# succinctlabs/sp1

Hardware: AMD Instinct MI355X
Metric: RISC-V cycles proved/sec (core shard prove): whole ShardProof of a full core shard of the reference's `fibonacci` guest, see config (higher is better)
Workload: dtype u32 (KoalaBear Montgomery words, exact integer arithmetic)

## Files before the change

### sp1_amd/csrc/gkr.hip

```cpp
#include <algorithm>
#include <array>
#include <chrono>
#include <cstring>
#include <optional>
#include <string>
#include <vector>

#include "device_ctx.hpp"
#include "host_par.hpp"

namespace sp1hip {
bool gkr_host_simd_available();
void gkr_host_round_sums(const uint32_t* tab, size_t stride, const uint32_t* eq, size_t eq_stride, size_t real_pairs, uint32_t out[6][4]);
void gkr_host_round_fold(const uint32_t* tab, uint32_t* out, size_t stride, size_t real_pairs, const uint32_t alpha[4]);
}
#include "round_sync.hpp"
#include "tensor_table.hpp"
#include "ext_host.hpp"
#include "gkr_kernels.hpp"
#include "gkr_rounds_host.hpp"

namespace sp1hip {

void challenger_observe(sp1hip_challenger_t* ch, uint32_t x);
kb::Ext challenger_sample_ext(sp1hip_challenger_t* ch);
void challenger_restore(sp1hip_challenger_t* dst, const sp1hip_challenger_t* src);

namespace gkr {

using namespace ext_host;

using gkr_rounds::Poly4;
Ext poly_eval(const Poly4& c, const Ext& x) { return ((c[3] * x + c[2]) * x + c[1]) * x + c[0]; }

Poly4 interpolate4(const Ext (&xs)[4], const Ext (&ys)[4]) {
    Poly4 res{kb::ext_zero(), kb::ext_zero(), kb::ext_zero(), kb::ext_zero()};
    Ext num[4][4], den[4];
    bool live[4];
    for (int i = 0; i < 4; i++) {
        live[i] = !kb::ext_eq(ys[i], kb::ext_zero());
        if (!live[i]) continue;
        den[i] = kb::ext_one();
        Ext cur[4] = {ys[i], kb::ext_zero(), kb::ext_zero(), kb::ext_zero()};
        int deg = 0;
        for (int j = 0; j < 4; j++) {
            if (j == i) continue;
            den[i] = den[i] * (xs[i] - xs[j]);
            Ext nxt[4] = {kb::ext_zero(), kb::ext_zero(), kb::ext_zero(), kb::ext_zero()};
            for (int k = 0; k <= deg; k++) { nxt[k + 1] = nxt[k + 1] + cur[k]; nxt[k] = nxt[k] - cur[k] * xs[j]; }
            deg++;
            for (int k = 0; k < 4; k++) cur[k] = nxt[k];
        }
        for (int k = 0; k < 4; k++) num[i][k] = cur[k];
    }
    Ext prefix[4], running = kb::ext_one();
    for (int i = 0; i < 4; i++) if (live[i]) { prefix[i] = running; running = running * den[i]; }
    Ext inv_all = kb::ext_inv(running);
    for (int i = 3; i >= 0; i--) {
        if (!live[i]) continue;
        const Ext inv = inv_all * prefix[i];
        inv_all = inv_all * den[i];
        for (int k = 0; k < 4; k++) res[k] = res[k] + num[i][k] * inv;
    }
    return res;
}

struct Bytes {
    std::vector<uint8_t> b;
    void u64(uint64_t v) { for (int i = 0; i < 8; i++) b.push_back((uint8_t)(v >> (8 * i))); }
    void felt(uint32_t m) { const uint32_t v = kb::from_monty(m); for (int i = 0; i < 4; i++) b.push_back((uint8_t)(v >> (8 * i))); }
    void ext(const Ext& e) { for (int k = 0; k < 4; k++) felt(e.c[k]); }
};

void observe_ext(sp1hip_challenger_t* ch, const Ext& e) { for (int k = 0; k < 4; k++) challenger_observe(ch, e.c[k]); }

struct ChipInfo {
    std::string name;
    uint32_t rows, k, main_w, prep_w, int0;
    const uint32_t* d_main;
    const uint32_t* d_prep;
};

constexpr uint32_t MAX_TILES = 512;
constexpr uint64_t GKR_LOOKAHEAD_DEFAULT = 4;
uint32_t tiles_for(uint64_t threads) { return (uint32_t)std::min<uint64_t>(std::max<uint64_t>((threads + 255) / 256, 1), MAX_TILES); }

struct ParsedInt { uint32_t is_send, kind; std::vector<uint32_t> mult; std::vector<std::vector<uint32_t>> values; };
struct RoundOut { Ext n0, n1, d0, d1; std::vector<Poly4> polys; Ext claimed_sum, eval; std::vector<Ext> point; };
struct PassShape { int fv, sv; bool first; uint32_t tiles, tile_size, total_slots; size_t flat_off; bool flat; };

struct GkrTimer {
    enum Part { ROWS, INT, LAYER_HEAD, WAIT, HOST, LAUNCH, SKIP };
    using Clock = std::chrono::steady_clock;
    bool on = false;
    Clock::time_point last, clk[2];
    double part_ms[7] = {};
    int waits = 0;
    static double ms(Clock::time_point a, Clock::time_point b) { return std::chrono::duration<double, std::milli>(b - a).count(); }
    void start() { static const bool env = env_flag("SP1HIP_GKR_DEBUG", false); on = env; last = Clock::now(); }
    void mark(const char* what) {
        if (!on) return;
        const auto now = Clock::now();
        fprintf(stderr, "[sp1hip gkr] %-28s %8.3f ms\n", what, ms(last, now));
        last = now;
    }
    void lap(Part p) {
        if (!on) return;
        const auto now = Clock::now();
        part_ms[p] += ms(clk[p >= WAIT], now);
        clk[p >= WAIT] = now;
        waits += p == WAIT;
    }
    void report_layers() {
        if (!on) return;
        fprintf(stderr, "[sp1hip gkr]   of which row-variable rounds %.3f ms, interaction-variable rounds (host) %.3f ms\n", part_ms[ROWS], part_ms[INT]);
        fprintf(stderr, "[sp1hip gkr]   %d hand-overs inside the layers: waiting for the sums %.3f ms, closed forms + transcript %.3f ms, launch calls %.3f ms\n",
                waits, part_ms[WAIT], part_ms[HOST], part_ms[LAUNCH]);
    }
};

struct Levels {
    int L = 0;
    uint32_t K = 0;
    std::vector<uint32_t> h;
    std::vector<size_t> entries;
    std::vector<std::vector<size_t>> off;
    std::vector<DeviceBuf> N, D;
    uint32_t rows_at(uint32_t i, int l) const { return (uint32_t)(((uint64_t)h[i] + (((uint64_t)1 << (L - l)) - 1)) >> (L - l)); }
    void* n_ptr(int l, uint32_t i) const { return (char*)N[l].p + off[l][i] * (l == L ? 4 : 16); }
    Ext* d_ptr(int l, uint32_t i) const { return D[l].ext() + off[l][i]; }
    int alloc(int L_, std::vector<uint32_t> rows_of_interaction, hipStream_t s) {
        L = L_; h = std::move(rows_of_interaction); K = (uint32_t)h.size();
        entries.assign(L + 2, 0);
        off.assign(L + 1, std::vector<size_t>(K + 1, 0));
        for (int l = 1; l <= L; l++) {
            for (uint32_t i = 0; i < K; i++) off[l][i + 1] = off[l][i] + rows_at(i, l);
            entries[l] = off[l][K];
        }
        N = std::vector<DeviceBuf>(L + 1); D = std::vector<DeviceBuf>(L + 1);
        for (int l = 1; l <= L; l++) {
            SP1HIP_TRY(N[l].alloc(std::max<size_t>(entries[l], 1) * (l == L ? 4 : 16), s));
            SP1HIP_TRY(D[l].alloc(std::max<size_t>(entries[l], 1) * 16, s));
        }
        return SP1HIP_SUCCESS;
    }
};

struct PassPlan {
    std::vector<PassShape> shapes;
    std::vector<PassDesc> all_descs;
    std::vector<uint16_t> flat_index;
};
struct PassChoice { int sv; bool flat; uint64_t total_slots; };
PassChoice choose_pass(const std::vector<uint32_t>& rows_in, int fv, int left, int depth, uint32_t flat_max_slots) {
    auto total_slots = [&](int sv) {
        uint64_t n = 0;
        for (uint32_t rin : rows_in) { const uint32_t ro = (rin + (1u << fv) - 1) >> fv; n += ((ro + (1u << sv) - 1) >> sv) << sv; }
        return n;
    };
    const bool index_fits = rows_in.size() <= 65536;
    if (depth > 2 && left > 2) {
        const int sv = std::min(depth, left);
        const uint64_t n = total_slots(sv);
        if (n <= flat_max_slots && index_fits) return PassChoice{sv, true, n};
    }
    const int sv = std::min(2, left);
    const uint64_t n = total_slots(sv);
    return PassChoice{sv, n <= flat_max_slots && index_fits, n};
}
size_t count_passes(const Levels& lv, uint32_t flat_max_slots, int depth) {
    size_t n = 0;
    std::vector<uint32_t> rows_in(lv.K);
    for (int v = 1; v <= lv.L - 1; v++) {
        for (uint32_t i = 0; i < lv.K; i++) rows_in[i] = (lv.rows_at(i, v + 1) + 1) / 2;
        for (int t = v, fv = 0;;) {
            const int sv = choose_pass(rows_in, fv, t - fv, depth, flat_max_slots).sv;
            for (uint32_t& r : rows_in) r = (r + (1u << fv) - 1) >> fv;
            t -= fv;
            n++;
            if (sv == 0) break;
            fv = sv;
        }
    }
    return n;
}

void plan_passes(const Levels& lv, uint32_t flat_max_slots, int depth, size_t n_passes, Ext* const (&scratch)[2], Ext* host_rows, PassPlan& plan) {
    const uint32_t K = lv.K;
    auto scratch_ptr = [&](int b, uint32_t i, int which, const std::vector<size_t>& so) -> Ext* { return scratch[b] + 4 * so[i] + (size_t)which * (so[i + 1] - so[i]); };
    constexpr uint32_t TARGET_TILES = 2048;
    plan.all_descs.reserve(n_passes * K);
    std::vector<uint32_t> rows_in(K);
    std::vector<size_t> so_prev, so_next;
    for (int v = 1; v <= lv.L - 1; v++) {
        for (uint32_t i = 0; i < K; i++) rows_in[i] = (lv.rows_at(i, v + 1) + 1) / 2;
        int cur = 0, t = v, fv = 0, pass = 0;
        for (;;) {
            const PassChoice choice = choose_pass(rows_in, fv, t - fv, depth, flat_max_slots);
            const int sv = choice.sv;
            const bool first = pass <= 1;
            if (fv > 0) { so_next.assign(K + 1, 0); for (uint32_t i = 0; i < K; i++) so_next[i + 1] = so_next[i] + ((rows_in[i] + (1u << fv) - 1) >> fv); }
            auto slots_of = [&](uint32_t rin) -> uint32_t { const uint32_t ro = (rin + (1u << fv) - 1) >> fv; return ((ro + (1u << sv) - 1) >> sv) << sv; };
            const uint64_t total_slots = choice.total_slots;
            const bool flat = choice.flat;
            const uint32_t tile_size = flat ? 1u : (uint32_t)std::max<uint64_t>(256, ((total_slots + TARGET_TILES - 1) / TARGET_TILES + 255) / 256 * 256);
            const size_t flat_off = plan.flat_index.size();
            plan.all_descs.resize(plan.all_descs.size() + K);
            PassDesc* out = plan.all_descs.data() + plan.all_descs.size() - K;
            uint32_t tile0 = 0;
            for (uint32_t i = 0; i < K; i++) {
                PassDesc& d = out[i];
                d = PassDesc{};
                d.rows_in = rows_in[i]; d.eq_int_index = i;
                if (first) { d.src[0] = lv.n_ptr(v + 1, i); d.src[1] = lv.d_ptr(v + 1, i); d.rows_x = lv.rows_at(i, v + 1); }
                else for (int w = 0; w < 4; w++) d.src[w] = scratch_ptr(cur ^ 1, i, w, so_prev);
                if (fv > 0) for (int w = 0; w < 4; w++)
                    d.dst[w] = (sv == 0 && host_rows) ? host_rows + 4 * so_next[i] + (size_t)w * (so_next[i + 1] - so_next[i]) : scratch_ptr(cur, i, w, so_next);
                d.tile0 = tile0;
                const uint32_t n_tiles = (slots_of(rows_in[i]) + tile_size - 1) / tile_size;
                if (flat) plan.flat_index.insert(plan.flat_index.end(), n_tiles, (uint16_t)i);
                tile0 += n_tiles;
// ... 97 lines not shown
        for (int w = 0; w < 4; w++) { tab[0][w].assign(W, (w & 1) ? kb::ext_one() : kb::ext_zero()); tab[1][w].resize(W / 2 + 1); }
    }
    void set_row(uint32_t i, const Ext* row) { for (int w = 0; w < 4; w++) tab[0][w][i] = row[w]; }
    RoundSums sums(int m, size_t real_pairs) const {
        const std::vector<Ext>& eqi = eq.tabs[m];
        const Ext *n0 = tab[side][0].data(), *d0 = tab[side][1].data(), *n1 = tab[side][2].data(), *d1 = tab[side][3].data();
        RoundSums parts[HostPar::Scope::MAX_THREADS];
        const int nparts = par.threads();
        for (int q = 0; q < nparts; q++) parts[q] = RoundSums{kb::ext_zero(), kb::ext_zero(), kb::ext_zero(), kb::ext_zero(), kb::ext_zero(), kb::ext_zero()};
        par.run(real_pairs, 24, [&](int part, size_t kb0, size_t ke) {
            RoundSums acc = parts[part];
            for (size_t k = kb0; k < ke; k++) {
                const size_t a = 2 * k, b = 2 * k + 1;
                acc.x0 = acc.x0 + eqi[a] * (d0[a] * n1[a] + d1[a] * n0[a]);
                acc.y0 = acc.y0 + eqi[a] * (d0[a] * d1[a]);
                const Ext sn0 = n0[a] + n0[b], sn1 = n1[a] + n1[b], sd0 = d0[a] + d0[b], sd1 = d1[a] + d1[b];
                const Ext es = eqi[a] + eqi[b];
                acc.xh = acc.xh + es * (sd0 * sn1 + sd1 * sn0);
                acc.yh = acc.yh + es * (sd0 * sd1);
                acc.e0 = acc.e0 + eqi[a];
                acc.es = acc.es + es;
            }
            parts[part] = acc;
        });
        RoundSums t = parts[0];
        for (int q = 1; q < nparts; q++) {
            t.x0 = t.x0 + parts[q].x0; t.y0 = t.y0 + parts[q].y0; t.xh = t.xh + parts[q].xh; t.yh = t.yh + parts[q].yh;
            t.e0 = t.e0 + parts[q].e0; t.es = t.es + parts[q].es;
        }
        return t;
    }
    void fold(size_t real_pairs, size_t half, const Ext& alpha) {
        const Ext *n0 = tab[side][0].data(), *d0 = tab[side][1].data(), *n1 = tab[side][2].data(), *d1 = tab[side][3].data();
        Ext *o0 = tab[side ^ 1][0].data(), *o1 = tab[side ^ 1][1].data(), *o2 = tab[side ^ 1][2].data(), *o3 = tab[side ^ 1][3].data();
        par.run(real_pairs, 48, [&](int, size_t kb0, size_t ke) {
            for (size_t k = kb0; k < ke; k++) {
                o0[k] = n0[2 * k] + alpha * (n0[2 * k + 1] - n0[2 * k]); o1[k] = d0[2 * k] + alpha * (d0[2 * k + 1] - d0[2 * k]);
                o2[k] = n1[2 * k] + alpha * (n1[2 * k + 1] - n1[2 * k]); o3[k] = d1[2 * k] + alpha * (d1[2 * k + 1] - d1[2 * k]);
            }
        });
        if (real_pairs < half) { o0[real_pairs] = kb::ext_zero(); o1[real_pairs] = kb::ext_one(); o2[real_pairs] = kb::ext_zero(); o3[real_pairs] = kb::ext_one(); }
        side ^= 1;
    }
    void first_row(Ext (&f)[4]) const { for (int w = 0; w < 4; w++) f[w] = tab[side][w][0]; }
};

template <class Tables>
void interaction_rounds(Tables& tb, size_t real, const std::vector<Ext>& int_point, const Ext& lambda, const Ext& PA, const Consts& k, LayerRounds& lr) {
    const int niv = (int)int_point.size();
    Ext eq_scale = k.one;
    for (int j = 0; j < niv; j++) {
        const size_t half = ((size_t)1 << (niv - j)) / 2, real_pairs = (real + 1) / 2;
        const RoundSums t = tb.sums(niv - j, real_pairs);
        const Ext pt = int_point[niv - 1 - j];
        const Ext s0 = lambda * t.x0 + t.y0 + ((k.one - pt) - t.e0);
        const Ext sh = lambda * t.xh + t.yh + (k.one - t.es) * k.four;
        const Ext PAe = PA * eq_scale;
        const Ext p0 = PAe * s0, ph = PAe * sh * k.inv8;
        const Ext xs[4] = {k.zero, k.one, k.inv2, (k.one - pt) * kb::ext_inv(k.one - (pt + pt))};
        const Ext ys[4] = {p0, lr.claim - p0, ph, k.zero};
        tb.fold(real_pairs, half, lr.finish_round(interpolate4(xs, ys), pt, eq_scale));
        real = real_pairs;
    }
    Ext f[4];
    tb.first_row(f);
    lr.ro.n0 = f[0]; lr.ro.d0 = f[1]; lr.ro.n1 = f[2]; lr.ro.d1 = f[3];
}

void interaction_rounds_host(bool simd, HostPar::Scope& par, const EqTabs& eq, uint32_t W, const std::vector<size_t>& so, const Ext* rows,
                             const std::vector<Ext>& int_point, const Ext& lambda, const Ext& PA, const Consts& k, LayerRounds& lr, GkrTimer& timer) {
    auto run = [&](auto tb) {
        const uint32_t K = (uint32_t)so.size() - 1;
        for (uint32_t i = 0; i < K; i++) if (so[i + 1] != so[i]) tb.set_row(i, rows + 4 * so[i]);
        timer.lap(GkrTimer::ROWS);
        interaction_rounds(tb, K, int_point, lambda, PA, k, lr);
        timer.lap(GkrTimer::INT);
    };
    if (simd) run(PlaneTables(eq, W)); else run(ScalarTables(eq, par, W));
}

#define SP1HIP_GKR_REQUIRE(cond, msg) \
    do { if (!(cond)) { sp1hip::set_error("sp1hip_logup_gkr_prove: %s", msg); return SP1HIP_ERROR_INVALID_ARGUMENT; } } while (0)

struct GkrProver {
    const sp1hip_gkr_chip_t* const chips;
    const int n_chips, L;
    sp1hip_challenger_t* const challenger;
    uint8_t* const h_proof;
    size_t* const proof_len;
    const sp1hip_stream_t stream;
    const hipStream_t s;

    GkrTimer timer;
    const Consts k;
    std::vector<ChipInfo> info;
    std::vector<ParsedInt> progs;
    size_t max_arity = 0, total_cols = 0, need = 0;
    uint32_t K = 0, W = 0;
    int niv = 0;
    struct Cloned { sp1hip_challenger_t* c = nullptr; ~Cloned() { sp1hip_challenger_free(c); } } clone;
    sp1hip_challenger_t* ch = nullptr;
    uint32_t witness = 0, flat_max_slots = 0;
    int lookahead = 2;
    Ext alpha;
    std::vector<Ext> betas;
    std::vector<uint32_t> int_chip;
    Levels lv;
    size_t n_passes_total = 0;
    hipStream_t side = nullptr;
    hipEvent_t* side_ev = nullptr;
    DeviceBuf d_all, d_flat;
    PinnedStage side_stage, stage;
    DeviceBuf d_progs, d_betas, d_descs;
    std::vector<uint32_t> flat;
    std::vector<IntDesc> descs;
    DeviceBuf d_trans, d_trans2;
    Mailbox mb;
    DeviceBuf d_eq_int, d_T, d_TL, d_partials, scratch[2];
    bool direct_final = false, simd = false;
    PassPlan plan;
    std::vector<Ext> out_n, out_d, eval_point;
    Ext num_eval, den_eval;
    size_t launch_idx = 0;
    RoundSyncHost rsync;
    std::optional<HostPar::Scope> par;
    std::vector<RoundOut> rounds;
    std::vector<Ext> trace_point, openings;

    int parse_programs() {
        info.resize(n_chips);
        for (int c = 0; c < n_chips; c++) {
            const sp1hip_gkr_chip_t& ci = chips[c];
            SP1HIP_GKR_REQUIRE(ci.name && ci.interactions, "null chip field");
            SP1HIP_GKR_REQUIRE(ci.real_rows <= ((uint64_t)1 << L), "chip taller than 2^max_log_row_count");
            SP1HIP_GKR_REQUIRE(ci.real_rows == 0 || ci.main_width == 0 || ci.d_main, "null main trace");
            SP1HIP_GKR_REQUIRE(ci.real_rows == 0 || ci.prep_width == 0 || ci.d_prep, "null preprocessed trace");
            if (c) SP1HIP_GKR_REQUIRE(strcmp(chips[c - 1].name, ci.name) < 0, "chips must be sorted by name (BTreeSet order)");
            info[c] = ChipInfo{ci.name, (uint32_t)ci.real_rows, 0, ci.main_width, ci.prep_width, (uint32_t)progs.size(), ci.d_main, ci.d_prep};
            const uint32_t* p = ci.interactions;
            const uint32_t* end = p + ci.n_words;
            SP1HIP_GKR_REQUIRE(ci.n_words >= 1, "empty interaction program");
            const uint32_t ni = *p++;
            info[c].k = ni;
            auto vcol = [&](std::vector<uint32_t>& out) -> bool {
                if (p + 2 > end) return false;
                const uint32_t nt = p[0];
                if (p[1] >= kb::P || p + 2 + 3 * (size_t)nt > end) return false;
                out.push_back(nt);
                out.push_back(kb::to_monty(p[1]));
                p += 2;
                for (uint32_t t = 0; t < nt; t++, p += 3) {
                    if (p[0] > 1 || p[2] >= kb::P) return false;
                    if (p[1] >= (p[0] ? ci.main_width : ci.prep_width)) return false;
                    out.push_back(p[0]); out.push_back(p[1]); out.push_back(kb::to_monty(p[2]));
                }
                return true;
            };
            for (uint32_t i = 0; i < ni; i++) {
                SP1HIP_GKR_REQUIRE(p + 3 <= end, "truncated interaction program");
                const uint32_t nv = p[2];
                SP1HIP_GKR_REQUIRE(p[0] <= 1 && p[1] < kb::P && nv < 4096, "bad interaction header");
                ParsedInt pi{p[0], p[1], {}, std::vector<std::vector<uint32_t>>(nv)};
                p += 3;
                SP1HIP_GKR_REQUIRE(vcol(pi.mult), "bad multiplicity column");
                for (uint32_t j = 0; j < nv; j++) SP1HIP_GKR_REQUIRE(vcol(pi.values[j]), "bad value column (index or weight out of range)");
                max_arity = std::max<size_t>(max_arity, nv + 1);
                progs.push_back(std::move(pi));
            }
            SP1HIP_GKR_REQUIRE(p == end, "trailing words in interaction program");
            total_cols += (size_t)ci.main_width + ci.prep_width;
        }
        K = (uint32_t)progs.size();
        SP1HIP_GKR_REQUIRE(K >= 1, "no interactions in the shard");
        niv = log2_ceil(K);
        W = 1u << niv;
        return SP1HIP_SUCCESS;
    }

    size_t proof_size() const {
        size_t n = 2 * (8 + (size_t)2 * W * 16 + 24) + 8;
        for (int v = 1; v <= L - 1; v++) n += 64 + 8 + (size_t)(niv + v) * (8 + 64) + 16 + 8 + (size_t)(niv + v) * 16 + 16;
        n += 8 + (size_t)L * 16 + 8;
        for (int c = 0; c < n_chips; c++) {
            n += 8 + info[c].name.size() + 8 + (size_t)info[c].main_w * 16 + 16 + 1;
            if (info[c].prep_w) n += 8 + (size_t)info[c].prep_w * 16 + 16;
        }
        return n + 4;
    }

    int transcript_head() {
        SP1HIP_TRY(sp1hip_challenger_clone(challenger, &clone.c));
        ch = clone.c;
        SP1HIP_TRY(sp1hip_challenger_grind(ch, 12, &witness, stream));
        alpha = challenger_sample_ext(ch);
        std::vector<Ext> beta_seed(log2_ceil(max_arity));
        for (auto& b : beta_seed) b = challenger_sample_ext(ch);
        (void)challenger_sample_ext(ch);
        betas = partial_lagrange_host(beta_seed);
        return SP1HIP_SUCCESS;
    }

    int alloc_levels_and_plan_buffers() {
        int_chip.resize(K);
        std::vector<uint32_t> rows(K);
        for (int c = 0; c < n_chips; c++) for (uint32_t i = 0; i < info[c].k; i++) { int_chip[info[c].int0 + i] = c; rows[info[c].int0 + i] = info[c].rows; }
        SP1HIP_TRY(lv.alloc(L, std::move(rows), s));
        timer.mark("parse + level buffers");
        flat_max_slots = (uint32_t)env_uint("SP1HIP_GKR_FLAT_SLOTS", 65536);
        lookahead = (int)std::min<uint64_t>(std::max<uint64_t>(env_uint("SP1HIP_GKR_LOOKAHEAD", GKR_LOOKAHEAD_DEFAULT), 2), 4);
        n_passes_total = count_passes(lv, flat_max_slots, lookahead);
        SP1HIP_TRY(aux_stream_for(s, 2, &side, &side_ev));
        SP1HIP_TRY(d_all.alloc(std::max<size_t>(n_passes_total * K, 1) * sizeof(PassDesc), side));
        SP1HIP_TRY(d_flat.alloc((n_passes_total * (size_t)flat_max_slots + 4) * sizeof(uint16_t), side));
        SP1HIP_TRY(side_stage.init(side));
        return stage.init(s);
    }

    int build_first_layer_and_tree() {
        std::vector<size_t> poff(K);
        for (uint32_t i = 0; i < K; i++) {
            poff[i] = flat.size();
            const ParsedInt& pi = progs[i];
            Ext head = alpha + kb::ext_mul_base(betas[0], kb::to_monty(pi.kind));
            uint32_t live = 0;
            for (size_t j = 0; j < pi.values.size(); j++) {
                if (pi.values[j][0] == 0) head = head + kb::ext_mul_base(betas[1 + j], pi.values[j][1]);
                else live++;
            }
            flat.insert(flat.end(), {pi.is_send, live, head.c[0], head.c[1], head.c[2], head.c[3]});
            flat.insert(flat.end(), pi.mult.begin(), pi.mult.end());
            for (size_t j = 0; j < pi.values.size(); j++) {
                if (pi.values[j][0] == 0) continue;
                flat.push_back((uint32_t)(1 + j));
                flat.insert(flat.end(), pi.values[j].begin(), pi.values[j].end());
            }
        }
        SP1HIP_TRY(upload(d_progs, flat.data(), flat.size() * 4, s, stage));
        SP1HIP_TRY(upload(d_betas, betas.data(), betas.size() * 16, s, stage));
        uint32_t max_rows = 0;
        descs.resize(K);
        for (uint32_t i = 0; i < K; i++) {
            const ChipInfo& c = info[int_chip[i]];
            descs[i] = IntDesc{d_progs.u32() + poff[i], c.d_main, c.d_prep, c.rows, (uint32_t*)lv.n_ptr(L, i), lv.d_ptr(L, i)};
            max_rows = std::max(max_rows, c.rows);
        }
        const bool fused_tree = L >= 3 && env_flag("SP1HIP_GKR_FUSED", true);
        if (fused_tree) {
            std::vector<FirstDesc> fdescs(K);
            for (uint32_t i = 0; i < K; i++)
                fdescs[i] = FirstDesc{descs[i].prog, descs[i].main, descs[i].prep, descs[i].rows, descs[i].n_out, descs[i].d_out,
                                      (Ext*)lv.n_ptr(L - 1, i), lv.d_ptr(L - 1, i), (Ext*)lv.n_ptr(L - 2, i), lv.d_ptr(L - 2, i)};
            SP1HIP_TRY(upload(d_descs, fdescs.data(), fdescs.size() * sizeof(FirstDesc), s, stage));
            if (max_rows) {
                ScopedTimer t("gkr_first_layer", s);
                hipLaunchKernelGGL(first_layers_kernel, dim3(tiles_for((max_rows + 3) / 4), K), dim3(256), 0, s, (const FirstDesc*)d_descs.p,
                                   (const Ext*)d_betas.p);
                SP1HIP_LAUNCH_CHECK();
            }
        } else {
            SP1HIP_TRY(upload(d_descs, descs.data(), descs.size() * sizeof(IntDesc), s, stage));
            if (max_rows) {
                ScopedTimer t("gkr_first_layer", s);
                hipLaunchKernelGGL(first_layer_kernel, dim3(tiles_for(max_rows), K), dim3(256), 0, s, (const IntDesc*)d_descs.p,
                                   (const Ext*)d_betas.p);
                SP1HIP_LAUNCH_CHECK();
            }
        }
        timer.mark("first layer enqueued");
        const int top = fused_tree ? L - 2 : L;
        std::vector<Trans2Desc> t2;
        std::vector<TransDesc> t1;
        std::vector<uint32_t> t2_mr, t1_mr;
        std::vector<int> t1_level;
        int l = top;
        if (fused_tree)
            for (; l >= 3; l -= 2) {
                uint32_t mr = 0;
                for (uint32_t i = 0; i < K; i++) {
                    const uint32_t rin = lv.rows_at(i, l);
                    t2.push_back(Trans2Desc{(const Ext*)lv.n_ptr(l, i), lv.d_ptr(l, i), (Ext*)lv.n_ptr(l - 1, i), lv.d_ptr(l - 1, i), (Ext*)lv.n_ptr(l - 2, i), lv.d_ptr(l - 2, i), rin});
                    mr = std::max(mr, (rin + 3) / 4);
                }
                t2_mr.push_back(mr);
            }
        for (; l >= 2; l--) {
            uint32_t mr = 0;
            for (uint32_t i = 0; i < K; i++) {
                const uint32_t rin = lv.rows_at(i, l);
                t1.push_back(TransDesc{lv.n_ptr(l, i), lv.d_ptr(l, i), (Ext*)lv.n_ptr(l - 1, i), lv.d_ptr(l - 1, i), rin});
                mr = std::max(mr, (rin + 1) / 2);
            }
            t1_mr.push_back(mr);
            t1_level.push_back(l);
        }
        if (!t2.empty()) SP1HIP_TRY(upload(d_trans2, t2.data(), t2.size() * sizeof(Trans2Desc), s, stage));
        if (!t1.empty()) SP1HIP_TRY(upload(d_trans, t1.data(), t1.size() * sizeof(TransDesc), s, stage));
        for (size_t j = 0; j < t2_mr.size(); j++) {
            if (!t2_mr[j]) continue;
            ScopedTimer t("gkr_transition", s);
            hipLaunchKernelGGL(transition2_kernel, dim3(tiles_for(t2_mr[j]), K), dim3(256), 0, s, (const Trans2Desc*)d_trans2.p + j * K);
            SP1HIP_LAUNCH_CHECK();
        }
        for (size_t j = 0; j < t1_mr.size(); j++) {
            if (!t1_mr[j]) continue;
            const TransDesc* d_t = (const TransDesc*)d_trans.p + j * K;
            ScopedTimer t("gkr_transition", s);
            if (t1_level[j] == L) hipLaunchKernelGGL(transition_kernel<true>, dim3(tiles_for(t1_mr[j]), K), dim3(256), 0, s, d_t);
            else hipLaunchKernelGGL(transition_kernel<false>, dim3(tiles_for(t1_mr[j]), K), dim3(256), 0, s, d_t);
            SP1HIP_LAUNCH_CHECK();
        }
        timer.mark("tree enqueued");
        return SP1HIP_SUCCESS;
    }

    int plan_and_upload_passes() {
        SP1HIP_TRY(mb.init(s));
        SP1HIP_TRY(d_eq_int.alloc((size_t)W * 16, s));
        SP1HIP_TRY(d_T.alloc(((size_t)2 << std::max(L - 1, 1)) * 16, s));
// ... 201 lines not shown
            for (uint32_t g = 0; g < info[c].prep_w; g += OPEN_COLS) od.push_back(OpenDesc{info[c].d_prep, info[c].rows, info[c].prep_w, g, out0 + g});
            out0 += info[c].prep_w;
            max_rows_open = std::max(max_rows_open, info[c].rows);
        }
        const uint32_t chunks = std::max<uint32_t>((max_rows_open + OPEN_ROWS - 1) / OPEN_ROWS, 1);
        SP1HIP_TRY(upload(d_od, od.data(), od.size() * sizeof(OpenDesc), s, stage));
        SP1HIP_TRY(d_part.alloc((size_t)chunks * total_cols * 16, s));
        SP1HIP_TRY(d_res.alloc(total_cols * 16, s));
        SP1HIP_HIP(hipMemsetAsync(d_part.p, 0, (size_t)chunks * total_cols * 16, s));
        ScopedTimer t("gkr_openings", s);
        hipLaunchKernelGGL(open_columns_kernel, dim3((uint32_t)od.size(), chunks), dim3(256), 0, s, (const OpenDesc*)d_od.p, d_eq.u32(),
                           1u << L, d_part.u32(), (uint32_t)total_cols);
        SP1HIP_LAUNCH_CHECK();
        hipLaunchKernelGGL(open_sum_kernel, dim3(((uint32_t)total_cols * 4 + 63) / 64), dim3(256), 0, s, d_part.u32(), chunks,
                           (uint32_t)total_cols * 4, d_res.u32());
        SP1HIP_LAUNCH_CHECK();
        return mb.fetch(d_res.p, total_cols * 4, openings.data());
    }

    void observe_openings() {
        challenger_observe(ch, kb::to_monty((uint32_t)n_chips));
        size_t o = 0;
        for (int c = 0; c < n_chips; c++) {
            const Ext* main = openings.data() + o;
            const Ext* prep = main + info[c].main_w;
            if (info[c].prep_w) {
                challenger_observe(ch, kb::to_monty(info[c].prep_w));
                for (uint32_t j = 0; j < info[c].prep_w; j++) observe_ext(ch, prep[j]);
            }
            challenger_observe(ch, kb::to_monty(info[c].main_w));
            for (uint32_t j = 0; j < info[c].main_w; j++) observe_ext(ch, main[j]);
            o += info[c].main_w + info[c].prep_w;
        }
        timer.mark("openings");
    }

    int write_proof() {
        Bytes w;
        for (const std::vector<Ext>* vv : {&out_n, &out_d}) {
            w.u64(vv->size());
            for (auto& e : *vv) w.ext(e);
            w.u64(2); w.u64(vv->size()); w.u64(1);
        }
        w.u64(rounds.size());
        for (auto& r : rounds) {
            w.ext(r.n0); w.ext(r.n1); w.ext(r.d0); w.ext(r.d1);
            w.u64(r.polys.size());
            for (auto& p : r.polys) { w.u64(4); for (auto& c : p) w.ext(c); }
            w.ext(r.claimed_sum);
            w.u64(r.point.size());
            for (auto& x : r.point) w.ext(x);
            w.ext(r.eval);
        }
        w.u64(trace_point.size());
        for (auto& x : trace_point) w.ext(x);
        w.u64(n_chips);
        size_t o = 0;
        for (int c = 0; c < n_chips; c++) {
            w.u64(info[c].name.size());
            for (char chr : info[c].name) w.b.push_back((uint8_t)chr);
            w.u64(info[c].main_w);
            for (uint32_t j = 0; j < info[c].main_w; j++) w.ext(openings[o + j]);
            w.u64(1); w.u64(info[c].main_w);
            w.b.push_back(info[c].prep_w ? 1 : 0);
            if (info[c].prep_w) {
                w.u64(info[c].prep_w);
                for (uint32_t j = 0; j < info[c].prep_w; j++) w.ext(openings[o + info[c].main_w + j]);
                w.u64(1); w.u64(info[c].prep_w);
            }
            o += info[c].main_w + info[c].prep_w;
        }
        w.felt(witness);
        if (w.b.size() != need) {
            set_error("internal error: GKR proof size %zu != expected %zu", w.b.size(), need);
            return SP1HIP_ERROR_RUNTIME;
        }
        memcpy(h_proof, w.b.data(), w.b.size());
        *proof_len = w.b.size();
        return SP1HIP_SUCCESS;
    }

    int prove() {
        timer.start();
        SP1HIP_TRY(parse_programs());
        need = proof_size();
        if (!h_proof || *proof_len < need) {
            *proof_len = need;
            set_error("sp1hip_logup_gkr_prove: proof buffer too small, need %zu bytes", need);
            return SP1HIP_ERROR_BUFFER_TOO_SMALL;
        }
        const DeviceCtx* ctx;
        SP1HIP_TRY(get_device_ctx(&ctx));
        SP1HIP_TRY(transcript_head());
        SP1HIP_TRY(alloc_levels_and_plan_buffers());
        SP1HIP_TRY(build_first_layer_and_tree());
        SP1HIP_TRY(plan_and_upload_passes());
        SP1HIP_TRY(fetch_circuit_output());
        SP1HIP_TRY(prove_layers());
        SP1HIP_TRY(open_traces());
        observe_openings();
        SP1HIP_TRY(write_proof());
        challenger_restore(challenger, ch);
        return SP1HIP_SUCCESS;
    }
};
#undef SP1HIP_GKR_REQUIRE
}
}

using namespace sp1hip;

extern "C" int sp1hip_logup_gkr_prove(const sp1hip_gkr_chip_t* chips, int n_chips, int max_log_row_count, sp1hip_challenger_t* challenger,
                                      uint8_t* h_proof, size_t* proof_len, sp1hip_stream_t stream) {
    SP1HIP_REQUIRE(chips && n_chips > 0 && challenger && proof_len, "bad argument");
    SP1HIP_REQUIRE(max_log_row_count >= 1 && max_log_row_count <= 30, "max_log_row_count out of range");
    gkr::GkrProver p{chips, n_chips, max_log_row_count, challenger, h_proof, proof_len, stream, S(stream)};
    return p.prove();
}
```

### sp1_amd/csrc/jagged.hip

```cpp
#include <algorithm>
#include <array>
#include <chrono>
#include <cstring>
#include <vector>

#include "device_ctx.hpp"
#include "jagged_host.hpp"
#include "round_sync.hpp"
#include "stacked_data.hpp"
#include "tensor_table.hpp"
#include "ext_host.hpp"
#include "jagged_kernels.hpp"

namespace sp1hip {

void challenger_observe(sp1hip_challenger_t* ch, uint32_t x);
kb::Ext challenger_sample_ext(sp1hip_challenger_t* ch);
void challenger_restore(sp1hip_challenger_t* dst, const sp1hip_challenger_t* src);

namespace {

using namespace ext_host;

struct Bytes {
// ... 99 lines not shown
};

struct StageMarks {
    bool open = false;
    void next(const char* name) { if (open) roctx_pop(); roctx_push(name); open = true; }
    ~StageMarks() { if (open) roctx_pop(); }
};

struct FirstRoundsPlan {
    int rf = 0;
    std::vector<JgTab> tabs0;
    uint32_t n_tiles0 = 0, n_tiles1 = 0, n_tiles2 = 0;
    bool tables_mult4 = false;
    bool skip_level1 = false;
    bool lookahead01 = false;
    std::vector<std::pair<uint64_t, uint64_t>> zero_tails;
    bool table_major() const { return !tabs0.empty(); }
};

FirstRoundsPlan plan_first_rounds(const std::vector<uint32_t>& prefix, uint32_t T, int log_m, int max_log_row_count,
                                  StackedCore* const* rounds, int n_rounds, bool factored, bool lookahead) {
    FirstRoundsPlan pl;
    uint32_t g = T;
    for (uint32_t pfx : prefix) g |= pfx;
    pl.rf = g ? __builtin_ctz(g) : 0;
    pl.rf = std::min(pl.rf, std::min(log_m - 2, max_log_row_count - 1));
    if (!factored) pl.rf = 0;
    if (pl.rf < 2) pl.rf = 0;
    if ((g & 1u) != 0 || !factored) return pl;
    uint64_t seg_start = 0;
    uint32_t col = 0;
    for (int r = 0; r < n_rounds; r++) {
        const StackedCore* d = rounds[r];
        uint64_t off = 0;
        const size_t n_real = d->row_counts.size() - 2;
        for (size_t t = 0; t < d->row_counts.size(); t++) {
            const uint32_t h = (uint32_t)d->row_counts[t], w = (uint32_t)d->column_counts[t];
            if (t < n_real && h && w) {
                for (uint32_t c_lo = 0; c_lo < w; c_lo += JG_COL_SLICE) {
                    const uint32_t wc = std::min(JG_COL_SLICE, w - c_lo);
                    const uint64_t o = off + (uint64_t)c_lo * h;
                    pl.tabs0.push_back(JgTab{(const uint32_t*)d->d_dense + o, h, col + c_lo, wc, pl.n_tiles0, (uint32_t)(seg_start + o),
                                             pl.n_tiles1, pl.n_tiles2});
                    pl.n_tiles0 += (h / 2 + JG_TAB_PAIRS - 1) / JG_TAB_PAIRS;
                    pl.n_tiles1 += ((h + 3) / 4 + JG_TAB_PAIRS - 1) / JG_TAB_PAIRS;
                    pl.n_tiles2 += ((h + 7) / 8 + JG_TAB_PAIRS - 1) / JG_TAB_PAIRS;
                }
            }
            if (t == n_real) pl.zero_tails.push_back({seg_start + off, seg_start + d->padded});
            off += (uint64_t)h * w;
            col += w;
        }
        seg_start += d->padded;
    }
    if (pl.table_major()) {
        pl.tables_mult4 = (g & 3u) == 0;
        pl.skip_level1 = (g & 7u) == 0 && pl.rf >= 2 && log_m >= 4;
        pl.lookahead01 = pl.skip_level1 && lookahead;
    }
    return pl;
}

void build_layer_matrices(const std::vector<Ext>& z_row, const std::vector<Ext>& z_index, int D, std::vector<Ext>* out) {
    auto lsb = [](const std::vector<Ext>& p, size_t i) { return p.size() <= i ? kb::ext_zero() : p[p.size() - 1 - i]; };
    out->assign((size_t)D * 4 * 16, kb::ext_zero());
    const Ext one = kb::ext_one();
    for (int layer = 0; layer < D; layer++) {
        const Ext zr = lsb(z_row, layer), zi = lsb(z_index, layer);
        const Ext er[2] = {one - zr, zr}, ei[2] = {one - zi, zi};
        for (int cb = 0; cb < 2; cb++)
            for (int nb = 0; nb < 2; nb++)
                for (int m = 0; m < 4; m++) {
                    const int carry = m & 1, cmp = m >> 1;
                    for (int rb = 0; rb < 2; rb++)
                        for (int ib = 0; ib < 2; ib++) {
                            const int sum = rb + carry + cb;
                            if (ib != (sum & 1)) continue;
                            const int new_cmp = ib == nb ? cmp : nb;
                            const int target = (sum >> 1) + 2 * new_cmp;
                            Ext& e = (*out)[(((size_t)layer * 4 + cb * 2 + nb) * 4 + m) * 4 + target];
                            e = e + er[rb] * ei[ib];
                        }
                }
    }
}

struct JeProver {
    const std::vector<uint32_t>& prefix;
    const int D;
    const std::vector<Ext>&z_row, &z_col, &z_trace;
    Scratch& sc;
    RoundTranscript& tr;

    const hipStream_t s = sc.s;
    const Ext half = kb::ext_inv(ext_c(2));
    uint32_t n = 0, nb = 0;
    std::vector<Ext> mats;
    DeviceBuf d_t, d_u, d_zc, d_mats, d_suffix, d_state, d_inter;
    JeCols C{};
    std::vector<Ext> B;
    DeviceBuf d_B, d_suffix2;

    int setup_columns() {
        const std::vector<Ext> col_eq = partial_lagrange_host(z_col);
        std::vector<uint32_t> ts, us;
        std::vector<Ext> zc;
        for (size_t c = 0; c + 1 < prefix.size(); c++) {
            if (!ts.empty() && ts.back() == prefix[c] && us.back() == prefix[c + 1]) zc.back() = zc.back() + col_eq[c];
            else { ts.push_back(prefix[c]); us.push_back(prefix[c + 1]); zc.push_back(col_eq[c]); }
        }
        n = (uint32_t)ts.size();
        SP1HIP_TRY(upload(d_t, ts.data(), n * 4, s, sc.stage));
        SP1HIP_TRY(upload(d_u, us.data(), n * 4, s, sc.stage));
        SP1HIP_TRY(upload(d_zc, zc.data(), (size_t)n * 16, s, sc.stage));
        build_layer_matrices(z_row, z_trace, D, &mats);
        SP1HIP_TRY(upload(d_mats, mats.data(), mats.size() * 16, s, sc.stage));
        SP1HIP_TRY(d_suffix.alloc((size_t)D * n * 64, s));
        SP1HIP_TRY(d_state.alloc((size_t)n * 128, s));
        SP1HIP_TRY(d_inter.alloc((size_t)n * 16, s));
        C = JeCols{d_t.u32(), d_u.u32(), d_zc.ext(), n};
        nb = Scratch::blocks_for(n);
        return SP1HIP_SUCCESS;
    }

    int finish_round() {
        SP1HIP_LAUNCH_CHECK();
        Ext y0, yh;
        SP1HIP_TRY(sc.finish(&y0, &yh));
        tr.finish_round(y0, yh + yh + yh + yh);
        return SP1HIP_SUCCESS;
    }

    int phase1() {
        hipLaunchKernelGGL(je_suffix_kernel<true>, dim3(nb), dim3(256), 0, s, C, (const Ext*)d_mats.p, D, d_suffix.ext(), sc.tail());
        SP1HIP_LAUNCH_CHECK();
        Ext expected_sum, unused;
        SP1HIP_TRY(sc.finish(&expected_sum, &unused));
        observe_ext(tr.ch, expected_sum);
        tr.begin(expected_sum);
        for (int r = 0; r < D; r++) {
            hipLaunchKernelGGL(je_phase1_round, dim3(nb), dim3(256), 0, s, C, (const Ext*)d_mats.p, (const Ext*)d_suffix.p, D, r, tr.alpha,
                               half, d_state.ext(), d_inter.ext(), sc.tail());
            SP1HIP_TRY(finish_round());
        }
        return SP1HIP_SUCCESS;
    }

    int phase2() {
        B.resize((size_t)D * 2 * 16);
        for (int layer = 0; layer < D; layer++)
            for (int cb = 0; cb < 2; cb++)
                for (int e = 0; e < 16; e++) {
                    const Ext a0 = mats[((size_t)layer * 4 + cb * 2 + 0) * 16 + e], a1 = mats[((size_t)layer * 4 + cb * 2 + 1) * 16 + e];
                    B[((size_t)layer * 2 + cb) * 16 + e] = a0 + tr.alphas[layer] * (a1 - a0);
                }
        SP1HIP_TRY(upload(d_B, B.data(), B.size() * 16, s, sc.stage));
        SP1HIP_TRY(d_suffix2.alloc((size_t)D * n * 64, s));
        hipLaunchKernelGGL(je_suffix_kernel<false>, dim3(nb), dim3(256), 0, s, C, (const Ext*)d_B.p, D, d_suffix2.ext(), sc.tail());
        SP1HIP_LAUNCH_CHECK();
        Ext W[4] = {kb::ext_one(), kb::ext_zero(), kb::ext_zero(), kb::ext_zero()};
        for (int rp = 0; rp < D; rp++) {
            Ext V[8];
            for (int b = 0; b < 2; b++)
                for (int k = 0; k < 4; k++) {
                    Ext acc = kb::ext_zero();
                    for (int m = 0; m < 4; m++) acc = acc + W[m] * B[((size_t)rp * 2 + b) * 16 + 4 * m + k];
// ... 500 lines not shown
```

### sp1_amd/csrc/prover.hip

```cpp
#include <algorithm>
#include <array>
#include <cstring>
#include <functional>
#include <memory>
#include <vector>

#include "basefold_host.hpp"

namespace sp1hip {


struct DuplexChallenger {
    uint32_t state[16] = {0};
    uint32_t in[8];
    int n_in = 0;
    uint32_t out[8];
    int n_out = 0;
    uint32_t injected[4];
    int n_injected = 0, next_injected = 0;

    void duplexing() {
        for (int i = 0; i < n_in; i++) state[i] = in[i];
        n_in = 0;
        p2_host_permute(state);
// ... 406 lines not shown
    *out = new sp1hip_challenger_s(*ch);
    return SP1HIP_SUCCESS;
}
void sp1hip_challenger_free(sp1hip_challenger_t* ch) { delete ch; }
int sp1hip_challenger_observe(sp1hip_challenger_t* ch, const uint32_t* felts, size_t n) {
    SP1HIP_REQUIRE(ch && (felts || n == 0), "null argument");
    for (size_t i = 0; i < n; i++) SP1HIP_REQUIRE(felts[i] < kb::P, "non-reduced field word");
    ch->ch.observe_slice(felts, n);
    return SP1HIP_SUCCESS;
}
int sp1hip_challenger_sample(sp1hip_challenger_t* ch, uint32_t* out) {
    SP1HIP_REQUIRE(ch && out, "null argument");
    *out = ch->ch.sample();
    return SP1HIP_SUCCESS;
}
int sp1hip_challenger_sample_ext(sp1hip_challenger_t* ch, sp1hip_ext_t* out) {
    SP1HIP_REQUIRE(ch && out, "null argument");
    kb::Ext e = ch->ch.sample_ext();
    memcpy(out->c, e.c, 16);
    return SP1HIP_SUCCESS;
}
int sp1hip_challenger_sample_bits(sp1hip_challenger_t* ch, int bits, uint32_t* out) {
    SP1HIP_REQUIRE(ch && out && bits >= 0 && bits < 32, "bad argument");
    *out = ch->ch.sample_bits(bits);
    return SP1HIP_SUCCESS;
}
int sp1hip_challenger_check_witness(sp1hip_challenger_t* ch, int bits, uint32_t witness, int* ok) {
    SP1HIP_REQUIRE(ch && ok && bits >= 0 && bits < 32 && witness < kb::P, "bad argument");
    *ok = ch->ch.check_witness(bits, witness) ? 1 : 0;
    return SP1HIP_SUCCESS;
}
int sp1hip_challenger_grind(sp1hip_challenger_t* ch, int bits, uint32_t* witness, sp1hip_stream_t stream) {
    SP1HIP_REQUIRE(ch && witness, "null argument");
    return grind(ch->ch, bits, witness, S(stream));
}
int sp1hip_challenger_inject_pow_witnesses(sp1hip_challenger_t* ch, const uint32_t* witnesses, int n) {
    SP1HIP_REQUIRE(ch && n >= 0 && n <= 4 && (witnesses || n == 0), "bad argument");
    for (int i = 0; i < n; i++) SP1HIP_REQUIRE(witnesses[i] < kb::P, "witness not a canonical field element");
    for (int i = 0; i < n; i++) ch->ch.injected[i] = witnesses[i];
    ch->ch.n_injected = n;
    ch->ch.next_injected = 0;
    return SP1HIP_SUCCESS;
}
int sp1hip_challenger_state(const sp1hip_challenger_t* ch, uint32_t* out34) {
    SP1HIP_REQUIRE(ch && out34, "null argument");
    memset(out34, 0, 34 * 4);
    memcpy(out34, ch->ch.state, 64);
    out34[16] = (uint32_t)ch->ch.n_in;
    memcpy(out34 + 17, ch->ch.in, 4 * ch->ch.n_in);
    out34[25] = (uint32_t)ch->ch.n_out;
    memcpy(out34 + 26, ch->ch.out, 4 * ch->ch.n_out);
    return SP1HIP_SUCCESS;
}

}

namespace sp1hip {
int basefold_data_alloc(BasefoldData* pd, const sp1hip_tensor_t* mles, int n_mles, int lg_n, int lg_blowup, hipStream_t s) {
    pd->lg_n = lg_n;
    pd->lg_blowup = lg_blowup;
    const size_t N = (size_t)1 << (lg_n + lg_blowup);
    for (int i = 0; i < n_mles; i++) {
        pd->mles.push_back(mles[i]);
        pd->cws.emplace_back(new DeviceBuf());
        SP1HIP_TRY(pd->cws.back()->alloc(N * mles[i].width * 4, s));
        pd->cw_tensors.push_back({pd->cws.back()->u32(), mles[i].width});
        pd->total_width += mles[i].width;
    }
    return pd->tree.alloc((2 * N - 1) * 32, s);
}

int basefold_data_fetch_commit(BasefoldData* pd, const uint32_t* d_root_and_commit, uint32_t h_commit[8], hipStream_t s) {
    uint32_t h[16];
    Mailbox mb;
    SP1HIP_TRY(mb.init(s));
    SP1HIP_TRY(mb.fetch(d_root_and_commit, 16, h));
    memcpy(pd->root, h, 32);
    memcpy(pd->commit, h + 8, 32);
    memcpy(h_commit, pd->commit, 32);
    return SP1HIP_SUCCESS;
}

int commit_mles_hooked(const sp1hip_tensor_t* mles, int n_mles, int lg_n, int lg_blowup, uint32_t h_commit[8],
                       sp1hip_basefold_data_t** out, sp1hip_stream_t stream, const std::function<int(int, hipStream_t)>* before_encode) {
    SP1HIP_REQUIRE(mles && n_mles > 0 && out && h_commit, "bad argument");
    SP1HIP_REQUIRE(lg_n >= 0 && lg_blowup >= 0 && lg_n + lg_blowup <= kb::TWO_ADICITY, "size out of range");
    hipStream_t s = S(stream);
    const DeviceCtx* ctx;
    SP1HIP_TRY(get_device_ctx(&ctx));
    std::unique_ptr<sp1hip_basefold_data_s> pd(new sp1hip_basefold_data_s());
    for (int i = 0; i < n_mles; i++) SP1HIP_REQUIRE(mles[i].d_data || mles[i].width == 0, "null mle");
    SP1HIP_TRY(basefold_data_alloc(pd.get(), mles, n_mles, lg_n, lg_blowup, s));
    const int lg_h = lg_n + lg_blowup;
    const size_t N = (size_t)1 << lg_h;
    DeviceBuf rc;
    SP1HIP_TRY(rc.alloc(64, s));
    const bool overlap = env_flag("SP1HIP_COMMIT_OVERLAP", N * (size_t)pd->total_width >= ((size_t)1 << 24));
    std::vector<LeafPart> parts;
    if (overlap) leaf_hash_plan(pd->cw_tensors.data(), n_mles, &parts);
    if (parts.size() >= 2) {
        hipStream_t aux;
        hipEvent_t* ev;
        SP1HIP_TRY(aux_stream_for(s, n_mles + 1, &aux, &ev));
        struct Join {
            hipStream_t aux;
            ~Join() { (void)hipStreamSynchronize(aux); }
        };
        TensorTable tab;
        uint32_t tw;
        SP1HIP_TRY(make_tensor_table(pd->cw_tensors.data(), n_mles, &tab, &tw));
        DeviceBuf cols, carry;
        SP1HIP_TRY(cols.alloc((size_t)tw * sizeof(uint32_t*), s));
        SP1HIP_TRY(carry.alloc(N * 8 * 4, s));
        SP1HIP_TRY(expand_columns_async(tab, tw, N, (const uint32_t**)cols.p, s));
        SP1HIP_HIP(hipEventRecord(ev[n_mles], s));
        SP1HIP_HIP(hipStreamWaitEvent(aux, ev[n_mles], 0));
        {
            Join join{aux};
            for (int i = 0; i < n_mles; i++) {
                if (before_encode) SP1HIP_TRY((*before_encode)(i, aux));
                SP1HIP_TRY(sp1hip_rs_encode_batch(pd->cws[i]->u32(), mles[i].d_data, lg_n, lg_blowup, mles[i].width, aux));
                SP1HIP_HIP(hipEventRecord(ev[i], aux));
            }
            for (int k = 0; k < (int)parts.size(); k++) {
                SP1HIP_HIP(hipStreamWaitEvent(s, ev[parts[k].last_tensor], 0));
                SP1HIP_TRY(leaf_hash_part((const uint32_t* const*)cols.p + parts[k].c0, parts[k].width, k, (int)parts.size(),
                                          (uint32_t)N, carry.u32(), pd->tree.u32(), ctx, s));
            }
            SP1HIP_TRY(merkle_finish_tree(pd->tree.u32(), lg_h, tw, rc.u32(), ctx, s));
            SP1HIP_TRY(basefold_data_fetch_commit(pd.get(), rc.u32(), h_commit, s));
        }
        *out = pd.release();
        return SP1HIP_SUCCESS;
    }
    for (int i = 0; i < n_mles; i++) {
        if (before_encode) SP1HIP_TRY((*before_encode)(i, s));
        SP1HIP_TRY(sp1hip_rs_encode_batch(pd->cws[i]->u32(), mles[i].d_data, lg_n, lg_blowup, mles[i].width, s));
    }
    SP1HIP_TRY(sp1hip_merkle_commit(pd->cw_tensors.data(), n_mles, lg_h, pd->tree.u32(), rc.u32(), s));
    SP1HIP_TRY(basefold_data_fetch_commit(pd.get(), rc.u32(), h_commit, s));
    *out = pd.release();
    return SP1HIP_SUCCESS;
}
}

extern "C" {

int sp1hip_commit_mles(const sp1hip_tensor_t* mles, int n_mles, int lg_n, int lg_blowup, uint32_t h_commit[8],
                       sp1hip_basefold_data_t** out, sp1hip_stream_t stream) {
    return commit_mles_hooked(mles, n_mles, lg_n, lg_blowup, h_commit, out, stream, nullptr);
}

void sp1hip_basefold_data_free(sp1hip_basefold_data_t* data) { delete data; }

int sp1hip_basefold_data_codeword(const sp1hip_basefold_data_t* data, int k, const uint32_t** d_cw, uint32_t* width,
                                  int* lg_height) {
    SP1HIP_REQUIRE(data && k >= 0 && k < (int)data->cws.size(), "bad argument");
    if (d_cw) *d_cw = data->cws[k]->u32();
    if (width) *width = data->mles[k].width;
    if (lg_height) *lg_height = data->lg_n + data->lg_blowup;
    return SP1HIP_SUCCESS;
}
int sp1hip_basefold_data_tree(const sp1hip_basefold_data_t* data, const uint32_t** d_tree, int* lg_height) {
    SP1HIP_REQUIRE(data, "null argument");
    if (d_tree) *d_tree = data->tree.u32();
    if (lg_height) *lg_height = data->lg_n + data->lg_blowup;
    return SP1HIP_SUCCESS;
}

size_t sp1hip_basefold_proof_size(int dim, const uint32_t* round_widths, int n_rounds, sp1hip_fri_config_t config) {
    return basefold_proof_size(32, dim, round_widths, n_rounds, config);
}

int sp1hip_basefold_prove(const sp1hip_ext_t* h_point, int dim, sp1hip_basefold_data_t* const* rounds, int n_rounds,
                          const sp1hip_ext_t* h_claims, size_t n_claims, sp1hip_fri_config_t config,
                          sp1hip_challenger_t* challenger, uint8_t* h_proof, size_t* proof_len, sp1hip_stream_t stream) {
    SP1HIP_REQUIRE(rounds && n_rounds > 0 && challenger, "null argument");
    std::vector<BasefoldData*> data(rounds, rounds + n_rounds);
    InnerBasefoldBackend be(challenger->ch);
    return basefold_prove_with(be, h_point, dim, data.data(), n_rounds, h_claims, n_claims, config, h_proof, proof_len, stream);
}

}
```

### sp1_amd/csrc/shard.hip

```cpp
#include <chrono>
#include <cstring>
#include <memory>
#include <string>
#include <mutex>
#include <unordered_map>
#include <vector>

#include "device_ctx.hpp"
#include "stacked_data.hpp"

namespace sp1hip {
void challenger_observe(sp1hip_challenger_t* ch, uint32_t x);
kb::Ext challenger_sample_ext(sp1hip_challenger_t* ch);
void challenger_restore(sp1hip_challenger_t* dst, const sp1hip_challenger_t* src);
size_t jagged_proof_size(int lsh, const std::vector<uint32_t>& round_widths, const std::vector<size_t>& tables_per_round,
                         uint64_t total_area, sp1hip_fri_config_t config);

namespace {

struct Reader {
    const uint8_t* p;
    size_t n, o = 0;
    uint64_t u64() { uint64_t v = 0; for (int i = 0; i < 8; i++) v |= (uint64_t)p[o + i] << (8 * i); o += 8; return v; }
    uint32_t canonical() { uint32_t v = 0; for (int i = 0; i < 4; i++) v |= (uint32_t)p[o + i] << (8 * i); o += 4; return v; }
    kb::Ext ext() { kb::Ext e; for (int k = 0; k < 4; k++) e.c[k] = kb::to_monty(canonical()); return e; }
    void skip(size_t k) { o += k; }
};

void put_u64(std::vector<uint8_t>& b, uint64_t v) { for (int i = 0; i < 8; i++) b.push_back((uint8_t)(v >> (8 * i))); }
void put_felt(std::vector<uint8_t>& b, uint32_t monty) { const uint32_t v = kb::from_monty(monty); for (int i = 0; i < 4; i++) b.push_back((uint8_t)(v >> (8 * i))); }

}
}

using namespace sp1hip;

extern "C" {

int sp1hip_prove_shard(const sp1hip_shard_chip_t* chips, int n_chips, const uint32_t* h_publics, int n_publics,
                       sp1hip_stacked_data_t* preprocessed, sp1hip_shard_params_t params, sp1hip_challenger_t* challenger,
                       uint8_t* h_proof, size_t* proof_len, sp1hip_stream_t stream) {
    SP1HIP_REQUIRE(chips && n_chips > 0 && preprocessed && challenger && proof_len, "bad argument");
    SP1HIP_REQUIRE(h_publics || n_publics == 0, "null public values");
    ActiveProver active;
    const auto sh_entry = std::chrono::steady_clock::now();
    uint64_t miss_n0 = 0, miss_b0 = 0;
    arena_miss_stats(&miss_n0, &miss_b0);
    const int L = params.max_log_row_count, lsh = params.log_stacking_height;
    SP1HIP_REQUIRE(preprocessed->jagged && preprocessed->max_log_row_count == L && preprocessed->log_stacking_height == lsh,
                   "the preprocessed round was committed with different parameters");
    hipStream_t s = S(stream);

    std::vector<sp1hip_gkr_chip_t> gk(n_chips);
    std::vector<sp1hip_zc_chip_t> zc(n_chips);
    std::vector<sp1hip_table_t> tables(n_chips);
    uint64_t main_area = 0;
    size_t total_w = 0, prep_cols = 0, opened_bytes = 8;
    for (int c = 0; c < n_chips; c++) {
        const sp1hip_shard_chip_t& ci = chips[c];
        SP1HIP_REQUIRE(ci.name && ci.program && ci.interactions, "null chip field");
        SP1HIP_REQUIRE(ci.main_width > 0, "a chip needs at least one main column");
        gk[c] = sp1hip_gkr_chip_t{ci.name, ci.interactions, ci.n_words, ci.main_width, ci.prep_width, ci.d_main, ci.d_prep, ci.real_rows};
        zc[c] = sp1hip_zc_chip_t{ci.program, ci.n_instr, ci.main_width, ci.prep_width, ci.num_constraints, ci.d_main, ci.d_prep, ci.real_rows};
        tables[c] = sp1hip_table_t{ci.d_main, ci.real_rows, ci.main_width};
        main_area += ci.real_rows * (uint64_t)ci.main_width;
        total_w += ci.main_width + ci.prep_width;
        prep_cols += ci.prep_width;
        opened_bytes += 8 + strlen(ci.name) + 8 + (size_t)ci.prep_width * 16 + 8 + (size_t)ci.main_width * 16 + 8 + (size_t)(L + 1) * 4;
    }
    SP1HIP_REQUIRE(prep_cols > 0, "a shard needs at least one preprocessed column (two commitment rounds)");
    SP1HIP_REQUIRE(main_area > 0, "empty shard");
    uint64_t shape_sig = 0xcbf29ce484222325ull;
    {
        auto mix = [&](uint64_t v) { shape_sig = (shape_sig ^ v) * 0x100000001b3ull; };
        mix((uint64_t)n_chips); mix((uint64_t)L); mix((uint64_t)lsh); mix((uint64_t)params.fri.log_blowup); mix((uint64_t)params.fri.num_queries);
        for (int c = 0; c < n_chips; c++) { mix(chips[c].real_rows); mix((uint64_t)chips[c].main_width << 32 | (uint32_t)chips[c].n_instr); }
    }

    size_t gkr_size = 0, zc_size = 0;
    uint64_t size_sig = shape_sig;
    for (int c = 0; c < n_chips; c++) {
        size_sig = (size_sig ^ ((uint64_t)chips[c].n_words << 32 | chips[c].num_constraints)) * 0x100000001b3ull;
        size_sig = (size_sig ^ ((uint64_t)strlen(chips[c].name) << 32 | chips[c].prep_width)) * 0x100000001b3ull;
    }
    size_sig = (size_sig ^ (uint64_t)n_publics) * 0x100000001b3ull;
    static std::mutex size_mutex;
    static std::unordered_map<uint64_t, std::pair<size_t, size_t>> size_cache;
    bool have_sizes = false;
    {
        std::lock_guard<std::mutex> lk(size_mutex);
        auto it = size_cache.find(size_sig);
        if (it != size_cache.end()) { gkr_size = it->second.first; zc_size = it->second.second; have_sizes = true; }
    }
    if (!have_sizes) {
        int st = sp1hip_logup_gkr_prove(gk.data(), n_chips, L, challenger, nullptr, &gkr_size, stream);
        if (st != SP1HIP_ERROR_BUFFER_TOO_SMALL) return st == SP1HIP_SUCCESS ? SP1HIP_ERROR_RUNTIME : st;
        std::vector<sp1hip_ext_t> dummy(std::max<size_t>({total_w, (size_t)L, 1}));
        st = sp1hip_zerocheck_prove(zc.data(), n_chips, L, dummy.data(), dummy.data(), dummy[0], dummy[0], h_publics, n_publics,
                                    challenger, nullptr, &zc_size, stream);
        if (st != SP1HIP_ERROR_BUFFER_TOO_SMALL) return st == SP1HIP_SUCCESS ? SP1HIP_ERROR_RUNTIME : st;
        std::lock_guard<std::mutex> lk(size_mutex);
        if (size_cache.size() > 4096) size_cache.clear();
        size_cache[size_sig] = {gkr_size, zc_size};
    }
    const uint64_t H = (uint64_t)1 << lsh;
    const uint64_t main_padded = std::max<uint64_t>((main_area + H - 1) / H, 1) * H;
    const std::vector<uint32_t> round_widths{(uint32_t)(preprocessed->padded >> lsh), (uint32_t)(main_padded >> lsh)};
    const std::vector<size_t> tables_per_round{preprocessed->row_counts.size(), (size_t)n_chips + 2};
    const size_t jag_size = jagged_proof_size(lsh, round_widths, tables_per_round, preprocessed->padded + main_padded, params.fri);
    const size_t zc_sumcheck_size = zc_size - (8 + (size_t)n_chips * 8 + total_w * 16);
    const size_t need = 8 + (size_t)n_publics * 4 + 32 + gkr_size + zc_sumcheck_size + opened_bytes + jag_size;
    if (!h_proof || *proof_len < need) {
        *proof_len = need;
        set_error("sp1hip_prove_shard: proof buffer too small, need %zu bytes", need);
        return SP1HIP_ERROR_BUFFER_TOO_SMALL;
    }

    const bool sh_timing = env_flag("SP1HIP_SHARD_TIMING", false);
    std::chrono::steady_clock::time_point sh_t[6];
    sh_t[0] = std::chrono::steady_clock::now();
    RoctxRange proof_range("sp1hip_prove_shard");
    struct StageMarks {
        hipStream_t s;
        bool open = false;
        int idx = -1;
        void close() { if (idx >= 0) timer_end(idx, s); idx = -1; if (open) roctx_pop(); open = false; set_stage_note(""); }
        void next(const char* name) {
            close();
            roctx_push(name);
            set_stage_note(name);
            open = true;
            if (timers_on()) { char buf[64]; snprintf(buf, sizeof buf, "stage_%s", name); idx = timer_begin(buf, s); }
        }
        ~StageMarks() { close(); }
    } marks{S(stream)};
    WaitPlan wait_plan(shape_sig);
    marks.next("commit");
    sp1hip_challenger_t* ch = nullptr;
    SP1HIP_TRY(sp1hip_challenger_clone(challenger, &ch));
    struct ChGuard { sp1hip_challenger_t* c; ~ChGuard() { sp1hip_challenger_free(c); } } guard{ch};

    for (int i = 0; i < n_publics; i++) {
        SP1HIP_REQUIRE(h_publics[i] < kb::P, "public value not reduced");
        challenger_observe(ch, h_publics[i]);
    }
    uint32_t main_commit[8];
    sp1hip_stacked_data_t* main_data = nullptr;
    SP1HIP_TRY(sp1hip_jagged_commit(tables.data(), n_chips, L, lsh, params.batch_size, params.fri.log_blowup, main_commit, &main_data, stream));
    std::unique_ptr<sp1hip_stacked_data_s> main_guard(main_data);
    for (int k = 0; k < 8; k++) challenger_observe(ch, main_commit[k]);
    challenger_observe(ch, kb::to_monty((uint32_t)n_chips));
    for (int c = 0; c < n_chips; c++) {
        challenger_observe(ch, kb::to_monty((uint32_t)chips[c].real_rows));
        const size_t nl = strlen(chips[c].name);
        challenger_observe(ch, kb::to_monty((uint32_t)nl));
        for (size_t b = 0; b < nl; b++) challenger_observe(ch, kb::to_monty((uint8_t)chips[c].name[b]));
    }

    sh_t[1] = std::chrono::steady_clock::now();
    marks.next("logup_gkr");
    std::vector<uint8_t> gkr_blob(gkr_size);
    size_t glen = gkr_size;
    SP1HIP_TRY(sp1hip_logup_gkr_prove(gk.data(), n_chips, L, ch, gkr_blob.data(), &glen, stream));
    std::vector<kb::Ext> zeta(L), openings;
    {
        Reader r{gkr_blob.data(), glen};
        for (int k = 0; k < 2; k++) { const uint64_t m = r.u64(); r.skip(m * 16 + 24); }
        const uint64_t nr = r.u64();
        for (uint64_t k = 0; k < nr; k++) {
            r.skip(64);
            const uint64_t np = r.u64();
            for (uint64_t q = 0; q < np; q++) { const uint64_t nc = r.u64(); r.skip(nc * 16); }
            r.skip(16);
            const uint64_t pl = r.u64();
            r.skip(pl * 16 + 16);
        }
        SP1HIP_REQUIRE(r.u64() == (uint64_t)L, "internal: GKR point dimension");
        for (auto& z : zeta) z = r.ext();
        SP1HIP_REQUIRE(r.u64() == (uint64_t)n_chips, "internal: GKR chip count");
        for (int c = 0; c < n_chips; c++) {
            r.skip(r.u64());
            const uint64_t mw = r.u64();
            for (uint64_t k = 0; k < mw; k++) openings.push_back(r.ext());
            r.skip(16);
            if (r.p[r.o++]) {
                const uint64_t pw = r.u64();
                for (uint64_t k = 0; k < pw; k++) openings.push_back(r.ext());
                r.skip(16);
            }
        }
    }
    sh_t[2] = std::chrono::steady_clock::now();
    marks.next("zerocheck");
    const kb::Ext batching = challenger_sample_ext(ch), gkr_batch = challenger_sample_ext(ch);
    sp1hip_ext_t c_batching, c_gkr;
    memcpy(&c_batching, &batching, 16);
    memcpy(&c_gkr, &gkr_batch, 16);
    std::vector<uint8_t> zc_blob(zc_size);
    size_t zlen = zc_size;
    SP1HIP_TRY(sp1hip_zerocheck_prove(zc.data(), n_chips, L, reinterpret_cast<const sp1hip_ext_t*>(zeta.data()),
                                      reinterpret_cast<const sp1hip_ext_t*>(openings.data()), c_batching, c_gkr, h_publics, n_publics, ch,
                                      zc_blob.data(), &zlen, stream));
    std::vector<kb::Ext> z_row(L), prep_claims, main_claims;
    std::vector<std::vector<kb::Ext>> chip_evals(n_chips);
    {
        Reader r{zc_blob.data(), zlen};
        const uint64_t np = r.u64();
        for (uint64_t q = 0; q < np; q++) { const uint64_t nc = r.u64(); r.skip(nc * 16); }
        r.skip(16);
        SP1HIP_REQUIRE(r.u64() == (uint64_t)L, "internal: zerocheck point dimension");
        for (auto& z : z_row) z = r.ext();
        r.skip(16);
        SP1HIP_REQUIRE(r.o == zc_sumcheck_size, "internal: zerocheck sumcheck size");
        SP1HIP_REQUIRE(r.u64() == (uint64_t)n_chips, "internal: zerocheck chip count");
        for (int c = 0; c < n_chips; c++) {
            const uint64_t w = r.u64();
            SP1HIP_REQUIRE(w == (uint64_t)chips[c].main_width + chips[c].prep_width, "internal: zerocheck opening width");
            for (uint64_t k = 0; k < w; k++) chip_evals[c].push_back(r.ext());
            prep_claims.insert(prep_claims.end(), chip_evals[c].begin(), chip_evals[c].begin() + chips[c].prep_width);
            main_claims.insert(main_claims.end(), chip_evals[c].begin() + chips[c].prep_width, chip_evals[c].end());
        }
    }
    sh_t[3] = std::chrono::steady_clock::now();
    marks.next("evaluation_proof");
    std::vector<kb::Ext> claims = prep_claims;
    claims.insert(claims.end(), main_claims.begin(), main_claims.end());
    const size_t per_round[2] = {prep_claims.size(), main_claims.size()};
    sp1hip_stacked_data_t* rounds[2] = {preprocessed, main_data};
    SP1HIP_REQUIRE(need >= jag_size, "internal error: shard proof sizes");
    uint8_t* const jag_at = h_proof + (need - jag_size);
    size_t jlen = jag_size;
    SP1HIP_TRY(sp1hip_jagged_prove(reinterpret_cast<const sp1hip_ext_t*>(z_row.data()), L, rounds, 2,
                                   reinterpret_cast<const sp1hip_ext_t*>(claims.data()), per_round, params.fri, ch, jag_at, &jlen,
                                   stream));
    SP1HIP_REQUIRE(jlen == jag_size, "internal error: jagged proof size");
    (void)s;

    sh_t[4] = std::chrono::steady_clock::now();
    marks.next("proof_bytes");
    std::vector<uint8_t> out;
    out.reserve(need - jag_size);
    put_u64(out, n_publics);
    for (int i = 0; i < n_publics; i++) put_felt(out, h_publics[i]);
    for (int k = 0; k < 8; k++) put_felt(out, main_commit[k]);
    out.insert(out.end(), gkr_blob.begin(), gkr_blob.begin() + glen);
    out.insert(out.end(), zc_blob.begin(), zc_blob.begin() + zc_sumcheck_size);
    put_u64(out, n_chips);
    for (int c = 0; c < n_chips; c++) {
        const size_t nl = strlen(chips[c].name);
        put_u64(out, nl);
        out.insert(out.end(), chips[c].name, chips[c].name + nl);
        put_u64(out, chips[c].prep_width);
        for (uint32_t k = 0; k < chips[c].prep_width; k++) for (int q = 0; q < 4; q++) put_felt(out, chip_evals[c][k].c[q]);
        put_u64(out, chips[c].main_width);
        for (uint32_t k = 0; k < chips[c].main_width; k++) for (int q = 0; q < 4; q++) put_felt(out, chip_evals[c][chips[c].prep_width + k].c[q]);
        put_u64(out, L + 1);
        for (int b = L; b >= 0; b--) put_felt(out, ((chips[c].real_rows >> b) & 1) ? kb::R1 : 0u);
    }
    if (out.size() + jlen != need) {
        set_error("internal error: shard proof size %zu != expected %zu", out.size() + jlen, need);
        return SP1HIP_ERROR_RUNTIME;
    }
    memcpy(h_proof, out.data(), out.size());
    *proof_len = need;
    challenger_restore(challenger, ch);
    if (sh_timing) {
        sh_t[5] = std::chrono::steady_clock::now();
        const auto ms = [&](int a, int b) { return std::chrono::duration<double, std::milli>(sh_t[b] - sh_t[a]).count(); };
        uint64_t miss_n1 = 0, miss_b1 = 0;
        arena_miss_stats(&miss_n1, &miss_b1);
        fprintf(stderr, "[sp1hip shard] prologue %.3f ms | commit %.3f | LogUp-GKR %.3f | zerocheck %.3f | evaluation proof %.3f | proof bytes %.3f | %llu arena misses (%.1f MB)\n",
                std::chrono::duration<double, std::milli>(sh_t[0] - sh_entry).count(), ms(0, 1), ms(1, 2), ms(2, 3), ms(3, 4), ms(4, 5),
                (unsigned long long)(miss_n1 - miss_n0), (double)(miss_b1 - miss_b0) / 1e6);
    }
    wait_plan.ok = true;
    return SP1HIP_SUCCESS;
}


struct sp1hip_pk_s {
    sp1hip_stacked_data_t* preprocessed = nullptr;
    sp1hip_vk_t vk{};
    sp1hip_shard_params_t params{};
    ~sp1hip_pk_s() { if (preprocessed) sp1hip_stacked_data_free(preprocessed); }
};

int sp1hip_setup(const sp1hip_table_t* preprocessed_tables, int n_tables, const uint32_t pc_start[3],
                 const uint32_t initial_global_cumulative_sum[14], uint32_t enable_untrusted_programs,
                 sp1hip_shard_params_t params, sp1hip_pk_t** out, sp1hip_stream_t stream) {
    SP1HIP_REQUIRE(preprocessed_tables && n_tables > 0 && pc_start && initial_global_cumulative_sum && out, "null argument");
    for (int i = 0; i < 3; i++) SP1HIP_REQUIRE(pc_start[i] < kb::P, "pc_start not reduced");
    for (int i = 0; i < 14; i++) SP1HIP_REQUIRE(initial_global_cumulative_sum[i] < kb::P, "cumulative sum not reduced");
    SP1HIP_REQUIRE(enable_untrusted_programs < kb::P, "flag not reduced");
    std::unique_ptr<sp1hip_pk_s> pk(new sp1hip_pk_s());
    SP1HIP_TRY(sp1hip_jagged_commit(preprocessed_tables, n_tables, params.max_log_row_count, params.log_stacking_height,
                                    params.batch_size, params.fri.log_blowup, pk->vk.preprocessed_commit, &pk->preprocessed, stream));
    memcpy(pk->vk.pc_start, pc_start, 12);
    memcpy(pk->vk.initial_global_cumulative_sum, initial_global_cumulative_sum, 56);
    pk->vk.enable_untrusted_programs = enable_untrusted_programs;
    pk->params = params;
    *out = pk.release();
    return SP1HIP_SUCCESS;
}

void sp1hip_pk_free(sp1hip_pk_t* pk) { delete pk; }

int sp1hip_pk_vk(const sp1hip_pk_t* pk, sp1hip_vk_t* out) {
    SP1HIP_REQUIRE(pk && out, "null argument");
    *out = pk->vk;
    return SP1HIP_SUCCESS;
}

int sp1hip_vk_observe_into(const sp1hip_vk_t* vk, sp1hip_challenger_t* challenger) {
    SP1HIP_REQUIRE(vk && challenger, "null argument");
    for (int k = 0; k < 8; k++) challenger_observe(challenger, vk->preprocessed_commit[k]);
    for (int k = 0; k < 3; k++) challenger_observe(challenger, vk->pc_start[k]);
    for (int k = 0; k < 14; k++) challenger_observe(challenger, vk->initial_global_cumulative_sum[k]);
    challenger_observe(challenger, vk->enable_untrusted_programs);
    for (int k = 0; k < 6; k++) challenger_observe(challenger, 0u);
    return SP1HIP_SUCCESS;
}

int sp1hip_prove_shard_with_pk(const sp1hip_pk_t* pk, const sp1hip_shard_chip_t* chips, int n_chips, const uint32_t* h_publics,
                               int n_publics, const uint32_t* pow_witnesses, int n_pow_witnesses, uint8_t* h_proof, size_t* proof_len,
                               sp1hip_stream_t stream) {
    SP1HIP_REQUIRE(pk && proof_len, "null argument");
    sp1hip_challenger_t* ch = nullptr;
    SP1HIP_TRY(sp1hip_challenger_new(&ch));
    struct ChGuard { sp1hip_challenger_t* c; ~ChGuard() { sp1hip_challenger_free(c); } } guard{ch};
    SP1HIP_TRY(sp1hip_vk_observe_into(&pk->vk, ch));
    if (n_pow_witnesses) SP1HIP_TRY(sp1hip_challenger_inject_pow_witnesses(ch, pow_witnesses, n_pow_witnesses));
    return sp1hip_prove_shard(chips, n_chips, h_publics, n_publics, pk->preprocessed, pk->params, ch, h_proof, proof_len, stream);
}

}
```

### sp1_amd/csrc/stacked.hip

```cpp
#include <cstring>
#include <memory>
#include <algorithm>
#include <functional>
#include <vector>

#include "device_ctx.hpp"
#include "round_sync.hpp"
#include "stacked_data.hpp"
#include "tensor_table.hpp"

using namespace sp1hip;

namespace sp1hip {
int commit_mles_hooked(const sp1hip_tensor_t* mles, int n_mles, int lg_n, int lg_blowup, uint32_t h_commit[8],
                       sp1hip_basefold_data_t** out, sp1hip_stream_t stream, const std::function<int(int, hipStream_t)>* before_encode);
}

namespace {
struct DenseSeg { const uint32_t* src; uint64_t dst_off, n; };
__global__ __launch_bounds__(256) void dense_fill_kernel(const DenseSeg* __restrict__ segs, uint32_t* __restrict__ dense) {
    const DenseSeg sg = segs[blockIdx.y];
    uint32_t* dst = dense + sg.dst_off;
    for (uint64_t base = (uint64_t)blockIdx.x * 1024u; base < sg.n; base += (uint64_t)gridDim.x * 1024u) {
#pragma unroll
        for (int k = 0; k < 4; k++) {
            const uint64_t i = base + (uint64_t)k * 256u + threadIdx.x;
            if (i < sg.n) dst[i] = sg.src[i];
        }
    }
}

void host_hash(const std::vector<uint32_t>& in, uint32_t out[8]) {
    uint32_t s[16] = {0};
    size_t fill = 0;
    for (uint32_t x : in) {
        s[fill++] = x;
        if (fill == 8) { p2_host_permute(s); fill = 0; }
    }
    if (fill) p2_host_permute(s);
    memcpy(out, s, 32);
}
void host_compress(const uint32_t l[8], const uint32_t r[8], uint32_t out[8]) {
    uint32_t s[16];
    memcpy(s, l, 32);
    memcpy(s + 8, r, 32);
    p2_host_permute(s);
    memcpy(out, s, 32);
}
}

namespace sp1hip {

int stacked_commit_dense(const sp1hip_table_t* tables, int n_tables, int log_stacking_height, int batch_size, int lg_blowup,
                         StackedCore* sd, uint64_t* num_added_vals, hipStream_t s, const std::function<int(const FillBatch&)>& commit) {
    SP1HIP_REQUIRE((tables || n_tables == 0) && n_tables >= 0 && sd, "bad argument");
    SP1HIP_REQUIRE(log_stacking_height >= 0 && log_stacking_height + lg_blowup <= kb::TWO_ADICITY, "stacking height out of range");
    SP1HIP_REQUIRE(batch_size >= 1, "batch_size must be positive");
    const DeviceCtx* ctx;
    SP1HIP_TRY(get_device_ctx(&ctx));
    const uint64_t H = (uint64_t)1 << log_stacking_height;
    uint64_t area = 0;
    for (int i = 0; i < n_tables; i++) {
        SP1HIP_REQUIRE(tables[i].d_data || tables[i].rows * tables[i].cols == 0, "null table data");
        area += tables[i].rows * (uint64_t)tables[i].cols;
    }
    uint64_t padded = ((area + H - 1) / H) * H;
    if (padded < H) padded = H;
    sd->stream = s;
    sd->area = area;
    sd->padded = padded;
    sd->log_stacking_height = log_stacking_height;
    SP1HIP_TRY(arena_alloc(&sd->d_dense, padded * 4, s));
    std::vector<uint64_t> table_off(n_tables + 1, 0);
    for (int i = 0; i < n_tables; i++) table_off[i + 1] = table_off[i] + tables[i].rows * (uint64_t)tables[i].cols;
    if (padded > area) SP1HIP_HIP(hipMemsetAsync((uint32_t*)sd->d_dense + area, 0, (padded - area) * 4, s));
    uint32_t* const dense = (uint32_t*)sd->d_dense;
    const uint64_t batch_words = (uint64_t)batch_size * H;
    const uint64_t n_batches_total = area == 0 ? 1 : (padded / H + (uint64_t)batch_size - 1) / (uint64_t)batch_size;
    std::vector<DenseSeg> segs;
    std::vector<std::pair<uint32_t, uint32_t>> batch_segs(n_batches_total, {0u, 0u});
    std::vector<uint64_t> batch_max(n_batches_total, 0);
    for (uint64_t b = 0; b < n_batches_total; b++) {
        const uint64_t lo = b * batch_words, hi = std::min<uint64_t>(lo + batch_words, area);
        batch_segs[b].first = (uint32_t)segs.size();
        for (int i = 0; i < n_tables && lo < hi; i++) {
            const uint64_t a = std::max(lo, table_off[i]), e = std::min(hi, table_off[i + 1]);
            if (a < e) { segs.push_back(DenseSeg{tables[i].d_data + (a - table_off[i]), a, e - a}); batch_max[b] = std::max(batch_max[b], e - a); }
        }
        batch_segs[b].second = (uint32_t)segs.size() - batch_segs[b].first;
    }
    AsyncScratch d_segs;
    PinnedStage seg_stage;
    SP1HIP_TRY(seg_stage.init(s));
    SP1HIP_TRY(d_segs.alloc(std::max<size_t>(segs.size(), 1) * sizeof(DenseSeg), s));
    SP1HIP_TRY(seg_stage.upload(d_segs.p, segs.data(), segs.size() * sizeof(DenseSeg)));
    const std::function<int(int, hipStream_t)> fill_batch = [&](int b, hipStream_t on) -> int {
        if ((uint64_t)b >= n_batches_total || batch_segs[b].second == 0) return SP1HIP_SUCCESS;
        const uint32_t gx = (uint32_t)std::min<uint64_t>((batch_max[b] + 1023) / 1024, 2048);
        hipLaunchKernelGGL(dense_fill_kernel, dim3(gx, batch_segs[b].second), dim3(256), 0, on,
                           (const DenseSeg*)d_segs.p + batch_segs[b].first, dense);
        SP1HIP_LAUNCH_CHECK();
        return SP1HIP_SUCCESS;
    };
    const uint64_t ncols = area == 0 ? 0 : padded / H;
    if (ncols == 0) sd->batches.push_back({(const uint32_t*)sd->d_dense, 0u});
    for (uint64_t c0 = 0; c0 < ncols; c0 += (uint64_t)batch_size) {
        const uint32_t w = (uint32_t)std::min<uint64_t>((uint64_t)batch_size, ncols - c0);
        sd->batches.push_back({(const uint32_t*)sd->d_dense + c0 * H, w});
    }
    SP1HIP_REQUIRE(sd->batches.size() <= 128, "more than 128 stacked batches in one commitment");
    SP1HIP_TRY(commit(fill_batch));
    if (num_added_vals) *num_added_vals = padded - area;
    return SP1HIP_SUCCESS;
}

int jagged_select_tables(const sp1hip_table_t* tables, int n_tables, int max_log_row_count, JaggedTables* out) {
    SP1HIP_REQUIRE((tables || n_tables == 0) && out, "bad argument");
    SP1HIP_REQUIRE(max_log_row_count >= 0 && max_log_row_count <= 30, "max_log_row_count out of range");
    const uint64_t M = (uint64_t)1 << max_log_row_count;
    for (int i = 0; i < n_tables; i++) {
        SP1HIP_REQUIRE(tables[i].rows <= M, "table taller than 2^max_log_row_count");
        out->rows.push_back(tables[i].rows);
        out->cols.push_back(tables[i].cols);
        if (tables[i].rows) out->dense.push_back(tables[i]);
    }
    return SP1HIP_SUCCESS;
}

std::vector<uint32_t> jagged_finish_counts(uint64_t added, int max_log_row_count, JaggedTables&& t, StackedCore* sd) {
    const uint64_t M = (uint64_t)1 << max_log_row_count;
    uint64_t added_cols = (added + M - 1) / M;
    if (added_cols < 1) added_cols = 1;
    t.rows.push_back(M);
    t.rows.push_back(added - (added_cols - 1) * M);
    t.cols.push_back(added_cols - 1);
    t.cols.push_back(1);
    std::vector<uint32_t> meta;
    meta.push_back((uint32_t)t.rows.size());
    for (uint64_t r : t.rows) meta.push_back((uint32_t)r);
    for (uint64_t c : t.cols) meta.push_back((uint32_t)c);
    sd->jagged = true;
    sd->max_log_row_count = max_log_row_count;
    sd->row_counts = std::move(t.rows);
    sd->column_counts = std::move(t.cols);
    sd->padding_column_count = added_cols;
    return meta;
}

}

extern "C" {

int sp1hip_stacked_commit(const sp1hip_table_t* tables, int n_tables, int log_stacking_height, int batch_size,
                          int lg_blowup, uint32_t h_commit[8], uint64_t* num_added_vals, sp1hip_stacked_data_t** out,
                          sp1hip_stream_t stream) {
    SP1HIP_REQUIRE(h_commit && out, "bad argument");
    std::unique_ptr<sp1hip_stacked_data_s> sd(new sp1hip_stacked_data_s());
    SP1HIP_TRY(stacked_commit_dense(tables, n_tables, log_stacking_height, batch_size, lg_blowup, sd.get(), num_added_vals, S(stream),
                                    [&](const FillBatch& fill_batch) {
        return commit_mles_hooked(sd->batches.data(), (int)sd->batches.size(), log_stacking_height, lg_blowup, sd->commit,
                                  &sd->basefold, stream, &fill_batch);
    }));
    memcpy(h_commit, sd->commit, 32);
    *out = sd.release();
    return SP1HIP_SUCCESS;
}

void sp1hip_stacked_data_free(sp1hip_stacked_data_t* data) { delete data; }

int sp1hip_stacked_data_info(const sp1hip_stacked_data_t* data, sp1hip_basefold_data_t** basefold, int* n_batches,
                             const uint32_t** d_dense, uint64_t* padded_area) {
    SP1HIP_REQUIRE(data, "null argument");
    if (basefold) *basefold = data->basefold;
    if (n_batches) *n_batches = (int)data->batches.size();
    if (d_dense) *d_dense = (const uint32_t*)data->d_dense;
    if (padded_area) *padded_area = data->padded;
    return SP1HIP_SUCCESS;
}

int sp1hip_stacked_batch(const sp1hip_stacked_data_t* data, int k, sp1hip_tensor_t* batch) {
    SP1HIP_REQUIRE(data && batch && k >= 0 && k < (int)data->batches.size(), "bad argument");
    *batch = data->batches[k];
    return SP1HIP_SUCCESS;
}

int sp1hip_jagged_commit(const sp1hip_table_t* tables, int n_tables, int max_log_row_count, int log_stacking_height,
                         int batch_size, int lg_blowup, uint32_t h_commit[8], sp1hip_stacked_data_t** out,
                         sp1hip_stream_t stream) {
    SP1HIP_REQUIRE(h_commit && out, "bad argument");
    JaggedTables t;
    SP1HIP_TRY(jagged_select_tables(tables, n_tables, max_log_row_count, &t));
    uint32_t inner[8];
    uint64_t added = 0;
    SP1HIP_TRY(sp1hip_stacked_commit(t.dense.data(), (int)t.dense.size(), log_stacking_height, batch_size, lg_blowup, inner,
                                     &added, out, stream));
    std::vector<uint32_t> meta = jagged_finish_counts(added, max_log_row_count, std::move(t), *out);
    for (uint32_t& x : meta) x = kb::to_monty(x);
    uint32_t h[8];
    host_hash(meta, h);
    host_compress(inner, h, h_commit);
    memcpy((*out)->jagged_commit, h_commit, 32);
    return SP1HIP_SUCCESS;
}

}
```

### sp1_amd/csrc/zc_compile.cpp

```cpp
#include <algorithm>
#include <cstring>
#include <functional>
#include <memory>
#include <mutex>
#include <unordered_map>
#include <vector>

#include "zc_compile.hpp"

namespace sp1hip {

constexpr uint32_t ZC_CHUNK_LIMIT = 96;
constexpr uint32_t ZC_CHUNK_HARD_MAX = 320;

static inline bool zc_is_imm(uint32_t op) { return op >= ZC_ADDC && op <= ZC_MULC; }

static void fold_immediates(const uint32_t* ssa, uint32_t n, std::vector<uint32_t>* out) {
    out->assign(ssa, ssa + (size_t)n * 3);
    for (uint32_t k = 0; k < n; k++) {
        const uint32_t op = ssa[3 * k], a = ssa[3 * k + 1], b = ssa[3 * k + 2];
        if (op != ZC_ADD && op != ZC_SUB && op != ZC_MUL) continue;
        const bool ca = ssa[3 * a] == ZC_CONST, cb = ssa[3 * b] == ZC_CONST;
        if (ca == cb) continue;
        uint32_t* o = out->data() + 3 * (size_t)k;
// ... 577 lines not shown
            }
            std::vector<uint32_t> users(main_width, 0);
            std::vector<std::vector<uint8_t>> in_prod(np->polys.size(), std::vector<uint8_t>(main_width, 0)), in_any = in_prod;
            for (size_t pi = 0; pi < np->polys.size(); pi++) {
                const ZcPoly& pl = np->polys[pi];
                auto mark = [&](const ZcLinForm& f, bool prod) { for (uint32_t c : f.cols) if (c < main_width) { in_any[pi][c] = 1; if (prod) in_prod[pi][c] = 1; } };
                for (const ZcPolyTerm& t : pl.terms) for (int f = 0; f < 3; f++) for (auto& lf : t.f[f]) mark(lf, true);
                for (auto& f : pl.rest) mark(f, false);
                for (uint32_t c = 0; c < main_width; c++) users[c] += in_any[pi][c];
            }
            for (size_t pi = 0; pi < np->polys.size(); pi++)
                for (uint32_t c = 0; c < main_width; c++)
                    if (in_any[pi][c] && !in_prod[pi][c] && !interp[c] && users[c] == 1) np->polys[pi].owned.push_back(c);
        }
        for (const ZcPoly& pl : np->polys) np->poly_segs.push_back(zc_poly_segments(pl));
        auto drop_hinted = [&](std::vector<uint32_t>& sch) {
            if (np->macros.empty()) return;
            for (size_t k = 0; k < sch.size() / 3; k++)
                if (sch[3 * k] == ZC_ASSERT_ZERO && hinted(sch[3 * k + 2])) { sch[3 * k] = ZC_CONST; sch[3 * k + 1] = 0; sch[3 * k + 2] = 0; }
        };
        std::vector<uint32_t> folded, sched;
        fold_immediates(program, n_instr, &folded);
        constexpr uint32_t ZC_LAZY_MIN_REGS = 64;
        uint32_t best_regs = 0xffffffffu;
        for (int mode = 0; mode < 4; mode++) {
            if (mode == 3 && best_regs < ZC_LAZY_MIN_REGS) continue;
            std::vector<uint32_t> cand;
            std::vector<Chunk> mono;
            schedule_program(folded.data(), n_instr, main_width, mode, &cand);
            std::vector<uint32_t> cand_f = cand;
            drop_hinted(cand_f);
            SP1HIP_TRY(build_chunks(cand_f.data(), (uint32_t)(cand_f.size() / 3), main_width, prep_width, 0xffffffffu, &mono, ZC_CHUNK_HARD_MAX, &np->macros, &np->polys));
            uint32_t regs = 0;
            for (auto& ck : mono) regs = std::max(regs, ck.n_regs);
            if (regs < best_regs) { best_regs = regs; sched.swap(cand); np->mono.swap(mono); }
        }
        const uint32_t n_sched = (uint32_t)(sched.size() / 3);
        if (zc_debug) {
            size_t mono_instr = 0;
            for (auto& ck : np->mono) mono_instr += ck.prog.size() / 4;
            fprintf(stderr, "[sp1hip zc] chip %d: %u ssa instrs, %u+%u cols -> undivided program %zu words, %u registers\n",
                    chip_index, n_instr, main_width, prep_width, mono_instr, best_regs);
        }
        SP1HIP_TRY(allocate_registers(sched.data(), n_sched, &np->prog, &np->n_regs));
        std::vector<uint32_t> sched_f = sched;
        drop_hinted(sched_f);
        SP1HIP_TRY(build_chunks(sched_f.data(), n_sched, main_width, prep_width, ZC_CHUNK_LIMIT, &np->chunks, ZC_CHUNK_HARD_MAX, &np->macros, &np->polys));
        SP1HIP_TRY(build_chunks(sched_f.data(), n_sched, main_width, prep_width, ZC_FINE_LIMIT, &np->fine, ZC_FINE_LIMIT, &np->macros, &np->polys));
        np->sched = sched;
        if (!np->macros.empty()) {
            std::vector<uint32_t> row(main_width), prow(std::max<uint32_t>(prep_width, 1u)), want(asserts_total(program, n_instr), 0u);
            uint64_t x = 0x9E3779B97F4A7C15ull ^ h;
            auto rnd = [&]() { x ^= x << 13; x ^= x >> 7; x ^= x << 17; return (uint32_t)(x % kb::P); };
            for (auto& v : row) v = rnd();
            for (auto& v : prow) v = rnd();
            uint32_t n_pub = 1;
            for (uint32_t k = 0; k < n_instr; k++) if (program[3 * k] == ZC_PUBLIC) n_pub = std::max(n_pub, program[3 * k + 1] + 1);
            std::vector<uint32_t> pub(n_pub, 0u);
            eval_words_row(np->prog.data(), np->prog.size() / 4, np->n_regs, row.data(), prow.data(), pub.data(),
                           [&](uint32_t idx, uint32_t v) { if (idx < want.size()) want[idx] = v; });
            for (const ZcMacro& m : np->macros) {
                bool ok = true;
                uint32_t n_seen = 0;
                macro_eval_row(m, np->polys, row.data(), [&](uint32_t j, uint32_t v) {
                    n_seen++;
                    const bool same = m.first_constraint + j < want.size() && want[m.first_constraint + j] == v;
                    if (!same && zc_debug)
                        fprintf(stderr, "[sp1hip zc] hint kind %u: constraint %u + %u: pieces give %08x, the program %08x\n", m.kind, m.first_constraint, j,
                                v, m.first_constraint + j < want.size() ? want[m.first_constraint + j] : 0u);
                    ok &= same;
                });
                SP1HIP_REQUIRE(ok && n_seen == m.n_constraints(), "a fused-kernel hint does not match the constraints it annotates");
            }
        }
        plan = np;
        std::lock_guard<std::mutex> lk(plan_mutex);
        if (plan_cache.size() > 4096) plan_cache.clear();
        plan_cache[h] = plan;
    }
    *out = plan;
    return SP1HIP_SUCCESS;
}

Ext zc_eval_zero_row(const ZcPlan& plan, const Ext* alpha_pows, const uint32_t* publics) {
    Ext acc = kb::ext_zero();
    eval_words_row(plan.prog.data(), plan.prog.size() / 4, plan.n_regs, nullptr, nullptr, publics,
                   [&](uint32_t idx, uint32_t v) { acc = acc + kb::ext_mul_base(alpha_pows[idx], v); });
    return acc;
}

}

using namespace sp1hip;

extern "C" int sp1hip_zerocheck_plan_eval(const uint32_t* program, uint32_t n_instr, uint32_t main_width, uint32_t prep_width,
                                          const uint32_t* main_row, const uint32_t* prep_row, const uint32_t* publics,
                                          uint32_t n_publics, int form, uint32_t* out_values, uint32_t n_constraints,
                                          uint32_t* out_stats) {
    SP1HIP_REQUIRE(program || n_instr == 0, "null program");
    SP1HIP_REQUIRE(out_values || n_constraints == 0, "null output");
    SP1HIP_REQUIRE(form >= 0 && form <= 3, "form: 0 whole program, 1 chunks, 2 undivided, 3 fine");
    uint32_t asserts = 0;
    for (uint32_t k = 0; k < n_instr; k++) {
        const uint32_t op = program[3 * k], a = program[3 * k + 1];
        SP1HIP_REQUIRE(op <= ZC_ASSERT_ZERO || op == ZC_HINT, "bad opcode in constraint program");
        if (op == ZC_ASSERT_ZERO) asserts++;
        if (op == ZC_LOAD_MAIN) SP1HIP_REQUIRE(a < main_width && main_row, "main column out of range");
        if (op == ZC_LOAD_PREP) SP1HIP_REQUIRE(a < prep_width && prep_row, "preprocessed column out of range");
        if (op == ZC_PUBLIC) SP1HIP_REQUIRE(a < n_publics && publics, "public value index out of range");
    }
    SP1HIP_REQUIRE(asserts == n_constraints, "n_constraints does not match the program");
    std::shared_ptr<const ZcPlan> plan;
    SP1HIP_TRY(zc_get_plan(program, n_instr, main_width, prep_width, -1, &plan));
    std::vector<uint32_t> seen(n_constraints, 0);
    auto on_assert = [&](uint32_t idx, uint32_t v) { if (idx < n_constraints) { out_values[idx] = v; seen[idx]++; } };
    uint32_t words = 0, pieces = 0, regs = 0;
    if (form == 0) {
        eval_words_row(plan->prog.data(), plan->prog.size() / 4, plan->n_regs, main_row, prep_row, publics, on_assert);
        words = (uint32_t)(plan->prog.size() / 4); pieces = 1; regs = plan->n_regs;
    } else {
        const std::vector<Chunk>& cks = form == 1 ? plan->chunks : form == 2 ? plan->mono : plan->fine;
        for (const Chunk& ck : cks) {
            eval_words_row(ck.prog.data(), ck.prog.size() / 4, ck.n_regs, main_row, prep_row, publics, on_assert);
            words += (uint32_t)(ck.prog.size() / 4); pieces++; regs = std::max(regs, ck.n_regs);
        }
    }
    if (form != 0) {
        for (const ZcMacro& m : plan->macros) {
            macro_eval_row(m, plan->polys, main_row, [&](uint32_t j, uint32_t v) { on_assert(m.first_constraint + j, v); });
            pieces += m.n_pieces();
        }
    }
    for (uint32_t k = 0; k < n_constraints; k++) SP1HIP_REQUIRE(seen[k] == 1, "a constraint was not evaluated exactly once");
    if (out_stats) { out_stats[0] = words; out_stats[1] = pieces; out_stats[2] = regs; }
    return SP1HIP_SUCCESS;
}

extern "C" int sp1hip_zerocheck_poly_check(const uint32_t* program, uint32_t n_instr, uint32_t main_width, uint32_t prep_width,
                                           const uint32_t* main_row, sp1hip_ext_t alpha_c, sp1hip_ext_t* out_collapsed,
                                           sp1hip_ext_t* out_direct, uint32_t* n_identities) {
    SP1HIP_REQUIRE(program && main_row && out_collapsed && out_direct && n_identities, "null argument");
    for (uint32_t k = 0; k < n_instr; k++) SP1HIP_REQUIRE(program[3 * k] <= ZC_ASSERT_ZERO || program[3 * k] == ZC_HINT, "bad opcode in constraint program");
    std::shared_ptr<const ZcPlan> plan;
    SP1HIP_TRY(zc_get_plan(program, n_instr, main_width, prep_width, -1, &plan));
    const Ext alpha{{alpha_c.c[0], alpha_c.c[1], alpha_c.c[2], alpha_c.c[3]}};
    SP1HIP_REQUIRE(!kb::ext_eq(alpha, kb::ext_zero()), "the batching challenge is zero");
    const uint32_t n_c = asserts_total(program, n_instr);
    std::vector<Ext> pows(n_c);
    { Ext cur = kb::ext_one(); for (uint32_t k = n_c; k-- > 0;) { pows[k] = cur; cur = cur * alpha; } }
    const Ext rho = kb::ext_inv(alpha);
    Ext collapsed = kb::ext_zero(), direct = kb::ext_zero();
    std::vector<kb::Ext> scratch[2];
    uint32_t count = 0;
    for (const ZcMacro& m : plan->macros) {
        if (m.kind != ZC_HINT_POLY) continue;
        count++;
        const ZcPoly& pl = plan->polys[m.aux0];
        std::vector<uint32_t> tb;
        zc_poly_table(pl, plan->poly_segs[m.aux0], pows.data() + m.first_constraint, rho, &tb, scratch);
        size_t off = ZC_POLY_HDR;
        auto form = [&](uint32_t n, bool with_const) -> Ext {
            Ext f = kb::ext_zero();
            if (with_const) { f = Ext{{tb[off + 4], tb[off + 5], tb[off + 6], tb[off + 7]}}; off += ZC_POLY_ENTRY; }
            for (uint32_t k = 0; k < n; k++, off += ZC_POLY_ENTRY) f = f + kb::ext_mul_base(Ext{{tb[off + 4], tb[off + 5], tb[off + 6], tb[off + 7]}}, main_row[tb[off]]);
            return f;
        };
        Ext v = kb::ext_zero();
        for (uint32_t t = 0; t < tb[0]; t++) {
            Ext p = form(tb[4 + 3 * t], true) * form(tb[5 + 3 * t], true);
            if (tb[6 + 3 * t] != ZC_POLY_NONE) p = p * form(tb[6 + 3 * t], true);
            v = v + p;
// ... 11 lines not shown
```

### sp1_amd/csrc/zc_compile.hpp

```cpp
#pragma once
#include <memory>
#include <vector>

#include "common.hpp"
#include "zc_device.hpp"
#include "zc_poseidon2.hpp"
#include "zc_keccak.hpp"
#include "zc_mul.hpp"
#include "zc_poly.hpp"

namespace sp1hip {

using Ext = kb::Ext;
static inline Ext operator+(const Ext& a, const Ext& b) { return kb::ext_add(a, b); }
static inline Ext operator-(const Ext& a, const Ext& b) { return kb::ext_sub(a, b); }
static inline Ext operator*(const Ext& a, const Ext& b) { return kb::ext_mul(a, b); }

struct ZcMacro {
    uint32_t kind, base_col, first_constraint, aux0 = 0, aux1 = 0;
    uint32_t n_c = 0;
    uint32_t n_constraints() const { return kind == ZC_HINT_POLY ? n_c : kind == ZC_HINT_POSEIDON2 ? ZC_P2_CONSTRAINTS : kind == ZC_HINT_KECCAK ? ZC_KK_CONSTRAINTS : kind == ZC_HINT_MUL ? ZC_MUL_CONSTRAINTS : kind == ZC_HINT_SEPTIC_CURVE ? 7u : 14u; }
    uint32_t n_pieces() const { return kind == ZC_HINT_POLY ? 1u : kind == ZC_HINT_POSEIDON2 ? ZC_P2_PIECES : kind == ZC_HINT_KECCAK ? ZC_KK_PIECES : kind == ZC_HINT_MUL ? ZC_MUL_PIECES : kind == ZC_HINT_SEPTIC_CURVE ? 2u : 4u; }
    uint32_t n_host_pieces() const { return kind == ZC_HINT_SEPTIC_CURVE ? 1u : kind == ZC_HINT_SEPTIC_SUM ? 2u : n_pieces(); }
    void owned(uint32_t* lo, uint32_t* n) const {
        if (kind == ZC_HINT_POLY) { *lo = 0; *n = 0; }
        else if (kind == ZC_HINT_POSEIDON2) { *lo = base_col; *n = ZC_P2_COLUMNS; }
        else if (kind == ZC_HINT_KECCAK) { *lo = base_col; *n = ZC_KK_COLUMNS; }
        else if (kind == ZC_HINT_MUL) { *lo = base_col + MUL_CARRY; *n = ZC_MUL_OWNED; }
        else if (kind == ZC_HINT_SEPTIC_CURVE) { *lo = base_col; *n = 14; }
        else { *lo = aux0; *n = 28; }
    }
};

struct Chunk {
    std::vector<uint32_t> prog;
    uint32_t n_regs = 1, alpha_off = 0;
};

struct ZcPlan {
    uint32_t n_instr = 0, main_w = 0, prep_w = 0;
    bool macros_enabled = true;
    bool mul_enabled = true;
    std::vector<uint32_t> source;
    std::vector<uint32_t> prog;
    uint32_t n_regs = 1;
    std::vector<Chunk> chunks, mono, fine;
    std::vector<uint32_t> sched;
    std::vector<ZcMacro> macros;
    std::vector<ZcPoly> polys;
    std::vector<std::vector<ZcPolySeg>> poly_segs;
};

constexpr uint32_t ZC_FINE_LIMIT = 32, ZC_FINE_MAX_TERMS = 64;

int zc_get_plan(const uint32_t* program, uint32_t n_instr, uint32_t main_width, uint32_t prep_width, int chip_index,
                std::shared_ptr<const ZcPlan>* out, uint64_t rows = ~0ull);

Ext zc_eval_zero_row(const ZcPlan& plan, const Ext* alpha_pows, const uint32_t* publics);

}
```

### sp1_amd/csrc/zerocheck.hip

```cpp
#include <algorithm>
#include <array>
#include <chrono>
#include <cstring>
#include <memory>
#include <vector>

#include "zc_compile.hpp"
#include "zc_kernels.hpp"

namespace sp1hip {

constexpr uint32_t ZC_MONO_MIN_TERMS = 1024;
constexpr uint32_t ZC_FORK_MAX_BLOCKS = 1u << 30;
constexpr uint32_t ZC_MAX_PAIRS = 131072;
constexpr uint32_t ZC_SMALL_ROUND_WGS = 16384;
constexpr int ZC_FORK_STREAMS = 3, ZC_N_FORK = 2;

static Ext ext_c(uint32_t canonical) { return kb::ext_from_base(kb::to_monty(canonical)); }
using UniPoly = std::vector<Ext>;

struct VGeq {
    uint32_t threshold;
    Ext geq_c, eq_c;
    VGeq fix(const Ext& alpha) const {
        VGeq r;
        r.threshold = threshold >> 1;
        r.geq_c = geq_c;
        r.eq_c = (threshold & 1) == 0 ? (kb::ext_one() - alpha) * eq_c : alpha * (eq_c + geq_c) - geq_c;
        return r;
    }
    Ext at(size_t idx) const {
        if (idx < threshold) return kb::ext_zero();
        if (idx == threshold) return eq_c + geq_c;
        return geq_c;
    }
};

struct DevBuf {
    void* p = nullptr;
    hipStream_t s = nullptr;
    size_t n = 0;
    int alloc(size_t bytes, hipStream_t stream) {
        s = stream;
        n = bytes;
        return arena_alloc(&p, bytes, stream);
    }
    void release() { arena_free(p, n, s); p = nullptr; }
    ~DevBuf() { release(); }
    DevBuf() = default;
    DevBuf(const DevBuf&) = delete;
    DevBuf& operator=(const DevBuf&) = delete;
    uint32_t* u32() const { return (uint32_t*)p; }
};

template <bool FIRST> static inline size_t zc_rf_lane_bytes(uint32_t n_regs) { return (size_t)n_regs * (FIRST ? 4 : 16); }
constexpr size_t ZC_LDS_CU = 160 * 1024;
constexpr size_t ZC_LDS_BUDGET = ZC_LDS_CU;

template <bool FIRST> static inline uint32_t zc_wg_for(uint32_t n_regs, size_t other_lds) {
    uint32_t best = 0, best_lanes = 0;
    for (uint32_t wg = 256; wg >= 64; wg >>= 1) {
        const size_t per_wg = other_lds + zc_rf_lane_bytes<FIRST>(n_regs) * wg;
        if (per_wg > ZC_LDS_CU) continue;
        const uint32_t lanes = (uint32_t)std::min<size_t>(ZC_LDS_CU / per_wg, 2048 / wg) * wg;
        if (lanes > best_lanes) { best_lanes = lanes; best = wg; }
    }
    return best;
}

struct Group { bool staged; uint32_t wg, resident, max_regs, max_instr, block_lo, n_blocks; std::vector<int> chips; };
template <bool FIRST, class Kernel>
static int launch_interpreter(Kernel kern_staged, Kernel kern_plain, uint32_t wgs_per_block, const Group& g, const ZcDesc* d_descs, int n_descs,
                              const uint32_t* eq, uint32_t eq_len, const uint32_t* publics, uint32_t* partial, hipStream_t s) {
    const size_t lds = 32 * 4 + (g.staged ? (size_t)g.max_instr * 16 : 0);
    const uint32_t wg = zc_wg_for<FIRST>(g.max_regs, lds);
    SP1HIP_REQUIRE(wg != 0, "internal: a register file that does not fit LDS reached the launch (plan_round cuts such programs finer)");
    const size_t total = lds + zc_rf_lane_bytes<FIRST>(g.max_regs) * wg;
    const Kernel kern = g.staged ? kern_staged : kern_plain;
    if (total > 48 * 1024) SP1HIP_TRY(ensure_dynamic_lds((const void*)kern, (int)ZC_LDS_BUDGET));
    hipLaunchKernelGGL(kern, dim3(g.n_blocks * wgs_per_block), dim3(wg), total, s, d_descs, n_descs, eq, eq_len, publics, partial, (uint32_t)(lds / 4), g.block_lo);
    SP1HIP_LAUNCH_CHECK();
    return SP1HIP_SUCCESS;
}
template <bool FIRST, class... Args> static int launch_round(const Group& g, Args... args) {
    return launch_interpreter<FIRST>(zc_round_kernel<FIRST, 0, true>, zc_round_kernel<FIRST, 0, false>, 3u, g, args...);
}
template <class... Args> static int launch_biv_round(const Group& g, Args... args) {
    return launch_interpreter<false>(zc_biv_round_kernel<0, true>, zc_biv_round_kernel<0, false>, (uint32_t)ZC_BIV_GROUPS, g, args...);
}

struct ByteOut {
    std::vector<uint8_t> b;
    void u64(uint64_t v) { for (int i = 0; i < 8; i++) b.push_back((uint8_t)(v >> (8 * i))); }
    void ext(const Ext& e) {
        for (int k = 0; k < 4; k++) { uint32_t c = kb::from_monty(e.c[k]); for (int i = 0; i < 4; i++) b.push_back((uint8_t)(c >> (8 * i))); }
    }
};

void challenger_observe(sp1hip_challenger_t* ch, uint32_t x);
kb::Ext challenger_sample_ext(sp1hip_challenger_t* ch);
void challenger_restore(sp1hip_challenger_t* dst, const sp1hip_challenger_t* src);
// ... 189 lines not shown
                h = h - pe * small(gq);
            }
            H[i][xi(x)][xi(y)] = h;
        }
    }
}

struct RoundPlan {
    std::vector<ZcDesc> descs;
    std::vector<ZcChipRange> ranges;
    std::vector<int> desc_chip;
    std::vector<Group> groups;
    uint32_t total_blocks = 0, macro_lo[ZC_MACRO_KINDS + 1] = {}, macro_n[ZC_MACRO_KINDS + 1] = {};
    bool poly_wave = false;
    std::vector<ZcFixDesc> fds;
    std::vector<uint32_t*> fresh;
    std::vector<std::pair<int, bool>> owner;
    uint32_t fix_blocks = 0;
    size_t off_ranges = 0, off_fds = 0, pack_bytes = 0;
    std::vector<uint8_t> pack;
    std::vector<uint64_t> rows_next;
    std::vector<const uint32_t*> main_next, prep_next;
    int n_launches() const { return (int)groups.size() + (macro_n[1] ? 1 : 0) + (macro_n[2] ? 1 : 0) + (macro_n[3] ? 1 : 0) + (macro_n[5] ? 1 : 0) + (macro_n[7] ? 1 : 0); }
};
struct PlanViews { const ZcDesc* descs; const ZcChipRange* ranges; const ZcFixDesc* fds; };

struct RoundFork {
    hipStream_t s = nullptr;
    bool forked = false;
    hipStream_t* fork_s = nullptr;
    hipEvent_t* fork_ev = nullptr;
    bool used[ZC_FORK_STREAMS] = {};
    int begin(hipStream_t caller, bool fork) {
        s = caller;
        forked = fork;
        if (forked) {
            SP1HIP_TRY(fork_streams_for(s, ZC_FORK_STREAMS, &fork_s, &fork_ev));
            SP1HIP_HIP(hipEventRecord(fork_ev[0], s));
        }
        return SP1HIP_SUCCESS;
    }
    int stream_of(int slot, hipStream_t* out) {
        *out = s;
        if (!forked || slot == 0) return SP1HIP_SUCCESS;
        if (slot > ZC_N_FORK) slot = 1 + (slot - 1) % ZC_N_FORK;
        if (!used[slot - 1]) { used[slot - 1] = true; SP1HIP_HIP(hipStreamWaitEvent(fork_s[slot - 1], fork_ev[0], 0)); }
        *out = fork_s[slot - 1];
        return SP1HIP_SUCCESS;
    }
    int join() {
        if (forked)
            for (int k = 0; k < ZC_FORK_STREAMS; k++)
                if (used[k]) {
                    SP1HIP_HIP(hipEventRecord(fork_ev[1 + k], fork_s[k]));
                    SP1HIP_HIP(hipStreamWaitEvent(s, fork_ev[1 + k], 0));
                }
        return SP1HIP_SUCCESS;
    }
};

struct ZcTimer {
    enum Part { PLAN, WAIT, UNI };
    using Clock = std::chrono::steady_clock;
    bool on = false;
    Clock::time_point t0, t1, t2, iter;
    double part_ms[3] = {0, 0, 0};
    static double ms(Clock::time_point a, Clock::time_point b) { return std::chrono::duration<double, std::milli>(b - a).count(); }
    void start() { on = env_flag("SP1HIP_ZC_TIMING", false); t0 = t1 = t2 = iter = Clock::now(); }
    void setup_done() { t1 = iter = Clock::now(); }
    void lap(Part p) {
        if (!on) return;
        const auto now = Clock::now();
        part_ms[p] += ms(iter, now);
        iter = now;
    }
    void rounds_done() { t2 = Clock::now(); }
    void report(int n_rounds) const {
        if (!on) return;
        fprintf(stderr, "[sp1hip zerocheck] set-up %.3f ms | %d rounds %.3f ms (planning + launches %.3f, waiting for the sums %.3f, univariates + transcript %.3f) | openings + proof %.3f ms\n",
                ms(t0, t1), n_rounds, ms(t1, t2), part_ms[PLAN], part_ms[WAIT], part_ms[UNI], ms(t2, Clock::now()));
    }
};

struct ZcProver {
    const sp1hip_zc_chip_t* chips;
    const int n_chips, L;
    const sp1hip_ext_t *h_zeta, *h_openings;
    const Ext alpha, gkr;
    const uint32_t* h_publics;
    const int n_publics;
    sp1hip_challenger_t* challenger;
    uint8_t* h_proof;
    size_t* proof_len;
    hipStream_t s;

    ActiveProver active;
    size_t need = 0;
    const DeviceCtx* ctx = nullptr;
    ZcTimer timer;
    std::vector<uint32_t> publics;
    DevBuf d_publics;
    Mailbox mb;
    RoundSyncHost rsync;
    PinnedStage stage;
    std::vector<uint32_t> blob;
    std::vector<std::unique_ptr<ChipState>> st;
    DevBuf d_blob;
    std::vector<Ext> zeta;
    DevBuf d_eq_all;
    RoundTranscript tr;
    std::vector<std::array<uint32_t, 16>> sums;
    std::vector<uint32_t> h_sums;
    DevBuf d_partial, d_sums;
    size_t partial_cap = 0;
    DevBuf d_fold[2];
    DevBuf d_descs2[2];
    size_t descs_cap2[2] = {0, 0};
    bool fork_enabled = true, bivariate = true;
    std::vector<std::unique_ptr<RoundPlan>> plans;

    ZcProver(const sp1hip_zc_chip_t* chips_, int n_chips_, int max_log_row_count, const sp1hip_ext_t* h_zeta_, const sp1hip_ext_t* h_openings_,
             sp1hip_ext_t alpha_c, sp1hip_ext_t gkr_c, const uint32_t* h_publics_, int n_publics_, sp1hip_challenger_t* challenger_,
             uint8_t* h_proof_, size_t* proof_len_, sp1hip_stream_t stream)
        : chips(chips_), n_chips(n_chips_), L(max_log_row_count), h_zeta(h_zeta_), h_openings(h_openings_),
          alpha{{alpha_c.c[0], alpha_c.c[1], alpha_c.c[2], alpha_c.c[3]}}, gkr{{gkr_c.c[0], gkr_c.c[1], gkr_c.c[2], gkr_c.c[3]}},
          h_publics(h_publics_), n_publics(n_publics_), challenger(challenger_), h_proof(h_proof_), proof_len(proof_len_), s(S(stream)) {}

    int check_arguments() {
        SP1HIP_REQUIRE(chips && n_chips > 0 && h_zeta && h_openings && challenger && proof_len, "null argument");
        SP1HIP_REQUIRE(L >= 1 && L <= 30, "max_log_row_count out of range");
        SP1HIP_REQUIRE(h_publics || n_publics == 0, "null publics");
        size_t total_w = 0;
        for (int i = 0; i < n_chips; i++) {
            SP1HIP_REQUIRE(chips[i].program || chips[i].n_instr == 0, "null constraint program");
            SP1HIP_REQUIRE(chips[i].real_rows <= ((uint64_t)1 << L), "chip taller than 2^max_log_row_count");
            SP1HIP_REQUIRE(chips[i].real_rows == 0 || (chips[i].d_main || chips[i].main_width == 0), "null main trace");
            SP1HIP_REQUIRE(chips[i].real_rows == 0 || (chips[i].d_prep || chips[i].prep_width == 0), "null preprocessed trace");
            total_w += chips[i].main_width + chips[i].prep_width;
        }
        need = 8 + (size_t)L * (8 + 80) + 16 + 8 + (size_t)L * 16 + 16 + 8 + (size_t)n_chips * 8 + total_w * 16;
        if (!h_proof || *proof_len < need) {
            *proof_len = need;
            set_error("sp1hip_zerocheck_prove: proof buffer too small, need %zu bytes", need);
            return SP1HIP_ERROR_BUFFER_TOO_SMALL;
        }
        return SP1HIP_SUCCESS;
    }

    int setup_chips() {
        SP1HIP_TRY(get_device_ctx(&ctx));
        timer.start();
        publics.assign(h_publics, h_publics + n_publics);
        SP1HIP_TRY(d_publics.alloc((size_t)n_publics * 4, s));

        int max_constraints = 0;
        for (int i = 0; i < n_chips; i++) max_constraints = std::max<int>(max_constraints, chips[i].num_constraints);
        std::vector<Ext> pows(max_constraints);
        { Ext cur = kb::ext_one(); for (auto& x : pows) { x = cur; cur = cur * alpha; } }

        SP1HIP_TRY(mb.init(s));
        SP1HIP_TRY(rsync.init(s));
        SP1HIP_TRY(stage.init(s));
        if (n_publics) SP1HIP_TRY(stage.upload(d_publics.p, publics.data(), (size_t)n_publics * 4));
        Ext rho = kb::ext_zero();
        bool have_rho = false;
        std::vector<kb::Ext> poly_scratch[2];
        tr.chip.resize(n_chips);
        size_t oo = 0;
        for (int i = 0; i < n_chips; i++) {
            std::unique_ptr<ChipState> c(new ChipState());
            c->in = &chips[i];
            uint32_t asserts = 0;
            for (uint32_t k = 0; k < chips[i].n_instr; k++) {
                const uint32_t op = chips[i].program[3 * k], a = chips[i].program[3 * k + 1];
                SP1HIP_REQUIRE(op <= ZC_ASSERT_ZERO || op == ZC_HINT, "bad opcode in constraint program");
                if (op == ZC_ASSERT_ZERO) asserts++;
                if (op == ZC_LOAD_MAIN) SP1HIP_REQUIRE(a < chips[i].main_width, "main column out of range");
                if (op == ZC_LOAD_PREP) SP1HIP_REQUIRE(a < chips[i].prep_width, "preprocessed column out of range");
                if (op == ZC_PUBLIC) SP1HIP_REQUIRE((int)a < n_publics, "public value index out of range");
            }
            SP1HIP_REQUIRE(asserts == chips[i].num_constraints, "num_constraints does not match the program");
            {
                std::shared_ptr<const ZcPlan> plan;
                SP1HIP_TRY(zc_get_plan(chips[i].program, chips[i].n_instr, chips[i].main_width, chips[i].prep_width, i, &plan, chips[i].real_rows));
                c->chunks = plan->chunks; c->mono = plan->mono; c->fine = plan->fine;
                c->macros = plan->macros;
                c->plan = plan;
            }
            c->alpha_pows.assign(pows.begin(), pows.begin() + chips[i].num_constraints);
            std::reverse(c->alpha_pows.begin(), c->alpha_pows.end());
            { Ext cur = gkr; for (uint32_t k = 0; k < chips[i].main_width + chips[i].prep_width; k++) { c->gkr_pows.push_back(cur); cur = cur * gkr; } }
            ChipClaim& cc = tr.chip[i];
            cc.pad_adj = zc_eval_zero_row(*c->plan, c->alpha_pows.data(), publics.data());
            Ext claim = kb::ext_zero();
            for (uint32_t k = 0; k < chips[i].main_width + chips[i].prep_width; k++, oo++) {
                const Ext o{{h_openings[oo].c[0], h_openings[oo].c[1], h_openings[oo].c[2], h_openings[oo].c[3]}};
                claim = claim + o * c->gkr_pows[k];
            }
            tr.claims.push_back(claim);
            cc.rows = chips[i].real_rows;
            cc.eq_adj = kb::ext_one();
            cc.vgeq = VGeq{(uint32_t)chips[i].real_rows, kb::ext_one(), kb::ext_zero()};
            c->d_main = chips[i].d_main;
            c->d_prep = chips[i].d_prep;
            auto pad4 = [&]() { while (blob.size() & 3) blob.push_back(0); };
            pad4();
            c->off_prog = blob.size();
            for (auto form : {std::make_pair(&c->chunks, &c->chunk_off), std::make_pair(&c->mono, &c->mono_off), std::make_pair(&c->fine, &c->fine_off)})
                for (auto& ck : *form.first) {
                    form.second->push_back((uint32_t)((blob.size() - c->off_prog) / 4));
                    blob.insert(blob.end(), ck.prog.begin(), ck.prog.end());
                }
            pad4();
            c->off_alpha = blob.size();
            for (const Ext& e : c->alpha_pows) blob.insert(blob.end(), e.c, e.c + 4);
            c->off_gkr = blob.size();
            for (const Ext& e : c->gkr_pows) blob.insert(blob.end(), e.c, e.c + 4);
            c->poly_off.assign(c->macros.size(), 0);
            for (size_t mi = 0; mi < c->macros.size(); mi++) {
                const ZcMacro& m = c->macros[mi];
                if (m.kind != ZC_HINT_POLY) continue;
                if (!have_rho) {
                    SP1HIP_REQUIRE(!kb::ext_eq(alpha, kb::ext_zero()), "the batching challenge is zero");
                    rho = kb::ext_inv(alpha); have_rho = true;
                }
                while (blob.size() & 7) blob.push_back(0);
                c->poly_off[mi] = blob.size();
                zc_poly_table(c->plan->polys[m.aux0], c->plan->poly_segs[m.aux0], c->alpha_pows.data() + m.first_constraint, rho, &blob, poly_scratch);
            }
            st.push_back(std::move(c));
        }
        SP1HIP_TRY(d_blob.alloc(std::max<size_t>(blob.size(), 4) * 4, s));
        SP1HIP_TRY(stage.upload(d_blob.p, blob.data(), blob.size() * 4));
        for (auto& c : st) {
            c->p_prog = d_blob.u32() + c->off_prog;
            c->p_alpha = d_blob.u32() + c->off_alpha;
            c->p_gkr = d_blob.u32() + c->off_gkr;
            c->p_blob = d_blob.u32();
        }
        return SP1HIP_SUCCESS;
    }

    int setup_rounds() {
        zeta.resize(L);
        memcpy(zeta.data(), h_zeta, (size_t)L * 16);
        tr.begin(challenger);
        SP1HIP_TRY(d_eq_all.alloc(((size_t)1 << L) * 16, s));
        SP1HIP_TRY(eq_prefix_tables_soa_async(zeta.data(), L - 1, d_eq_all.u32(), s));
        sums.resize(n_chips);
        h_sums.resize((size_t)n_chips * 64);
        SP1HIP_TRY(d_sums.alloc((size_t)n_chips * 256, s));
        {
            size_t words[2] = {4, 4};
            for (int half = 0; half < 2; half++)
                for (int i = 0; i < n_chips; i++) {
                    uint64_t rows = chips[i].real_rows;
                    for (int k = 0; k < half && rows; k++) rows = (rows + 1) / 2;
                    if (rows == 0) continue;
                    const uint64_t out_rows = (rows + 1) / 2;
                    for (uint32_t width : {chips[i].main_width, chips[i].prep_width})
                        if (width) words[half] += (((size_t)out_rows * width * 4 + 3) & ~(size_t)3);
                }
            SP1HIP_TRY(d_fold[0].alloc(words[0] * 4, s));
            SP1HIP_TRY(d_fold[1].alloc(words[1] * 4, s));
        }
        timer.setup_done();
        fork_enabled = env_flag("SP1HIP_ZC_FORK", true);
        bivariate = env_flag("SP1HIP_ZC_BIVARIATE", true) && L >= 2;
        return plan_next(0);
    }

    int plan_round(int r, const std::vector<uint64_t>& vrows, const std::vector<const uint32_t*>& vmain,
                   const std::vector<const uint32_t*>& vprep, RoundPlan& rp, bool biv) {
        const uint64_t unit = biv ? 4 : 2;
        std::vector<ZcDesc>& descs = rp.descs;
        std::vector<ZcChipRange>& ranges = rp.ranges;
        std::vector<int>& desc_chip = rp.desc_chip;
        std::vector<Group>& groups = rp.groups;
        std::vector<char> use_mono(n_chips, 0);
        for (int i = 0; i < n_chips; i++) {
            ChipState& c = *st[i];
            if (vrows[i] == 0) continue;
            const uint32_t terms = (uint32_t)((vrows[i] + unit - 1) / unit);
            uint32_t mono_regs = 1;
            for (auto& ck : c.mono) mono_regs = std::max(mono_regs, ck.n_regs);
            const uint32_t mono_wg = (r == 0 && !biv) ? zc_wg_for<true>(mono_regs, 128) : zc_wg_for<false>(mono_regs, 128);
            size_t chunk_words = 0, mono_words = 0;
            for (auto& ck : c.chunks) chunk_words += ck.prog.size();
            for (auto& ck : c.mono) mono_words += ck.prog.size();
            use_mono[i] = c.chunks.size() > 1 && terms >= ZC_MONO_MIN_TERMS && mono_wg != 0 && 2 * chunk_words > 3 * mono_words;
            if (!use_mono[i] && terms <= ZC_FINE_MAX_TERMS && c.fine.size() > c.chunks.size()) use_mono[i] = 2;
            const std::vector<Chunk>& cks = use_mono[i] == 1 ? c.mono : use_mono[i] == 2 ? c.fine : c.chunks;
            uint32_t regs = 1, instr = 1;
            for (auto& ck : cks) { regs = std::max(regs, ck.n_regs); instr = std::max<uint32_t>(instr, (uint32_t)(ck.prog.size() / 4)); }
            const uint32_t stage_max = (uint32_t)env_uint("SP1HIP_ZC_STAGE_MAX", 0);
            bool staged = instr <= stage_max;
            uint32_t wg = (r == 0 && !biv) ? zc_wg_for<true>(regs, staged ? 128 + (size_t)instr * 16 : 128) : zc_wg_for<false>(regs, staged ? 128 + (size_t)instr * 16 : 128);
            if (wg == 0 && use_mono[i] != 2) {
                use_mono[i] = 2;
                regs = 1; instr = 1;
                for (auto& ck : c.fine) { regs = std::max(regs, ck.n_regs); instr = std::max<uint32_t>(instr, (uint32_t)(ck.prog.size() / 4)); }
                staged = instr <= stage_max;
                wg = (r == 0 && !biv) ? zc_wg_for<true>(regs, staged ? 128 + (size_t)instr * 16 : 128) : zc_wg_for<false>(regs, staged ? 128 + (size_t)instr * 16 : 128);
            }
            SP1HIP_REQUIRE(wg != 0, "constraint program too large: one constraint keeps more than 160 extension values live (the LDS register file of one wave)");
            uint32_t resident = 0;
            if (terms > ZC_FINE_MAX_TERMS) {
                const size_t per_wg = (staged ? 128 + (size_t)instr * 16 : 128) + ((r == 0 && !biv) ? zc_rf_lane_bytes<true>(regs) : zc_rf_lane_bytes<false>(regs)) * wg;
                resident = (uint32_t)std::min<size_t>(ZC_LDS_CU / per_wg, 2048 / wg);
            }
            size_t g = 0;
            for (; g < groups.size(); g++) if (groups[g].staged == staged && groups[g].wg == wg && groups[g].resident == resident) break;
            if (g == groups.size()) groups.push_back(Group{staged, wg, resident, 1, 1, 0, 0, {}});
            groups[g].max_regs = std::max(groups[g].max_regs, regs);
            groups[g].max_instr = std::max(groups[g].max_instr, instr);
            groups[g].chips.push_back(i);
        }
        uint32_t& total_blocks = rp.total_blocks;
        total_blocks = 0;
        for (auto& g : groups) {
            g.block_lo = total_blocks;
            for (int i : g.chips) {
                ChipState& c = *st[i];
                const uint32_t terms = (uint32_t)((vrows[i] + unit - 1) / unit);
                const uint32_t bp = g.wg ? g.wg : 256u;
                uint32_t blocks = (terms + bp - 1) / bp;
                if (blocks > ZC_MAX_PAIRS / bp) blocks = std::max(1u, ZC_MAX_PAIRS / bp);
                const std::vector<Chunk>& cks = use_mono[i] == 1 ? c.mono : use_mono[i] == 2 ? c.fine : c.chunks;
                const std::vector<uint32_t>& offs = use_mono[i] == 1 ? c.mono_off : use_mono[i] == 2 ? c.fine_off : c.chunk_off;
                ZcChipRange rg{total_blocks, 0, biv ? (uint32_t)(vrows[i] / 4) : terms - 1, 0};
                for (size_t q = 0; q < cks.size(); q++) {
                    ZcDesc d{};
                    d.prog = c.p_prog + (size_t)offs[q] * 4;
                    d.n_instr = (uint32_t)(cks[q].prog.size() / 4);
                    d.main = vmain[i]; d.prep = vprep[i]; d.main_w = c.in->main_width; d.prep_w = c.in->prep_width;
                    d.rows = (uint32_t)vrows[i]; d.alpha_pows = c.p_alpha; d.gkr_pows = c.p_gkr;
                    d.block_start = total_blocks; d.n_blocks = blocks;
                    d.alpha_off = cks[q].alpha_off; d.flags = (q == 0 && !biv) ? 1u : 0u;
                    d.block_pairs = bp;
                    total_blocks += blocks;
                    descs.push_back(d);
                }
                rg.n_blocks = total_blocks - rg.block_start;
                ranges.push_back(rg);
                desc_chip.push_back(i);
            }
            g.n_blocks = total_blocks - g.block_lo;
        }
// ... 342 lines not shown
        if (!rp.descs.empty()) SP1HIP_TRY(round_sums(r, rp));
        SP1HIP_TRY(plan_next(r + 1));
        {
            std::vector<char> have(n_chips, 0);
            for (size_t k = 0; k < rp.desc_chip.size(); k++) {
                const int ci = rp.desc_chip[k];
                const uint32_t* src = h_sums.data() + k * 16;
                if (!have[ci]) { memcpy(sums[ci].data(), src, 64); have[ci] = 1; }
                else for (int w = 0; w < 12; w++) sums[ci][w] = kb::add(sums[ci][w], src[w]);
            }
        }
        std::vector<std::array<Ext, 3>> hv(n_chips);
        tr.node_values(sums, hv);
        const Ext a_r = tr.round_messages(zeta[L - r - 1], hv);
        timer.lap(ZcTimer::UNI);
        if (!rp.fds.empty()) {
            const ZcFixDesc* d_fix = device_plan(rp, r & 1).fds;
            ScopedTimer tm("zerocheck_fix", s);
            if (r == 0) hipLaunchKernelGGL(zc_fix_kernel<true>, dim3(rp.fix_blocks), dim3(256), 0, s, d_fix, (int)rp.fds.size(), a_r);
            else hipLaunchKernelGGL(zc_fix_kernel<false>, dim3(rp.fix_blocks), dim3(256), 0, s, d_fix, (int)rp.fds.size(), a_r);
            SP1HIP_LAUNCH_CHECK();
            apply_fix(rp);
        }
        tr.update_claims();
        tr.fold_rows(2);
        return SP1HIP_SUCCESS;
    }

    int write_proof() {
        ByteOut w;
        w.u64((uint64_t)L);
        for (auto& m : tr.msgs) { w.u64(m.size()); for (auto& cf : m) w.ext(cf); }
        Ext claimed = kb::ext_zero(), final_eval = kb::ext_zero();
        for (auto& cl : tr.claims) claimed = claimed * tr.lambda + cl;
        for (int i = 0; i < n_chips; i++) final_eval = final_eval * tr.lambda + tr.round_claims[i];
        w.ext(claimed);
        w.u64(tr.point.size());
        for (auto& x : tr.point) w.ext(x);
        w.ext(final_eval);
        w.u64((uint64_t)n_chips);
        std::vector<std::vector<Ext>> chip_evals(n_chips);
        {
            std::vector<ZcGatherDesc> gd;
            size_t total_words = 0;
            for (int i = 0; i < n_chips; i++) {
                ChipState& c = *st[i];
                const uint32_t wp = c.in->prep_width, wm = c.in->main_width;
                if (tr.chip[i].rows && wp) gd.push_back({c.d_prep, wp * 4, (uint32_t)total_words});
                total_words += (size_t)wp * 4;
                if (tr.chip[i].rows && wm) gd.push_back({c.d_main, wm * 4, (uint32_t)total_words});
                total_words += (size_t)wm * 4;
            }
            std::vector<uint32_t> flat(total_words, 0);
            if (!gd.empty()) {
                DevBuf d_gd, d_flat;
                SP1HIP_TRY(d_gd.alloc(gd.size() * sizeof(ZcGatherDesc), s));
                SP1HIP_TRY(d_flat.alloc(total_words * 4, s));
                SP1HIP_HIP(hipMemsetAsync(d_flat.p, 0, total_words * 4, s));
                SP1HIP_TRY(stage.upload(d_gd.p, gd.data(), gd.size() * sizeof(ZcGatherDesc)));
                hipLaunchKernelGGL(zc_gather_kernel, dim3((unsigned)gd.size()), dim3(256), 0, s, (const ZcGatherDesc*)d_gd.p, d_flat.u32());
                SP1HIP_LAUNCH_CHECK();
                SP1HIP_TRY(mb.fetch(d_flat.p, total_words, flat.data()));
            }
            size_t off = 0;
            for (int i = 0; i < n_chips; i++) {
                const uint32_t wtot = st[i]->in->prep_width + st[i]->in->main_width;
                for (uint32_t k = 0; k < wtot; k++, off += 4)
                    chip_evals[i].push_back(Ext{{flat[off], flat[off + 1], flat[off + 2], flat[off + 3]}});
                w.u64(chip_evals[i].size());
                for (auto& e : chip_evals[i]) w.ext(e);
            }
        }
        challenger_observe(challenger, kb::to_monty((uint32_t)n_chips));
        for (int i = 0; i < n_chips; i++) {
            const uint32_t wp = st[i]->in->prep_width, wm = st[i]->in->main_width;
            challenger_observe(challenger, kb::to_monty(wp));
            for (uint32_t k = 0; k < wp; k++) for (int q = 0; q < 4; q++) challenger_observe(challenger, chip_evals[i][k].c[q]);
            challenger_observe(challenger, kb::to_monty(wm));
            for (uint32_t k = 0; k < wm; k++) for (int q = 0; q < 4; q++) challenger_observe(challenger, chip_evals[i][wp + k].c[q]);
        }
        if (w.b.size() != need) { set_error("internal error: zerocheck proof size %zu != %zu", w.b.size(), need); return SP1HIP_ERROR_RUNTIME; }
        memcpy(h_proof, w.b.data(), need);
        *proof_len = need;
        return SP1HIP_SUCCESS;
    }
};

static int zerocheck_prove_impl(ZcProver& p) {
    SP1HIP_TRY(p.check_arguments());
    SP1HIP_TRY(p.setup_chips());
    SP1HIP_TRY(p.setup_rounds());
    if (p.bivariate) SP1HIP_TRY(p.run_bivariate_rounds());
    for (int r = p.bivariate ? 2 : 0; r < p.L; r++) SP1HIP_TRY(p.run_round(r));
    p.tr.update_claims();
    p.timer.rounds_done();
    SP1HIP_TRY(p.write_proof());
    p.timer.report(p.L);
    return SP1HIP_SUCCESS;
}

template <bool FIRST>
__global__ __launch_bounds__(256) void fix_last_variable_kernel(const uint32_t* __restrict__ in, uint32_t rows, uint32_t width,
                                                                kb::Ext alpha, const uint32_t* __restrict__ padding,
                                                                uint32_t* __restrict__ out) {
    using K = KT<FIRST>;
    const uint32_t out_rows = (rows + 1) / 2;
    const size_t t = (size_t)blockIdx.x * 256u + threadIdx.x;
    if (t >= (size_t)out_rows * width) return;
    const uint32_t c = (uint32_t)(t / out_rows), i = (uint32_t)(t % out_rows);
    typename K::T x = K::load(in, c, rows, 2 * i), y;
    if (2 * i + 1 < rows) y = K::load(in, c, rows, 2 * i + 1);
    else if (!padding) y = K::zero();
    else y = K::load(padding, c, 1, 0);
    const kb::Ext r = kb::ext_add(K::scale(alpha, K::sub(y, x)), K::to_ext(x));
#pragma unroll
    for (int q = 0; q < 4; q++) out[((size_t)c * 4 + q) * out_rows + i] = r.c[q];
}
}

using namespace sp1hip;

extern "C" int sp1hip_zerocheck_biv_interp_host(uint32_t r00, uint32_t r01, uint32_t r10, uint32_t r11, uint32_t node, uint32_t* out) {
    SP1HIP_REQUIRE(out && node < (uint32_t)ZC_BIV_NODES, "node out of range");
    SP1HIP_REQUIRE(r00 < kb::P && r01 < kb::P && r10 < kb::P && r11 < kb::P, "word not reduced");
    *out = zc_biv_interp(r00, r01, r10, r11, zc_biv_node(node));
    return SP1HIP_SUCCESS;
}

extern "C" int sp1hip_fix_last_variable(const uint32_t* d_in, uint64_t rows, uint32_t width, int in_is_ext, sp1hip_ext_t alpha,
                                        const uint32_t* d_padding, uint32_t* d_out, sp1hip_stream_t stream) {
    SP1HIP_REQUIRE(rows < ((uint64_t)1 << 32), "too many rows");
    if (rows == 0 || width == 0) return SP1HIP_SUCCESS;
    SP1HIP_REQUIRE(d_in && d_out && d_in != d_out, "bad buffers");
    const kb::Ext a{{alpha.c[0], alpha.c[1], alpha.c[2], alpha.c[3]}};
    const uint64_t total = ((rows + 1) / 2) * width;
    SP1HIP_REQUIRE((total + 255) / 256 < ((uint64_t)1 << 31), "table too large for one launch");
    const dim3 grid((unsigned)((total + 255) / 256));
    if (in_is_ext) hipLaunchKernelGGL(fix_last_variable_kernel<false>, grid, dim3(256), 0, S(stream), d_in, (uint32_t)rows, width, a, d_padding, d_out);
    else hipLaunchKernelGGL(fix_last_variable_kernel<true>, grid, dim3(256), 0, S(stream), d_in, (uint32_t)rows, width, a, d_padding, d_out);
    SP1HIP_LAUNCH_CHECK();
    return SP1HIP_SUCCESS;
}

extern "C" int sp1hip_zerocheck_prove(const sp1hip_zc_chip_t* chips, int n_chips, int max_log_row_count,
                                      const sp1hip_ext_t* h_zeta, const sp1hip_ext_t* h_openings, sp1hip_ext_t alpha,
                                      sp1hip_ext_t gkr_batch, const uint32_t* h_publics, int n_publics,
                                      sp1hip_challenger_t* challenger, uint8_t* h_proof, size_t* proof_len,
                                      sp1hip_stream_t stream) {
    sp1hip_challenger_t* backup = nullptr;
    if (challenger) SP1HIP_TRY(sp1hip_challenger_clone(challenger, &backup));
    int st;
    {
        ZcProver p(chips, n_chips, max_log_row_count, h_zeta, h_openings, alpha, gkr_batch, h_publics, n_publics, challenger, h_proof, proof_len, stream);
        st = zerocheck_prove_impl(p);
    }
    if (st != SP1HIP_SUCCESS && challenger) challenger_restore(challenger, backup);
    sp1hip_challenger_free(backup);
    return st;
}
```

Measured before the change: 102.8 million.

## Prepare GKR and zerocheck host plans while the trace commitment runs

Splits the GKR and zerocheck provers into a challenge-independent prepared stage (parsing interaction programs, level layouts, constraint plans, flat program tables, fold buffer sizes) and a proving stage. A hook in the MLE commit lets that preparation run on the host while the device builds the Merkle tree, taking the host setup off the critical path. The jagged evaluation also gains a 4x4 transfer-matrix fold for the layers above D. The change adds a fair amount of plumbing and hand-over structs between stages.

Measured after the change: 102.9 million, median of 4. About the same (+0.1%).

```diff
diff --git a/sp1_amd/csrc/gkr.hip b/sp1_amd/csrc/gkr.hip
--- a/sp1_amd/csrc/gkr.hip
+++ b/sp1_amd/csrc/gkr.hip
@@ -19,6 +19,7 @@
 #include "ext_host.hpp"
 #include "gkr_kernels.hpp"
 #include "gkr_rounds_host.hpp"
+#include "stage_prepared.hpp"
 
 namespace sp1hip {
 
@@ -129,7 +130,7 @@
     uint32_t rows_at(uint32_t i, int l) const { return (uint32_t)(((uint64_t)h[i] + (((uint64_t)1 << (L - l)) - 1)) >> (L - l)); }
     void* n_ptr(int l, uint32_t i) const { return (char*)N[l].p + off[l][i] * (l == L ? 4 : 16); }
     Ext* d_ptr(int l, uint32_t i) const { return D[l].ext() + off[l][i]; }
-    int alloc(int L_, std::vector<uint32_t> rows_of_interaction, hipStream_t s) {
+    void layout(int L_, std::vector<uint32_t> rows_of_interaction) {
         L = L_; h = std::move(rows_of_interaction); K = (uint32_t)h.size();
         entries.assign(L + 2, 0);
         off.assign(L + 1, std::vector<size_t>(K + 1, 0));
@@ -137,6 +138,8 @@
             for (uint32_t i = 0; i < K; i++) off[l][i + 1] = off[l][i] + rows_at(i, l);
             entries[l] = off[l][K];
         }
+    }
+    int alloc(hipStream_t s) {
         N = std::vector<DeviceBuf>(L + 1); D = std::vector<DeviceBuf>(L + 1);
         for (int l = 1; l <= L; l++) {
             SP1HIP_TRY(N[l].alloc(std::max<size_t>(entries[l], 1) * (l == L ? 4 : 16), s));
@@ -400,50 +403,22 @@
 #define SP1HIP_GKR_REQUIRE(cond, msg) \
     do { if (!(cond)) { sp1hip::set_error("sp1hip_logup_gkr_prove: %s", msg); return SP1HIP_ERROR_INVALID_ARGUMENT; } } while (0)
 
-struct GkrProver {
-    const sp1hip_gkr_chip_t* const chips;
-    const int n_chips, L;
-    sp1hip_challenger_t* const challenger;
-    uint8_t* const h_proof;
-    size_t* const proof_len;
-    const sp1hip_stream_t stream;
-    const hipStream_t s;
-
-    GkrTimer timer;
-    const Consts k;
+struct GkrPrepared {
+    const sp1hip_gkr_chip_t* chips = nullptr;
+    int n_chips = 0, L = 0;
     std::vector<ChipInfo> info;
     std::vector<ParsedInt> progs;
     size_t max_arity = 0, total_cols = 0, need = 0;
     uint32_t K = 0, W = 0;
     int niv = 0;
-    struct Cloned { sp1hip_challenger_t* c = nullptr; ~Cloned() { sp1hip_challenger_free(c); } } clone;
-    sp1hip_challenger_t* ch = nullptr;
-    uint32_t witness = 0, flat_max_slots = 0;
-    int lookahead = 2;
-    Ext alpha;
-    std::vector<Ext> betas;
     std::vector<uint32_t> int_chip;
     Levels lv;
+    uint32_t flat_max_slots = 0;
+    int lookahead = 2;
     size_t n_passes_total = 0;
-    hipStream_t side = nullptr;
-    hipEvent_t* side_ev = nullptr;
-    DeviceBuf d_all, d_flat;
-    PinnedStage side_stage, stage;
-    DeviceBuf d_progs, d_betas, d_descs;
     std::vector<uint32_t> flat;
-    std::vector<IntDesc> descs;
-    DeviceBuf d_trans, d_trans2;
-    Mailbox mb;
-    DeviceBuf d_eq_int, d_T, d_TL, d_partials, scratch[2];
-    bool direct_final = false, simd = false;
-    PassPlan plan;
-    std::vector<Ext> out_n, out_d, eval_point;
-    Ext num_eval, den_eval;
-    size_t launch_idx = 0;
-    RoundSyncHost rsync;
-    std::optional<HostPar::Scope> par;
-    std::vector<RoundOut> rounds;
-    std::vector<Ext> trace_point, openings;
+    std::vector<size_t> poff;
+    double build_ms = 0;
 
     int parse_programs() {
         info.resize(n_chips);
@@ -495,16 +470,90 @@
         return SP1HIP_SUCCESS;
     }
 
-    size_t proof_size() const {
-        size_t n = 2 * (8 + (size_t)2 * W * 16 + 24) + 8;
-        for (int v = 1; v <= L - 1; v++) n += 64 + 8 + (size_t)(niv + v) * (8 + 64) + 16 + 8 + (size_t)(niv + v) * 16 + 16;
-        n += 8 + (size_t)L * 16 + 8;
-        for (int c = 0; c < n_chips; c++) {
-            n += 8 + info[c].name.size() + 8 + (size_t)info[c].main_w * 16 + 16 + 1;
-            if (info[c].prep_w) n += 8 + (size_t)info[c].prep_w * 16 + 16;
-        }
-        return n + 4;
-    }
+    size_t proof_size() const { return gkr_proof_size(chips, n_chips, L, K); }
+
+    void layout_and_programs() {
+        int_chip.resize(K);
+        std::vector<uint32_t> rows(K);
+        for (int c = 0; c < n_chips; c++) for (uint32_t i = 0; i < info[c].k; i++) { int_chip[info[c].int0 + i] = c; rows[info[c].int0 + i] = info[c].rows; }
+        lv.layout(L, std::move(rows));
+        flat_max_slots = (uint32_t)env_uint("SP1HIP_GKR_FLAT_SLOTS", 65536);
+        lookahead = (int)std::min<uint64_t>(std::max<uint64_t>(env_uint("SP1HIP_GKR_LOOKAHEAD", GKR_LOOKAHEAD_DEFAULT), 2), 4);
+        n_passes_total = count_passes(lv, flat_max_slots, lookahead);
+        poff.resize(K);
+        for (uint32_t i = 0; i < K; i++) {
+            poff[i] = flat.size();
+            const ParsedInt& pi = progs[i];
+            uint32_t live = 0;
+            for (size_t j = 0; j < pi.values.size(); j++) live += pi.values[j][0] != 0;
+            flat.insert(flat.end(), {pi.is_send, live, 0u, 0u, 0u, 0u});
+            flat.insert(flat.end(), pi.mult.begin(), pi.mult.end());
+            for (size_t j = 0; j < pi.values.size(); j++) {
+                if (pi.values[j][0] == 0) continue;
+                flat.push_back((uint32_t)(1 + j));
+                flat.insert(flat.end(), pi.values[j].begin(), pi.values[j].end());
+            }
+        }
+    }
+
+    int build(const sp1hip_gkr_chip_t* chips_, int n_chips_, int L_) {
+        const auto t0 = std::chrono::steady_clock::now();
+        chips = chips_; n_chips = n_chips_; L = L_;
+        SP1HIP_TRY(parse_programs());
+        need = proof_size();
+        layout_and_programs();
+        build_ms = std::chrono::duration<double, std::milli>(std::chrono::steady_clock::now() - t0).count();
+        return SP1HIP_SUCCESS;
+    }
+};
+
+struct GkrProver {
+    GkrPrepared& pp;
+    sp1hip_challenger_t* const challenger;
+    uint8_t* const h_proof;
+    size_t* const proof_len;
+    const sp1hip_stream_t stream;
+    const hipStream_t s;
+
+    const sp1hip_gkr_chip_t* const chips = pp.chips;
+    const int n_chips = pp.n_chips, L = pp.L;
+    const std::vector<ChipInfo>& info = pp.info;
+    const std::vector<ParsedInt>& progs = pp.progs;
+    const size_t max_arity = pp.max_arity, total_cols = pp.total_cols, need = pp.need;
+    const uint32_t K = pp.K, W = pp.W;
+    const int niv = pp.niv;
+    const std::vector<uint32_t>& int_chip = pp.int_chip;
+    Levels& lv = pp.lv;
+    const uint32_t flat_max_slots = pp.flat_max_slots;
+    const int lookahead = pp.lookahead;
+    const size_t n_passes_total = pp.n_passes_total;
+    std::vector<uint32_t>& flat = pp.flat;
+
+    GkrTimer timer;
+    const Consts k;
+    struct Cloned { sp1hip_challenger_t* c = nullptr; ~Cloned() { sp1hip_challenger_free(c); } } clone;
+    sp1hip_challenger_t* ch = nullptr;
+    uint32_t witness = 0;
+    Ext alpha;
+    std::vector<Ext> betas;
+    hipStream_t side = nullptr;
+    hipEvent_t* side_ev = nullptr;
+    DeviceBuf d_all, d_flat;
+    PinnedStage side_stage, stage;
+    DeviceBuf d_progs, d_betas, d_descs;
+    std::vector<IntDesc> descs;
+    DeviceBuf d_trans, d_trans2;
+    Mailbox mb;
+    DeviceBuf d_eq_int, d_T, d_TL, d_partials, scratch[2];
+    bool direct_final = false, simd = false;
+    PassPlan plan;
+    std::vector<Ext> out_n, out_d, eval_point;
+    Ext num_eval, den_eval;
+    size_t launch_idx = 0;
+    RoundSyncHost rsync;
+    std::optional<HostPar::Scope> par;
+    std::vector<RoundOut> rounds;
+    std::vector<Ext> trace_point, openings;
 
     int transcript_head() {
         SP1HIP_TRY(sp1hip_challenger_clone(challenger, &clone.c));
@@ -519,14 +568,8 @@
     }
 
     int alloc_levels_and_plan_buffers() {
-        int_chip.resize(K);
-        std::vector<uint32_t> rows(K);
-        for (int c = 0; c < n_chips; c++) for (uint32_t i = 0; i < info[c].k; i++) { int_chip[info[c].int0 + i] = c; rows[info[c].int0 + i] = info[c].rows; }
-        SP1HIP_TRY(lv.alloc(L, std::move(rows), s));
-        timer.mark("parse + level buffers");
-        flat_max_slots = (uint32_t)env_uint("SP1HIP_GKR_FLAT_SLOTS", 65536);
-        lookahead = (int)std::min<uint64_t>(std::max<uint64_t>(env_uint("SP1HIP_GKR_LOOKAHEAD", GKR_LOOKAHEAD_DEFAULT), 2), 4);
-        n_passes_total = count_passes(lv, flat_max_slots, lookahead);
+        SP1HIP_TRY(lv.alloc(s));
+        timer.mark("grind + level buffers");
         SP1HIP_TRY(aux_stream_for(s, 2, &side, &side_ev));
         SP1HIP_TRY(d_all.alloc(std::max<size_t>(n_passes_total * K, 1) * sizeof(PassDesc), side));
         SP1HIP_TRY(d_flat.alloc((n_passes_total * (size_t)flat_max_slots + 4) * sizeof(uint16_t), side));
@@ -535,23 +578,13 @@
     }
 
     int build_first_layer_and_tree() {
-        std::vector<size_t> poff(K);
+        const std::vector<size_t>& poff = pp.poff;
         for (uint32_t i = 0; i < K; i++) {
-            poff[i] = flat.size();
             const ParsedInt& pi = progs[i];
             Ext head = alpha + kb::ext_mul_base(betas[0], kb::to_monty(pi.kind));
-            uint32_t live = 0;
-            for (size_t j = 0; j < pi.values.size(); j++) {
+            for (size_t j = 0; j < pi.values.size(); j++)
                 if (pi.values[j][0] == 0) head = head + kb::ext_mul_base(betas[1 + j], pi.values[j][1]);
-                else live++;
-            }
-            flat.insert(flat.end(), {pi.is_send, live, head.c[0], head.c[1], head.c[2], head.c[3]});
-            flat.insert(flat.end(), pi.mult.begin(), pi.mult.end());
-            for (size_t j = 0; j < pi.values.size(); j++) {
-                if (pi.values[j][0] == 0) continue;
-                flat.push_back((uint32_t)(1 + j));
-                flat.insert(flat.end(), pi.values[j].begin(), pi.values[j].end());
-            }
+            memcpy(&flat[poff[i] + 2], head.c, 16);
         }
         SP1HIP_TRY(upload(d_progs, flat.data(), flat.size() * 4, s, stage));
         SP1HIP_TRY(upload(d_betas, betas.data(), betas.size() * 16, s, stage));
@@ -919,8 +952,7 @@
 
     int prove() {
         timer.start();
-        SP1HIP_TRY(parse_programs());
-        need = proof_size();
+        if (timer.on) fprintf(stderr, "[sp1hip gkr] %-28s %8.3f ms (before this call's clock: host only)\n", "prepared", pp.build_ms);
         if (!h_proof || *proof_len < need) {
             *proof_len = need;
             set_error("sp1hip_logup_gkr_prove: proof buffer too small, need %zu bytes", need);
@@ -941,7 +973,47 @@
         return SP1HIP_SUCCESS;
     }
 };
+}
+
+size_t gkr_proof_size(const sp1hip_gkr_chip_t* chips, int n_chips, int L, uint32_t K) {
+    const uint32_t W = 1u << gkr::log2_ceil(K);
+    const int niv = gkr::log2_ceil(K);
+    size_t n = 2 * (8 + (size_t)2 * W * 16 + 24) + 8;
+    for (int v = 1; v <= L - 1; v++) n += 64 + 8 + (size_t)(niv + v) * (8 + 64) + 16 + 8 + (size_t)(niv + v) * 16 + 16;
+    n += 8 + (size_t)L * 16 + 8;
+    for (int c = 0; c < n_chips; c++) {
+        n += 8 + strlen(chips[c].name) + 8 + (size_t)chips[c].main_width * 16 + 16 + 1;
+        if (chips[c].prep_width) n += 8 + (size_t)chips[c].prep_width * 16 + 16;
+    }
+    return n + 4;
+}
+int gkr_shape_size(const sp1hip_gkr_chip_t* chips, int n_chips, int L, size_t* out) {
+    uint64_t K = 0;
+    for (int c = 0; c < n_chips; c++) {
+        SP1HIP_GKR_REQUIRE(chips[c].name && chips[c].interactions, "null chip field");
+        SP1HIP_GKR_REQUIRE(chips[c].n_words >= 1, "empty interaction program");
+        K += chips[c].interactions[0];
+    }
+    SP1HIP_GKR_REQUIRE(K >= 1, "no interactions in the shard");
+    SP1HIP_GKR_REQUIRE(K < ((uint64_t)1 << 24), "too many interactions in the shard");
+    *out = gkr_proof_size(chips, n_chips, L, (uint32_t)K);
+    return SP1HIP_SUCCESS;
+}
 #undef SP1HIP_GKR_REQUIRE
+void GkrPreparedFree::operator()(gkr::GkrPrepared* p) const { delete p; }
+int gkr_prepare(const sp1hip_gkr_chip_t* chips, int n_chips, int L, GkrPreparedPtr* out) {
+    GkrPreparedPtr pp(new gkr::GkrPrepared());
+    SP1HIP_TRY(pp->build(chips, n_chips, L));
+    *out = std::move(pp);
+    return SP1HIP_SUCCESS;
+}
+size_t gkr_prepared_size(const gkr::GkrPrepared& pp) { return pp.need; }
+int gkr_prove_prepared(gkr::GkrPrepared& pp, sp1hip_challenger_t* challenger, uint8_t* h_proof, size_t* proof_len, sp1hip_stream_t stream,
+                       GkrHandOver* hand) {
+    gkr::GkrProver p{pp, challenger, h_proof, proof_len, stream, S(stream)};
+    SP1HIP_TRY(p.prove());
+    if (hand) { hand->zeta = std::move(p.trace_point); hand->openings = std::move(p.openings); }
+    return SP1HIP_SUCCESS;
 }
 }
 
@@ -951,6 +1023,8 @@
                                       uint8_t* h_proof, size_t* proof_len, sp1hip_stream_t stream) {
     SP1HIP_REQUIRE(chips && n_chips > 0 && challenger && proof_len, "bad argument");
     SP1HIP_REQUIRE(max_log_row_count >= 1 && max_log_row_count <= 30, "max_log_row_count out of range");
-    gkr::GkrProver p{chips, n_chips, max_log_row_count, challenger, h_proof, proof_len, stream, S(stream)};
+    gkr::GkrPrepared pp;
+    SP1HIP_TRY(pp.build(chips, n_chips, max_log_row_count));
+    gkr::GkrProver p{pp, challenger, h_proof, proof_len, stream, S(stream)};
     return p.prove();
 }
diff --git a/sp1_amd/csrc/jagged.hip b/sp1_amd/csrc/jagged.hip
--- a/sp1_amd/csrc/jagged.hip
+++ b/sp1_amd/csrc/jagged.hip
@@ -205,6 +205,41 @@
                             e = e + er[rb] * ei[ib];
                         }
                 }
+    }
+    const int layers = (int)std::max(z_row.size(), z_index.size()) + 1;
+    if (layers <= D || D < 1) return;
+    auto mul = [](const Ext* a, const Ext* b, Ext* c) {
+        for (int m = 0; m < 4; m++)
+            for (int j = 0; j < 4; j++) {
+                Ext acc = kb::ext_zero();
+                for (int k = 0; k < 4; k++) acc = acc + a[4 * m + k] * b[4 * k + j];
+                c[4 * m + j] = acc;
+            }
+    };
+    Ext H[16], tmp[16];
+    for (int e = 0; e < 16; e++) H[e] = e % 5 == 0 ? one : kb::ext_zero();
+    for (int layer = D; layer < layers; layer++) {
+        const Ext zr = lsb(z_row, layer), zi = lsb(z_index, layer);
+        const Ext er[2] = {one - zr, zr}, ei[2] = {one - zi, zi};
+        Ext M[16];
+        for (auto& e : M) e = kb::ext_zero();
+        for (int m = 0; m < 4; m++) {
+            const int carry = m & 1, cmp = m >> 1;
+            for (int rb = 0; rb < 2; rb++)
+                for (int ib = 0; ib < 2; ib++) {
+                    const int sum = rb + carry;
+                    if (ib != (sum & 1)) continue;
+                    const int new_cmp = ib == 0 ? cmp : 0;
+                    M[4 * m + (sum >> 1) + 2 * new_cmp] = M[4 * m + (sum >> 1) + 2 * new_cmp] + er[rb] * ei[ib];
+                }
+        }
+        mul(H, M, tmp);
+        memcpy(H, tmp, sizeof H);
+    }
+    for (int q = 0; q < 4; q++) {
+        Ext* A = out->data() + ((size_t)(D - 1) * 4 + q) * 16;
+        mul(A, H, tmp);
+        memcpy(A, tmp, sizeof tmp);
     }
 }
 
diff --git a/sp1_amd/csrc/prover.hip b/sp1_amd/csrc/prover.hip
--- a/sp1_amd/csrc/prover.hip
+++ b/sp1_amd/csrc/prover.hip
@@ -512,7 +512,8 @@
 }
 
 int commit_mles_hooked(const sp1hip_tensor_t* mles, int n_mles, int lg_n, int lg_blowup, uint32_t h_commit[8],
-                       sp1hip_basefold_data_t** out, sp1hip_stream_t stream, const std::function<int(int, hipStream_t)>* before_encode) {
+                       sp1hip_basefold_data_t** out, sp1hip_stream_t stream, const std::function<int(int, hipStream_t)>* before_encode,
+                       const std::function<void()>* while_committing) {
     SP1HIP_REQUIRE(mles && n_mles > 0 && out && h_commit, "bad argument");
     SP1HIP_REQUIRE(lg_n >= 0 && lg_blowup >= 0 && lg_n + lg_blowup <= kb::TWO_ADICITY, "size out of range");
     hipStream_t s = S(stream);
@@ -558,6 +559,7 @@
                                           (uint32_t)N, carry.u32(), pd->tree.u32(), ctx, s));
             }
             SP1HIP_TRY(merkle_finish_tree(pd->tree.u32(), lg_h, tw, rc.u32(), ctx, s));
+            if (while_committing) (*while_committing)();
             SP1HIP_TRY(basefold_data_fetch_commit(pd.get(), rc.u32(), h_commit, s));
         }
         *out = pd.release();
@@ -568,6 +570,7 @@
         SP1HIP_TRY(sp1hip_rs_encode_batch(pd->cws[i]->u32(), mles[i].d_data, lg_n, lg_blowup, mles[i].width, s));
     }
     SP1HIP_TRY(sp1hip_merkle_commit(pd->cw_tensors.data(), n_mles, lg_h, pd->tree.u32(), rc.u32(), s));
+    if (while_committing) (*while_committing)();
     SP1HIP_TRY(basefold_data_fetch_commit(pd.get(), rc.u32(), h_commit, s));
     *out = pd.release();
     return SP1HIP_SUCCESS;
@@ -578,7 +581,7 @@
 
 int sp1hip_commit_mles(const sp1hip_tensor_t* mles, int n_mles, int lg_n, int lg_blowup, uint32_t h_commit[8],
                        sp1hip_basefold_data_t** out, sp1hip_stream_t stream) {
-    return commit_mles_hooked(mles, n_mles, lg_n, lg_blowup, h_commit, out, stream, nullptr);
+    return commit_mles_hooked(mles, n_mles, lg_n, lg_blowup, h_commit, out, stream, nullptr, nullptr);
 }
 
 void sp1hip_basefold_data_free(sp1hip_basefold_data_t* data) { delete data; }
diff --git a/sp1_amd/csrc/shard.hip b/sp1_amd/csrc/shard.hip
--- a/sp1_amd/csrc/shard.hip
+++ b/sp1_amd/csrc/shard.hip
@@ -1,13 +1,13 @@
 #include <chrono>
 #include <cstring>
+#include <functional>
 #include <memory>
 #include <string>
-#include <mutex>
-#include <unordered_map>
 #include <vector>
 
 #include "device_ctx.hpp"
 #include "stacked_data.hpp"
+#include "stage_prepared.hpp"
 
 namespace sp1hip {
 void challenger_observe(sp1hip_challenger_t* ch, uint32_t x);
@@ -15,17 +15,11 @@
 void challenger_restore(sp1hip_challenger_t* dst, const sp1hip_challenger_t* src);
 size_t jagged_proof_size(int lsh, const std::vector<uint32_t>& round_widths, const std::vector<size_t>& tables_per_round,
                          uint64_t total_area, sp1hip_fri_config_t config);
+int jagged_commit_hooked(const sp1hip_table_t* tables, int n_tables, int max_log_row_count, int log_stacking_height, int batch_size,
+                         int lg_blowup, uint32_t h_commit[8], sp1hip_stacked_data_t** out, sp1hip_stream_t stream,
+                         const std::function<void()>* while_committing);
 
 namespace {
-
-struct Reader {
-    const uint8_t* p;
-    size_t n, o = 0;
-    uint64_t u64() { uint64_t v = 0; for (int i = 0; i < 8; i++) v |= (uint64_t)p[o + i] << (8 * i); o += 8; return v; }
-    uint32_t canonical() { uint32_t v = 0; for (int i = 0; i < 4; i++) v |= (uint32_t)p[o + i] << (8 * i); o += 4; return v; }
-    kb::Ext ext() { kb::Ext e; for (int k = 0; k < 4; k++) e.c[k] = kb::to_monty(canonical()); return e; }
-    void skip(size_t k) { o += k; }
-};
 
 void put_u64(std::vector<uint8_t>& b, uint64_t v) { for (int i = 0; i < 8; i++) b.push_back((uint8_t)(v >> (8 * i))); }
 void put_felt(std::vector<uint8_t>& b, uint32_t monty) { const uint32_t v = kb::from_monty(monty); for (int i = 0; i < 4; i++) b.push_back((uint8_t)(v >> (8 * i))); }
@@ -78,31 +72,8 @@
     }
 
     size_t gkr_size = 0, zc_size = 0;
-    uint64_t size_sig = shape_sig;
-    for (int c = 0; c < n_chips; c++) {
-        size_sig = (size_sig ^ ((uint64_t)chips[c].n_words << 32 | chips[c].num_constraints)) * 0x100000001b3ull;
-        size_sig = (size_sig ^ ((uint64_t)strlen(chips[c].name) << 32 | chips[c].prep_width)) * 0x100000001b3ull;
-    }
-    size_sig = (size_sig ^ (uint64_t)n_publics) * 0x100000001b3ull;
-    static std::mutex size_mutex;
-    static std::unordered_map<uint64_t, std::pair<size_t, size_t>> size_cache;
-    bool have_sizes = false;
-    {
-        std::lock_guard<std::mutex> lk(size_mutex);
-        auto it = size_cache.find(size_sig);
-        if (it != size_cache.end()) { gkr_size = it->second.first; zc_size = it->second.second; have_sizes = true; }
-    }
-    if (!have_sizes) {
-        int st = sp1hip_logup_gkr_prove(gk.data(), n_chips, L, challenger, nullptr, &gkr_size, stream);
-        if (st != SP1HIP_ERROR_BUFFER_TOO_SMALL) return st == SP1HIP_SUCCESS ? SP1HIP_ERROR_RUNTIME : st;
-        std::vector<sp1hip_ext_t> dummy(std::max<size_t>({total_w, (size_t)L, 1}));
-        st = sp1hip_zerocheck_prove(zc.data(), n_chips, L, dummy.data(), dummy.data(), dummy[0], dummy[0], h_publics, n_publics,
-                                    challenger, nullptr, &zc_size, stream);
-        if (st != SP1HIP_ERROR_BUFFER_TOO_SMALL) return st == SP1HIP_SUCCESS ? SP1HIP_ERROR_RUNTIME : st;
-        std::lock_guard<std::mutex> lk(size_mutex);
-        if (size_cache.size() > 4096) size_cache.clear();
-        size_cache[size_sig] = {gkr_size, zc_size};
-    }
+    SP1HIP_TRY(gkr_shape_size(gk.data(), n_chips, L, &gkr_size));
+    SP1HIP_TRY(zc_shape_size(zc.data(), n_chips, L, &zc_size));
     const uint64_t H = (uint64_t)1 << lsh;
     const uint64_t main_padded = std::max<uint64_t>((main_area + H - 1) / H, 1) * H;
     const std::vector<uint32_t> round_widths{(uint32_t)(preprocessed->padded >> lsh), (uint32_t)(main_padded >> lsh)};
@@ -119,6 +90,7 @@
     const bool sh_timing = env_flag("SP1HIP_SHARD_TIMING", false);
     std::chrono::steady_clock::time_point sh_t[6];
     sh_t[0] = std::chrono::steady_clock::now();
+    double prepare_ms = 0;
     RoctxRange proof_range("sp1hip_prove_shard");
     struct StageMarks {
         hipStream_t s;
@@ -144,10 +116,26 @@
         SP1HIP_REQUIRE(h_publics[i] < kb::P, "public value not reduced");
         challenger_observe(ch, h_publics[i]);
     }
+    GkrPreparedPtr gkr_pp;
+    ZcPreparedPtr zc_pp;
+    int prepare_st = SP1HIP_SUCCESS;
+    std::string prepare_err;
+    const std::function<void()> prepare_stages = [&]() {
+        const auto t0 = std::chrono::steady_clock::now();
+        prepare_st = gkr_prepare(gk.data(), n_chips, L, &gkr_pp);
+        if (prepare_st == SP1HIP_SUCCESS) prepare_st = zc_prepare(zc.data(), n_chips, L, h_publics, n_publics, &zc_pp);
+        if (prepare_st != SP1HIP_SUCCESS) prepare_err = sp1hip_last_error();
+        prepare_ms = std::chrono::duration<double, std::milli>(std::chrono::steady_clock::now() - t0).count();
+    };
     uint32_t main_commit[8];
     sp1hip_stacked_data_t* main_data = nullptr;
-    SP1HIP_TRY(sp1hip_jagged_commit(tables.data(), n_chips, L, lsh, params.batch_size, params.fri.log_blowup, main_commit, &main_data, stream));
+    const int commit_st = jagged_commit_hooked(tables.data(), n_chips, L, lsh, params.batch_size, params.fri.log_blowup, main_commit, &main_data,
+                                               stream, &prepare_stages);
     std::unique_ptr<sp1hip_stacked_data_s> main_guard(main_data);
+    if (commit_st != SP1HIP_SUCCESS) return commit_st;
+    if (prepare_st != SP1HIP_SUCCESS) { set_error("%s", prepare_err.c_str()); return prepare_st; }
+    SP1HIP_REQUIRE(gkr_pp && zc_pp, "internal: the stages were not prepared");
+    SP1HIP_REQUIRE(gkr_prepared_size(*gkr_pp) == gkr_size && zc_prepared_size(*zc_pp) == zc_size, "internal: prepared proof sizes");
     for (int k = 0; k < 8; k++) challenger_observe(ch, main_commit[k]);
     challenger_observe(ch, kb::to_monty((uint32_t)n_chips));
     for (int c = 0; c < n_chips; c++) {
@@ -161,35 +149,11 @@
     marks.next("logup_gkr");
     std::vector<uint8_t> gkr_blob(gkr_size);
     size_t glen = gkr_size;
-    SP1HIP_TRY(sp1hip_logup_gkr_prove(gk.data(), n_chips, L, ch, gkr_blob.data(), &glen, stream));
-    std::vector<kb::Ext> zeta(L), openings;
-    {
-        Reader r{gkr_blob.data(), glen};
-        for (int k = 0; k < 2; k++) { const uint64_t m = r.u64(); r.skip(m * 16 + 24); }
-        const uint64_t nr = r.u64();
-        for (uint64_t k = 0; k < nr; k++) {
-            r.skip(64);
-            const uint64_t np = r.u64();
-            for (uint64_t q = 0; q < np; q++) { const uint64_t nc = r.u64(); r.skip(nc * 16); }
-            r.skip(16);
-            const uint64_t pl = r.u64();
-            r.skip(pl * 16 + 16);
-        }
-        SP1HIP_REQUIRE(r.u64() == (uint64_t)L, "internal: GKR point dimension");
-        for (auto& z : zeta) z = r.ext();
-        SP1HIP_REQUIRE(r.u64() == (uint64_t)n_chips, "internal: GKR chip count");
-        for (int c = 0; c < n_chips; c++) {
-            r.skip(r.u64());
-            const uint64_t mw = r.u64();
-            for (uint64_t k = 0; k < mw; k++) openings.push_back(r.ext());
-            r.skip(16);
-            if (r.p[r.o++]) {
-                const uint64_t pw = r.u64();
-                for (uint64_t k = 0; k < pw; k++) openings.push_back(r.ext());
-                r.skip(16);
-            }
-        }
-    }
+    GkrHandOver gkr_out;
+    SP1HIP_TRY(gkr_prove_prepared(*gkr_pp, ch, gkr_blob.data(), &glen, stream, &gkr_out));
+    gkr_pp.reset();
+    SP1HIP_REQUIRE(gkr_out.zeta.size() == (size_t)L && gkr_out.openings.size() >= total_w, "internal: GKR hand-over");
+    const std::vector<kb::Ext>&zeta = gkr_out.zeta, &openings = gkr_out.openings;
     sh_t[2] = std::chrono::steady_clock::now();
     marks.next("zerocheck");
     const kb::Ext batching = challenger_sample_ext(ch), gkr_batch = challenger_sample_ext(ch);
@@ -198,28 +162,18 @@
     memcpy(&c_gkr, &gkr_batch, 16);
     std::vector<uint8_t> zc_blob(zc_size);
     size_t zlen = zc_size;
-    SP1HIP_TRY(sp1hip_zerocheck_prove(zc.data(), n_chips, L, reinterpret_cast<const sp1hip_ext_t*>(zeta.data()),
-                                      reinterpret_cast<const sp1hip_ext_t*>(openings.data()), c_batching, c_gkr, h_publics, n_publics, ch,
-                                      zc_blob.data(), &zlen, stream));
-    std::vector<kb::Ext> z_row(L), prep_claims, main_claims;
-    std::vector<std::vector<kb::Ext>> chip_evals(n_chips);
-    {
-        Reader r{zc_blob.data(), zlen};
-        const uint64_t np = r.u64();
-        for (uint64_t q = 0; q < np; q++) { const uint64_t nc = r.u64(); r.skip(nc * 16); }
-        r.skip(16);
-        SP1HIP_REQUIRE(r.u64() == (uint64_t)L, "internal: zerocheck point dimension");
-        for (auto& z : z_row) z = r.ext();
-        r.skip(16);
-        SP1HIP_REQUIRE(r.o == zc_sumcheck_size, "internal: zerocheck sumcheck size");
-        SP1HIP_REQUIRE(r.u64() == (uint64_t)n_chips, "internal: zerocheck chip count");
-        for (int c = 0; c < n_chips; c++) {
-            const uint64_t w = r.u64();
-            SP1HIP_REQUIRE(w == (uint64_t)chips[c].main_width + chips[c].prep_width, "internal: zerocheck opening width");
-            for (uint64_t k = 0; k < w; k++) chip_evals[c].push_back(r.ext());
-            prep_claims.insert(prep_claims.end(), chip_evals[c].begin(), chip_evals[c].begin() + chips[c].prep_width);
-            main_claims.insert(main_claims.end(), chip_evals[c].begin() + chips[c].prep_width, chip_evals[c].end());
-        }
+    ZcHandOver zc_out;
+    SP1HIP_TRY(zc_prove_prepared(*zc_pp, reinterpret_cast<const sp1hip_ext_t*>(zeta.data()), reinterpret_cast<const sp1hip_ext_t*>(openings.data()),
+                                 c_batching, c_gkr, ch, zc_blob.data(), &zlen, stream, &zc_out));
+    zc_pp.reset();
+    SP1HIP_REQUIRE(zlen == zc_size && zc_out.point.size() == (size_t)L && zc_out.chip_evals.size() == (size_t)n_chips, "internal: zerocheck hand-over");
+    const std::vector<kb::Ext>& z_row = zc_out.point;
+    const std::vector<std::vector<kb::Ext>>& chip_evals = zc_out.chip_evals;
+    std::vector<kb::Ext> prep_claims, main_claims;
+    for (int c = 0; c < n_chips; c++) {
+        SP1HIP_REQUIRE(chip_evals[c].size() == (size_t)chips[c].main_width + chips[c].prep_width, "internal: zerocheck opening width");
+        prep_claims.insert(prep_claims.end(), chip_evals[c].begin(), chip_evals[c].begin() + chips[c].prep_width);
+        main_claims.insert(main_claims.end(), chip_evals[c].begin() + chips[c].prep_width, chip_evals[c].end());
     }
     sh_t[3] = std::chrono::steady_clock::now();
     marks.next("evaluation_proof");
@@ -269,6 +223,7 @@
         const auto ms = [&](int a, int b) { return std::chrono::duration<double, std::milli>(sh_t[b] - sh_t[a]).count(); };
         uint64_t miss_n1 = 0, miss_b1 = 0;
         arena_miss_stats(&miss_n1, &miss_b1);
+        fprintf(stderr, "[sp1hip shard] stages prepared under the commit: %.3f ms of host time\n", prepare_ms);
         fprintf(stderr, "[sp1hip shard] prologue %.3f ms | commit %.3f | LogUp-GKR %.3f | zerocheck %.3f | evaluation proof %.3f | proof bytes %.3f | %llu arena misses (%.1f MB)\n",
                 std::chrono::duration<double, std::milli>(sh_t[0] - sh_entry).count(), ms(0, 1), ms(1, 2), ms(2, 3), ms(3, 4), ms(4, 5),
                 (unsigned long long)(miss_n1 - miss_n0), (double)(miss_b1 - miss_b0) / 1e6);
diff --git a/sp1_amd/csrc/stacked.hip b/sp1_amd/csrc/stacked.hip
--- a/sp1_amd/csrc/stacked.hip
+++ b/sp1_amd/csrc/stacked.hip
@@ -13,7 +13,8 @@
 
 namespace sp1hip {
 int commit_mles_hooked(const sp1hip_tensor_t* mles, int n_mles, int lg_n, int lg_blowup, uint32_t h_commit[8],
-                       sp1hip_basefold_data_t** out, sp1hip_stream_t stream, const std::function<int(int, hipStream_t)>* before_encode);
+                       sp1hip_basefold_data_t** out, sp1hip_stream_t stream, const std::function<int(int, hipStream_t)>* before_encode,
+                       const std::function<void()>* while_committing);
 }
 
 namespace {
@@ -147,23 +148,49 @@
     return meta;
 }
 
-}
-
-extern "C" {
-
-int sp1hip_stacked_commit(const sp1hip_table_t* tables, int n_tables, int log_stacking_height, int batch_size,
-                          int lg_blowup, uint32_t h_commit[8], uint64_t* num_added_vals, sp1hip_stacked_data_t** out,
-                          sp1hip_stream_t stream) {
+static int stacked_commit_hooked(const sp1hip_table_t* tables, int n_tables, int log_stacking_height, int batch_size, int lg_blowup,
+                                 uint32_t h_commit[8], uint64_t* num_added_vals, sp1hip_stacked_data_t** out, sp1hip_stream_t stream,
+                                 const std::function<void()>* while_committing) {
     SP1HIP_REQUIRE(h_commit && out, "bad argument");
     std::unique_ptr<sp1hip_stacked_data_s> sd(new sp1hip_stacked_data_s());
     SP1HIP_TRY(stacked_commit_dense(tables, n_tables, log_stacking_height, batch_size, lg_blowup, sd.get(), num_added_vals, S(stream),
                                     [&](const FillBatch& fill_batch) {
         return commit_mles_hooked(sd->batches.data(), (int)sd->batches.size(), log_stacking_height, lg_blowup, sd->commit,
-                                  &sd->basefold, stream, &fill_batch);
+                                  &sd->basefold, stream, &fill_batch, while_committing);
     }));
     memcpy(h_commit, sd->commit, 32);
     *out = sd.release();
     return SP1HIP_SUCCESS;
+}
+
+int jagged_commit_hooked(const sp1hip_table_t* tables, int n_tables, int max_log_row_count, int log_stacking_height, int batch_size,
+                         int lg_blowup, uint32_t h_commit[8], sp1hip_stacked_data_t** out, sp1hip_stream_t stream,
+                         const std::function<void()>* while_committing) {
+    SP1HIP_REQUIRE(h_commit && out, "bad argument");
+    JaggedTables t;
+    SP1HIP_TRY(jagged_select_tables(tables, n_tables, max_log_row_count, &t));
+    uint32_t inner[8];
+    uint64_t added = 0;
+    SP1HIP_TRY(stacked_commit_hooked(t.dense.data(), (int)t.dense.size(), log_stacking_height, batch_size, lg_blowup, inner, &added, out,
+                                     stream, while_committing));
+    std::vector<uint32_t> meta = jagged_finish_counts(added, max_log_row_count, std::move(t), *out);
+    for (uint32_t& x : meta) x = kb::to_monty(x);
+    uint32_t h[8];
+    host_hash(meta, h);
+    host_compress(inner, h, h_commit);
+    memcpy((*out)->jagged_commit, h_commit, 32);
+    return SP1HIP_SUCCESS;
+}
+
+}
+
+extern "C" {
+
+int sp1hip_stacked_commit(const sp1hip_table_t* tables, int n_tables, int log_stacking_height, int batch_size,
+                          int lg_blowup, uint32_t h_commit[8], uint64_t* num_added_vals, sp1hip_stacked_data_t** out,
+                          sp1hip_stream_t stream) {
+    SP1HIP_REQUIRE(h_commit && out, "bad argument");
+    return stacked_commit_hooked(tables, n_tables, log_stacking_height, batch_size, lg_blowup, h_commit, num_added_vals, out, stream, nullptr);
 }
 
 void sp1hip_stacked_data_free(sp1hip_stacked_data_t* data) { delete data; }
@@ -188,19 +215,7 @@
                          int batch_size, int lg_blowup, uint32_t h_commit[8], sp1hip_stacked_data_t** out,
                          sp1hip_stream_t stream) {
     SP1HIP_REQUIRE(h_commit && out, "bad argument");
-    JaggedTables t;
-    SP1HIP_TRY(jagged_select_tables(tables, n_tables, max_log_row_count, &t));
-    uint32_t inner[8];
-    uint64_t added = 0;
-    SP1HIP_TRY(sp1hip_stacked_commit(t.dense.data(), (int)t.dense.size(), log_stacking_height, batch_size, lg_blowup, inner,
-                                     &added, out, stream));
-    std::vector<uint32_t> meta = jagged_finish_counts(added, max_log_row_count, std::move(t), *out);
-    for (uint32_t& x : meta) x = kb::to_monty(x);
-    uint32_t h[8];
-    host_hash(meta, h);
-    host_compress(inner, h, h_commit);
-    memcpy((*out)->jagged_commit, h_commit, 32);
-    return SP1HIP_SUCCESS;
-}
-
-}
+    return jagged_commit_hooked(tables, n_tables, max_log_row_count, log_stacking_height, batch_size, lg_blowup, h_commit, out, stream, nullptr);
+}
+
+}
diff --git a/sp1_amd/csrc/stage_prepared.hpp b/sp1_amd/csrc/stage_prepared.hpp
--- /dev/null
+++ b/sp1_amd/csrc/stage_prepared.hpp
@@ -0,0 +1,30 @@
+#pragma once
+#include <memory>
+#include <vector>
+
+#include "common.hpp"
+
+namespace sp1hip {
+
+namespace gkr { struct GkrPrepared; }
+struct GkrPreparedFree { void operator()(gkr::GkrPrepared* p) const; };
+using GkrPreparedPtr = std::unique_ptr<gkr::GkrPrepared, GkrPreparedFree>;
+struct GkrHandOver { std::vector<kb::Ext> zeta, openings; };
+size_t gkr_proof_size(const sp1hip_gkr_chip_t* chips, int n_chips, int max_log_row_count, uint32_t n_interactions);
+int gkr_shape_size(const sp1hip_gkr_chip_t* chips, int n_chips, int max_log_row_count, size_t* out);
+int gkr_prepare(const sp1hip_gkr_chip_t* chips, int n_chips, int max_log_row_count, GkrPreparedPtr* out);
+size_t gkr_prepared_size(const gkr::GkrPrepared& pp);
+int gkr_prove_prepared(gkr::GkrPrepared& pp, sp1hip_challenger_t* challenger, uint8_t* h_proof, size_t* proof_len, sp1hip_stream_t stream,
+                       GkrHandOver* hand);
+
+struct ZcPrepared;
+struct ZcPreparedFree { void operator()(ZcPrepared* p) const; };
+using ZcPreparedPtr = std::unique_ptr<ZcPrepared, ZcPreparedFree>;
+struct ZcHandOver { std::vector<kb::Ext> point; std::vector<std::vector<kb::Ext>> chip_evals; };
+int zc_shape_size(const sp1hip_zc_chip_t* chips, int n_chips, int max_log_row_count, size_t* out);
+int zc_prepare(const sp1hip_zc_chip_t* chips, int n_chips, int max_log_row_count, const uint32_t* h_publics, int n_publics, ZcPreparedPtr* out);
+size_t zc_prepared_size(const ZcPrepared& pp);
+int zc_prove_prepared(ZcPrepared& pp, const sp1hip_ext_t* h_zeta, const sp1hip_ext_t* h_openings, sp1hip_ext_t alpha, sp1hip_ext_t gkr_batch,
+                      sp1hip_challenger_t* challenger, uint8_t* h_proof, size_t* proof_len, sp1hip_stream_t stream, ZcHandOver* hand);
+
+}
diff --git a/sp1_amd/csrc/zc_compile.cpp b/sp1_amd/csrc/zc_compile.cpp
--- a/sp1_amd/csrc/zc_compile.cpp
+++ b/sp1_amd/csrc/zc_compile.cpp
@@ -683,11 +683,9 @@
     return SP1HIP_SUCCESS;
 }
 
-Ext zc_eval_zero_row(const ZcPlan& plan, const Ext* alpha_pows, const uint32_t* publics) {
-    Ext acc = kb::ext_zero();
+void zc_zero_row_values(const ZcPlan& plan, const uint32_t* publics, std::vector<std::pair<uint32_t, uint32_t>>* out) {
     eval_words_row(plan.prog.data(), plan.prog.size() / 4, plan.n_regs, nullptr, nullptr, publics,
-                   [&](uint32_t idx, uint32_t v) { acc = acc + kb::ext_mul_base(alpha_pows[idx], v); });
-    return acc;
+                   [&](uint32_t idx, uint32_t v) { if (v) out->push_back({idx, v}); });
 }
 
 }
diff --git a/sp1_amd/csrc/zc_compile.hpp b/sp1_amd/csrc/zc_compile.hpp
--- a/sp1_amd/csrc/zc_compile.hpp
+++ b/sp1_amd/csrc/zc_compile.hpp
@@ -56,6 +56,6 @@
 int zc_get_plan(const uint32_t* program, uint32_t n_instr, uint32_t main_width, uint32_t prep_width, int chip_index,
                 std::shared_ptr<const ZcPlan>* out, uint64_t rows = ~0ull);
 
-Ext zc_eval_zero_row(const ZcPlan& plan, const Ext* alpha_pows, const uint32_t* publics);
+void zc_zero_row_values(const ZcPlan& plan, const uint32_t* publics, std::vector<std::pair<uint32_t, uint32_t>>* out);
 
 }
diff --git a/sp1_amd/csrc/zerocheck.hip b/sp1_amd/csrc/zerocheck.hip
--- a/sp1_amd/csrc/zerocheck.hip
+++ b/sp1_amd/csrc/zerocheck.hip
@@ -7,6 +7,7 @@
 
 #include "zc_compile.hpp"
 #include "zc_kernels.hpp"
+#include "stage_prepared.hpp"
 
 namespace sp1hip {
 
@@ -17,6 +18,9 @@
 constexpr int ZC_FORK_STREAMS = 3, ZC_N_FORK = 2;
 
 static Ext ext_c(uint32_t canonical) { return kb::ext_from_base(kb::to_monty(canonical)); }
+static size_t zc_proof_size(int L, int n_chips, size_t total_w) {
+    return 8 + (size_t)L * (8 + 80) + 16 + 8 + (size_t)L * 16 + 16 + 8 + (size_t)n_chips * 8 + total_w * 16;
+}
 using UniPoly = std::vector<Ext>;
 
 struct VGeq {
@@ -372,7 +376,88 @@
     }
 };
 
+struct ZcPrepared {
+    const sp1hip_zc_chip_t* chips = nullptr;
+    int n_chips = 0, L = 0, n_publics = 0;
+    size_t need = 0;
+    std::vector<uint32_t> publics;
+    std::vector<std::unique_ptr<ChipState>> st;
+    std::vector<std::vector<std::pair<uint32_t, uint32_t>>> zero_vals;
+    std::vector<uint32_t> blob;
+    int max_constraints = 0;
+    size_t fold_words[2] = {4, 4};
+    double build_ms = 0;
+
+    int check_arguments(const sp1hip_zc_chip_t* chips_, int n_chips_, int max_log_row_count, const uint32_t* h_publics, int n_publics_) {
+        chips = chips_; n_chips = n_chips_; L = max_log_row_count; n_publics = n_publics_;
+        SP1HIP_REQUIRE(chips && n_chips > 0, "null argument");
+        SP1HIP_REQUIRE(L >= 1 && L <= 30, "max_log_row_count out of range");
+        SP1HIP_REQUIRE(h_publics || n_publics == 0, "null publics");
+        size_t total_w = 0;
+        for (int i = 0; i < n_chips; i++) {
+            SP1HIP_REQUIRE(chips[i].program || chips[i].n_instr == 0, "null constraint program");
+            SP1HIP_REQUIRE(chips[i].real_rows <= ((uint64_t)1 << L), "chip taller than 2^max_log_row_count");
+            SP1HIP_REQUIRE(chips[i].real_rows == 0 || (chips[i].d_main || chips[i].main_width == 0), "null main trace");
+            SP1HIP_REQUIRE(chips[i].real_rows == 0 || (chips[i].d_prep || chips[i].prep_width == 0), "null preprocessed trace");
+            total_w += chips[i].main_width + chips[i].prep_width;
+        }
+        need = zc_proof_size(L, n_chips, total_w);
+        if (n_publics) publics.assign(h_publics, h_publics + n_publics);
+        return SP1HIP_SUCCESS;
+    }
+
+    int setup_chips() {
+        const auto t0 = std::chrono::steady_clock::now();
+        for (int i = 0; i < n_chips; i++) {
+            std::unique_ptr<ChipState> c(new ChipState());
+            c->in = &chips[i];
+            uint32_t asserts = 0;
+            for (uint32_t k = 0; k < chips[i].n_instr; k++) {
+                const uint32_t op = chips[i].program[3 * k], a = chips[i].program[3 * k + 1];
+                SP1HIP_REQUIRE(op <= ZC_ASSERT_ZERO || op == ZC_HINT, "bad opcode in constraint program");
+                if (op == ZC_ASSERT_ZERO) asserts++;
+                if (op == ZC_LOAD_MAIN) SP1HIP_REQUIRE(a < chips[i].main_width, "main column out of range");
+                if (op == ZC_LOAD_PREP) SP1HIP_REQUIRE(a < chips[i].prep_width, "preprocessed column out of range");
+                if (op == ZC_PUBLIC) SP1HIP_REQUIRE((int)a < n_publics, "public value index out of range");
+            }
+            SP1HIP_REQUIRE(asserts == chips[i].num_constraints, "num_constraints does not match the program");
+            max_constraints = std::max<int>(max_constraints, chips[i].num_constraints);
+            {
+                std::shared_ptr<const ZcPlan> plan;
+                SP1HIP_TRY(zc_get_plan(chips[i].program, chips[i].n_instr, chips[i].main_width, chips[i].prep_width, i, &plan, chips[i].real_rows));
+                c->chunks = plan->chunks; c->mono = plan->mono; c->fine = plan->fine;
+                c->macros = plan->macros;
+                c->plan = plan;
+            }
+            zero_vals.emplace_back();
+            zc_zero_row_values(*c->plan, publics.data(), &zero_vals.back());
+            c->d_main = chips[i].d_main;
+            c->d_prep = chips[i].d_prep;
+            while (blob.size() & 3) blob.push_back(0);
+            c->off_prog = blob.size();
+            for (auto form : {std::make_pair(&c->chunks, &c->chunk_off), std::make_pair(&c->mono, &c->mono_off), std::make_pair(&c->fine, &c->fine_off)})
+                for (auto& ck : *form.first) {
+                    form.second->push_back((uint32_t)((blob.size() - c->off_prog) / 4));
+                    blob.insert(blob.end(), ck.prog.begin(), ck.prog.end());
+                }
+            st.push_back(std::move(c));
+        }
+        for (int half = 0; half < 2; half++)
+            for (int i = 0; i < n_chips; i++) {
+                uint64_t rows = chips[i].real_rows;
+                for (int k = 0; k < half && rows; k++) rows = (rows + 1) / 2;
+                if (rows == 0) continue;
+                const uint64_t out_rows = (rows + 1) / 2;
+                for (uint32_t width : {chips[i].main_width, chips[i].prep_width})
+                    if (width) fold_words[half] += (((size_t)out_rows * width * 4 + 3) & ~(size_t)3);
+            }
+        build_ms = std::chrono::duration<double, std::milli>(std::chrono::steady_clock::now() - t0).count();
+        return SP1HIP_SUCCESS;
+    }
+};
+
 struct ZcProver {
+    ZcPrepared& pp;
     const sp1hip_zc_chip_t* chips;
     const int n_chips, L;
     const sp1hip_ext_t *h_zeta, *h_openings;
@@ -385,16 +470,16 @@
     hipStream_t s;
 
     ActiveProver active;
-    size_t need = 0;
+    const size_t need;
     const DeviceCtx* ctx = nullptr;
     ZcTimer timer;
-    std::vector<uint32_t> publics;
+    const std::vector<uint32_t>& publics;
     DevBuf d_publics;
     Mailbox mb;
     RoundSyncHost rsync;
     PinnedStage stage;
-    std::vector<uint32_t> blob;
-    std::vector<std::unique_ptr<ChipState>> st;
+    std::vector<uint32_t>& blob;
+    std::vector<std::unique_ptr<ChipState>>& st;
     DevBuf d_blob;
     std::vector<Ext> zeta;
     DevBuf d_eq_all;
@@ -408,27 +493,17 @@
     size_t descs_cap2[2] = {0, 0};
     bool fork_enabled = true, bivariate = true;
     std::vector<std::unique_ptr<RoundPlan>> plans;
-
-    ZcProver(const sp1hip_zc_chip_t* chips_, int n_chips_, int max_log_row_count, const sp1hip_ext_t* h_zeta_, const sp1hip_ext_t* h_openings_,
-             sp1hip_ext_t alpha_c, sp1hip_ext_t gkr_c, const uint32_t* h_publics_, int n_publics_, sp1hip_challenger_t* challenger_,
-             uint8_t* h_proof_, size_t* proof_len_, sp1hip_stream_t stream)
-        : chips(chips_), n_chips(n_chips_), L(max_log_row_count), h_zeta(h_zeta_), h_openings(h_openings_),
+    ZcHandOver* hand = nullptr;
+
+    ZcProver(ZcPrepared& pp_, const sp1hip_ext_t* h_zeta_, const sp1hip_ext_t* h_openings_, sp1hip_ext_t alpha_c, sp1hip_ext_t gkr_c,
+             sp1hip_challenger_t* challenger_, uint8_t* h_proof_, size_t* proof_len_, sp1hip_stream_t stream)
+        : pp(pp_), chips(pp_.chips), n_chips(pp_.n_chips), L(pp_.L), h_zeta(h_zeta_), h_openings(h_openings_),
           alpha{{alpha_c.c[0], alpha_c.c[1], alpha_c.c[2], alpha_c.c[3]}}, gkr{{gkr_c.c[0], gkr_c.c[1], gkr_c.c[2], gkr_c.c[3]}},
-          h_publics(h_publics_), n_publics(n_publics_), challenger(challenger_), h_proof(h_proof_), proof_len(proof_len_), s(S(stream)) {}
+          h_publics(pp_.publics.data()), n_publics(pp_.n_publics), challenger(challenger_), h_proof(h_proof_), proof_len(proof_len_), s(S(stream)),
+          need(pp_.need), publics(pp_.publics), blob(pp_.blob), st(pp_.st) {}
 
     int check_arguments() {
-        SP1HIP_REQUIRE(chips && n_chips > 0 && h_zeta && h_openings && challenger && proof_len, "null argument");
-        SP1HIP_REQUIRE(L >= 1 && L <= 30, "max_log_row_count out of range");
-        SP1HIP_REQUIRE(h_publics || n_publics == 0, "null publics");
-        size_t total_w = 0;
-        for (int i = 0; i < n_chips; i++) {
-            SP1HIP_REQUIRE(chips[i].program || chips[i].n_instr == 0, "null constraint program");
-            SP1HIP_REQUIRE(chips[i].real_rows <= ((uint64_t)1 << L), "chip taller than 2^max_log_row_count");
-            SP1HIP_REQUIRE(chips[i].real_rows == 0 || (chips[i].d_main || chips[i].main_width == 0), "null main trace");
-            SP1HIP_REQUIRE(chips[i].real_rows == 0 || (chips[i].d_prep || chips[i].prep_width == 0), "null preprocessed trace");
-            total_w += chips[i].main_width + chips[i].prep_width;
-        }
-        need = 8 + (size_t)L * (8 + 80) + 16 + 8 + (size_t)L * 16 + 16 + 8 + (size_t)n_chips * 8 + total_w * 16;
+        SP1HIP_REQUIRE(h_zeta && h_openings && challenger && proof_len, "null argument");
         if (!h_proof || *proof_len < need) {
             *proof_len = need;
             set_error("sp1hip_zerocheck_prove: proof buffer too small, need %zu bytes", need);
@@ -440,12 +515,10 @@
     int setup_chips() {
         SP1HIP_TRY(get_device_ctx(&ctx));
         timer.start();
-        publics.assign(h_publics, h_publics + n_publics);
+        if (timer.on) fprintf(stderr, "[sp1hip zerocheck] prepared %.3f ms (before this call's clock: host only)\n", pp.build_ms);
         SP1HIP_TRY(d_publics.alloc((size_t)n_publics * 4, s));
 
-        int max_constraints = 0;
-        for (int i = 0; i < n_chips; i++) max_constraints = std::max<int>(max_constraints, chips[i].num_constraints);
-        std::vector<Ext> pows(max_constraints);
+        std::vector<Ext> pows(pp.max_constraints);
         { Ext cur = kb::ext_one(); for (auto& x : pows) { x = cur; cur = cur * alpha; } }
 
         SP1HIP_TRY(mb.init(s));
@@ -458,30 +531,13 @@
         tr.chip.resize(n_chips);
         size_t oo = 0;
         for (int i = 0; i < n_chips; i++) {
-            std::unique_ptr<ChipState> c(new ChipState());
-            c->in = &chips[i];
-            uint32_t asserts = 0;
-            for (uint32_t k = 0; k < chips[i].n_instr; k++) {
-                const uint32_t op = chips[i].program[3 * k], a = chips[i].program[3 * k + 1];
-                SP1HIP_REQUIRE(op <= ZC_ASSERT_ZERO || op == ZC_HINT, "bad opcode in constraint program");
-                if (op == ZC_ASSERT_ZERO) asserts++;
-                if (op == ZC_LOAD_MAIN) SP1HIP_REQUIRE(a < chips[i].main_width, "main column out of range");
-                if (op == ZC_LOAD_PREP) SP1HIP_REQUIRE(a < chips[i].prep_width, "preprocessed column out of range");
-                if (op == ZC_PUBLIC) SP1HIP_REQUIRE((int)a < n_publics, "public value index out of range");
-            }
-            SP1HIP_REQUIRE(asserts == chips[i].num_constraints, "num_constraints does not match the program");
-            {
-                std::shared_ptr<const ZcPlan> plan;
-                SP1HIP_TRY(zc_get_plan(chips[i].program, chips[i].n_instr, chips[i].main_width, chips[i].prep_width, i, &plan, chips[i].real_rows));
-                c->chunks = plan->chunks; c->mono = plan->mono; c->fine = plan->fine;
-                c->macros = plan->macros;
-                c->plan = plan;
-            }
+            ChipState* const c = st[i].get();
             c->alpha_pows.assign(pows.begin(), pows.begin() + chips[i].num_constraints);
             std::reverse(c->alpha_pows.begin(), c->alpha_pows.end());
             { Ext cur = gkr; for (uint32_t k = 0; k < chips[i].main_width + chips[i].prep_width; k++) { c->gkr_pows.push_back(cur); cur = cur * gkr; } }
             ChipClaim& cc = tr.chip[i];
-            cc.pad_adj = zc_eval_zero_row(*c->plan, c->alpha_pows.data(), publics.data());
+            cc.pad_adj = kb::ext_zero();
+            for (const auto& zv : pp.zero_vals[i]) cc.pad_adj = cc.pad_adj + kb::ext_mul_base(c->alpha_pows[zv.first], zv.second);
             Ext claim = kb::ext_zero();
             for (uint32_t k = 0; k < chips[i].main_width + chips[i].prep_width; k++, oo++) {
                 const Ext o{{h_openings[oo].c[0], h_openings[oo].c[1], h_openings[oo].c[2], h_openings[oo].c[3]}};
@@ -491,17 +547,7 @@
             cc.rows = chips[i].real_rows;
             cc.eq_adj = kb::ext_one();
             cc.vgeq = VGeq{(uint32_t)chips[i].real_rows, kb::ext_one(), kb::ext_zero()};
-            c->d_main = chips[i].d_main;
-            c->d_prep = chips[i].d_prep;
-            auto pad4 = [&]() { while (blob.size() & 3) blob.push_back(0); };
-            pad4();
-            c->off_prog = blob.size();
-            for (auto form : {std::make_pair(&c->chunks, &c->chunk_off), std::make_pair(&c->mono, &c->mono_off), std::make_pair(&c->fine, &c->fine_off)})
-                for (auto& ck : *form.first) {
-                    form.second->push_back((uint32_t)((blob.size() - c->off_prog) / 4));
-                    blob.insert(blob.end(), ck.prog.begin(), ck.prog.end());
-                }
-            pad4();
+            while (blob.size() & 3) blob.push_back(0);
             c->off_alpha = blob.size();
             for (const Ext& e : c->alpha_pows) blob.insert(blob.end(), e.c, e.c + 4);
             c->off_gkr = blob.size();
@@ -518,7 +564,6 @@
                 c->poly_off[mi] = blob.size();
                 zc_poly_table(c->plan->polys[m.aux0], c->plan->poly_segs[m.aux0], c->alpha_pows.data() + m.first_constraint, rho, &blob, poly_scratch);
             }
-            st.push_back(std::move(c));
         }
         SP1HIP_TRY(d_blob.alloc(std::max<size_t>(blob.size(), 4) * 4, s));
         SP1HIP_TRY(stage.upload(d_blob.p, blob.data(), blob.size() * 4));
@@ -540,20 +585,8 @@
         sums.resize(n_chips);
         h_sums.resize((size_t)n_chips * 64);
         SP1HIP_TRY(d_sums.alloc((size_t)n_chips * 256, s));
-        {
-            size_t words[2] = {4, 4};
-            for (int half = 0; half < 2; half++)
-                for (int i = 0; i < n_chips; i++) {
-                    uint64_t rows = chips[i].real_rows;
-                    for (int k = 0; k < half && rows; k++) rows = (rows + 1) / 2;
-                    if (rows == 0) continue;
-                    const uint64_t out_rows = (rows + 1) / 2;
-                    for (uint32_t width : {chips[i].main_width, chips[i].prep_width})
-                        if (width) words[half] += (((size_t)out_rows * width * 4 + 3) & ~(size_t)3);
-                }
-            SP1HIP_TRY(d_fold[0].alloc(words[0] * 4, s));
-            SP1HIP_TRY(d_fold[1].alloc(words[1] * 4, s));
-        }
+        SP1HIP_TRY(d_fold[0].alloc(pp.fold_words[0] * 4, s));
+        SP1HIP_TRY(d_fold[1].alloc(pp.fold_words[1] * 4, s));
         timer.setup_done();
         fork_enabled = env_flag("SP1HIP_ZC_FORK", true);
         bivariate = env_flag("SP1HIP_ZC_BIVARIATE", true) && L >= 2;
@@ -1062,6 +1095,7 @@
         if (w.b.size() != need) { set_error("internal error: zerocheck proof size %zu != %zu", w.b.size(), need); return SP1HIP_ERROR_RUNTIME; }
         memcpy(h_proof, w.b.data(), need);
         *proof_len = need;
+        if (hand) { hand->point = tr.point; hand->chip_evals = std::move(chip_evals); }
         return SP1HIP_SUCCESS;
     }
 };
@@ -1122,19 +1156,55 @@
     return SP1HIP_SUCCESS;
 }
 
+static int zerocheck_run(ZcPrepared& pp, const sp1hip_ext_t* h_zeta, const sp1hip_ext_t* h_openings, sp1hip_ext_t alpha, sp1hip_ext_t gkr_batch,
+                         sp1hip_challenger_t* challenger, uint8_t* h_proof, size_t* proof_len, sp1hip_stream_t stream, ZcHandOver* hand) {
+    sp1hip_challenger_t* backup = nullptr;
+    if (challenger) SP1HIP_TRY(sp1hip_challenger_clone(challenger, &backup));
+    int st;
+    {
+        ZcProver p(pp, h_zeta, h_openings, alpha, gkr_batch, challenger, h_proof, proof_len, stream);
+        p.hand = hand;
+        st = zerocheck_prove_impl(p);
+    }
+    if (st != SP1HIP_SUCCESS && challenger) challenger_restore(challenger, backup);
+    sp1hip_challenger_free(backup);
+    return st;
+}
+
 extern "C" int sp1hip_zerocheck_prove(const sp1hip_zc_chip_t* chips, int n_chips, int max_log_row_count,
                                       const sp1hip_ext_t* h_zeta, const sp1hip_ext_t* h_openings, sp1hip_ext_t alpha,
                                       sp1hip_ext_t gkr_batch, const uint32_t* h_publics, int n_publics,
                                       sp1hip_challenger_t* challenger, uint8_t* h_proof, size_t* proof_len,
                                       sp1hip_stream_t stream) {
-    sp1hip_challenger_t* backup = nullptr;
-    if (challenger) SP1HIP_TRY(sp1hip_challenger_clone(challenger, &backup));
-    int st;
-    {
-        ZcProver p(chips, n_chips, max_log_row_count, h_zeta, h_openings, alpha, gkr_batch, h_publics, n_publics, challenger, h_proof, proof_len, stream);
-        st = zerocheck_prove_impl(p);
-    }
-    if (st != SP1HIP_SUCCESS && challenger) challenger_restore(challenger, backup);
-    sp1hip_challenger_free(backup);
-    return st;
-}
+    ZcPrepared pp;
+    SP1HIP_TRY(pp.check_arguments(chips, n_chips, max_log_row_count, h_publics, n_publics));
+    if (h_zeta && h_openings && challenger && proof_len && (!h_proof || *proof_len < pp.need)) {
+        *proof_len = pp.need;
+        set_error("sp1hip_zerocheck_prove: proof buffer too small, need %zu bytes", pp.need);
+        return SP1HIP_ERROR_BUFFER_TOO_SMALL;
+    }
+    SP1HIP_TRY(pp.setup_chips());
+    return zerocheck_run(pp, h_zeta, h_openings, alpha, gkr_batch, challenger, h_proof, proof_len, stream, nullptr);
+}
+
+namespace sp1hip {
+void ZcPreparedFree::operator()(ZcPrepared* p) const { delete p; }
+int zc_shape_size(const sp1hip_zc_chip_t* chips, int n_chips, int max_log_row_count, size_t* out) {
+    size_t total_w = 0;
+    for (int i = 0; i < n_chips; i++) total_w += chips[i].main_width + chips[i].prep_width;
+    *out = zc_proof_size(max_log_row_count, n_chips, total_w);
+    return SP1HIP_SUCCESS;
+}
+int zc_prepare(const sp1hip_zc_chip_t* chips, int n_chips, int max_log_row_count, const uint32_t* h_publics, int n_publics, ZcPreparedPtr* out) {
+    ZcPreparedPtr pp(new ZcPrepared());
+    SP1HIP_TRY(pp->check_arguments(chips, n_chips, max_log_row_count, h_publics, n_publics));
+    SP1HIP_TRY(pp->setup_chips());
+    *out = std::move(pp);
+    return SP1HIP_SUCCESS;
+}
+size_t zc_prepared_size(const ZcPrepared& pp) { return pp.need; }
+int zc_prove_prepared(ZcPrepared& pp, const sp1hip_ext_t* h_zeta, const sp1hip_ext_t* h_openings, sp1hip_ext_t alpha, sp1hip_ext_t gkr_batch,
+                      sp1hip_challenger_t* challenger, uint8_t* h_proof, size_t* proof_len, sp1hip_stream_t stream, ZcHandOver* hand) {
+    return zerocheck_run(pp, h_zeta, h_openings, alpha, gkr_batch, challenger, h_proof, proof_len, stream, hand);
+}
+}
```
